# tusen-ai/RangeDet

Hardware: AMD Instinct MI355X
Metric: range-image frames/sec (64x2650, 8ch) at 1/2/4/8 GPU; Meta-Kernel HBM GB/s vs peak (higher is better)
Workload: dtype bf16

## Files before the change

include/rangedet_hip.h:

```cpp
#ifndef RANGEDET_HIP_H_
#define RANGEDET_HIP_H_
#include <stddef.h>
#include <stdint.h>

#ifdef __cplusplus
extern "C" {
#endif

#define RD_OK 0
#define RD_EINVAL (-1)
#define RD_ESHAPE (-2)
#define RD_EWORKSPACE (-3)
#define RD_EHIP (-4)

#define RD_F32 0
#define RD_BF16 1
#define RD_F16 2

#define RD_RELU_PRE 1
#define RD_ADD 2
#define RD_RELU_POST 4
#define RD_SCALE_FOLDED 8
#define RD_MFMA16 16

int rd_version(void);
const char* rd_last_error_string(void);

int rd_nchw_to_nhwc(const float* src, void* dst, int B, int C, int H, int W, int dst_cstride, int dst_coff,
                    int zero_pad, int dst_dtype, void* stream);
int rd_nhwc_to_nchw(const void* src, float* dst, int B, int C, int H, int W, int src_cstride, int src_coff,
                    int src_dtype, void* stream);

int rd_copy_rows(const void* src, long src_row_bytes, void* dst, long dst_row_bytes, long dst_offset_bytes, long bytes,
                 int rows, void* stream);

size_t rd_conv_packed_bytes(int ntaps, int cin, int cout, int dtype);
int rd_pack_conv_weight_host(const float* w_oihw_host, int cout, int cin, int kh, int kw, int dtype,
                             void* packed_host);
int rd_deconv_phase_taps(int kh, int kw, int stride_w, int pad_w, int phase);
int rd_pack_deconv_weight_host(const float* w_iohw_host, int cin, int cout, int kh, int kw, int stride_w,
                               int pad_w, int phase, int dtype, void* packed_host);
int rd_pack_deconv_weight_folded_host(const float* w_iohw_host, const float* fold_scale_host, int cin, int cout, int kh, int kw,
                                      int stride_w, int pad_w, int phase, int dtype, void* packed_host);

int rd_conv2d_bn_act(const void* x, int x_cstride, int x_coff, const void* w_packed, const float* scale,
                     const float* shift, const void* residual, int r_cstride, int r_coff, void* y,
                     int y_cstride, int y_coff, int B, int H, int Win, int cin, int cout, int kh, int kw,
                     int stride_w, int flags, int dtype, void* stream);
size_t rd_conv3x3_ex_packed_bytes(int cin, int cout, int stride_w, int x_cstride);
int rd_pack_conv3x3_ex_host(const float* w_oihw_host, const float* fold_scale_host, int cout, int cin, int stride_w,
                            int x_cstride, int dtype, void* packed_host);
int rd_pack_conv3x3_m16_host(const float* w_oihw_host, const float* fold_scale_host, int cout, int cin, int dtype, void* packed_host);
int rd_conv3x3_mfma16_ok(int cin, int cout, int stride_w, int W, int fused_output_conv);
size_t rd_conv1x1_sc_packed_bytes(int cin, int cout);
int rd_pack_conv1x1_sc_host(const float* w_oi_host, const float* fold_scale_host, int cout, int cin, int dtype,
                            void* packed_host);
int rd_conv3x3_bn_act_ex(const void* x, int x_cstride, int x_coff, const void* w_packed, const float* scale, const float* shift,
                         const void* residual, int r_cstride, int r_coff, const void* sc_x, int sc_cstride, int sc_coff,
                         int sc_cin, const void* sc_w_packed, void* y, int y_cstride, int y_coff, int B, int H, int Win, int cin,
                         int cout, int stride_w, int flags, int dtype, void* stream);
size_t rd_block64_packed_bytes(int cin);
int rd_pack_block64_host(const float* w1_oihw_host, const float* fold_scale1_host, const float* w2_oihw_host,
                         const float* fold_scale2_host, int cin, int dtype, void* packed_host);
int rd_block64_bn_act(const void* x, int x_cstride, int x_coff, int cin, const void* w_packed, const float* shift1, const float* shift2,
                      const void* sc_w_packed, void* y, int y_cstride, int y_coff, int B, int H, int W, int dtype, void* stream);
int rd_pack_block64_m16_host(const float* w1_oihw_host, const float* fold_scale1_host, const float* w2_oihw_host,
                             const float* fold_scale2_host, int dtype, void* packed_host);
int rd_pack_conv1x1_sc_m16_host(const float* w_oi_host, const float* fold_scale_host, int dtype, void* packed_host);
int rd_block64_m16_bn_act(const void* x, int x_cstride, int x_coff, const void* w_packed, const float* shift1, const float* shift2,
                          const void* sc_w_packed, void* y, int y_cstride, int y_coff, int B, int H, int W, int dtype, void* stream);

size_t rd_head_packed_bytes(void);
int rd_pack_head_weight_host(const float* w, int nout, int cin, int dtype, void* out_host);
size_t rd_head_m16_packed_bytes(void);
int rd_pack_head_weight_m16_host(const float* w, int nout, int cin, int dtype, void* out_host);
int rd_conv2d_bn_act_head_out(const void* x, int x_cstride, int x_coff, const void* w_packed, const float* scale,
                              const float* shift, int B, int H, int W, int cin, int flags, const void* head_w_packed,
                              const float* head_bias, float* out, long out_batch_stride, long n_off, int nout, int dtype,
                              void* stream);

size_t rd_conv3x3_cat_packed_bytes(int cin1, int cin2, int cout);
int rd_pack_conv3x3_cat_host(const float* w, const float* fold_scale, int cout, int cin1, int cin2, int dtype, void* out_host);
int rd_conv3x3_bn_act_cat(const void* x1, int x1_cstride, int x1_coff, int cin1, const void* x2, int x2_cstride, int x2_coff, int cin2,
                          const void* w_packed, const float* shift, void* y, int y_cstride, int y_coff, int B, int H, int W, int cout,
                          int flags, int dtype, void* stream);

int rd_deconv2d_bn_act(const void* x, int x_cstride, int x_coff, const void* w_packed_phase,
                       const float* scale, const float* shift, const void* residual, int r_cstride,
                       int r_coff, void* y, int y_cstride, int y_coff, int B, int H, int Win, int cin,
                       int cout, int kh, int kw, int stride_w, int pad_w, int phase, int flags, int dtype,
                       void* stream);

int rd_deconv2d_all_phases_ok(int kh, int kw, int stride_w, int pad_w, int cout, int dtype);
int rd_deconv2d_bn_act_all(const void* x, int x_cstride, int x_coff, const void* w_packed_all, long w_phase_bytes,
                           const float* shift, const void* residual, int r_cstride, int r_coff, void* y, int y_cstride,
                           int y_coff, int B, int H, int Win, int cin, int cout, int kh, int kw, int stride_w, int pad_w,
                           int flags, int dtype, void* stream);

int rd_deconv2d_phase_pairs_ok(int kh, int kw, int stride_w, int pad_w, int cout, int dtype);
int rd_pack_deconv_phase_pair_host(const void* phase_a, const void* phase_b, int cin, int dtype, void* out);
int rd_deconv2d_bn_act_pairs(const void* x, int x_cstride, int x_coff, const void* w_packed_pairs, long w_pair_bytes,
                             const float* shift2, const void* residual, int r_cstride, int r_coff, void* y, int y_cstride,
                             int y_coff, int B, int H, int Win, int cin, int cout, int kh, int kw, int stride_w, int pad_w,
                             int flags, int dtype, void* stream);

int rd_head_out(const void* x, int x_cstride, int x_coff, const float* w, const float* bias, float* out,
                long out_batch_stride, long n_off, int B, int H, int W, int cin, int nout, int dtype,
                void* stream);

size_t rd_meta_packed_bytes(int dtype);
int rd_pack_meta_host(const float* w0, const float* b0, const float* w1, const float* b1, const float* s1,
                      const float* t1, const float* agg, const float* s2, const float* t2, int dtype,
                      void* packed_host);
int rd_meta_kernel_fwd(const void* data, int d_cstride, int d_coff, const float* coord_nchw,
                       const void* packed, void* y, int y_cstride, int y_coff, int B, int H, int W, int dtype,
                       void* stream);

size_t rd_sorted_foreground_workspace_bytes(long N, long k);
int rd_sorted_foreground(const float* cls_score, const float* bbox_delta, const float* pc, const float* mask,
                         int B, long N, long k, int D, int apply_sigmoid, float* out_score, float* out_delta,
                         float* out_pc, int* out_idx, void* ws, size_t ws_bytes, void* stream);

int rd_decode3d_bbox(const float* bbox_delta, const float* pc, float* out, int B, long N, int box_type,
                     int is_bin, void* stream);

size_t rd_score_filter_workspace_bytes(long n);
int rd_score_filter_dets(const float* scores, const float* boxes10, long n, float min_score, float* dets,
                         int* d_count, void* ws, size_t ws_bytes, void* stream);
int rd_score_filter_dets_batched(const float* scores, long scores_bstride, const float* boxes10, long boxes_bstride,
                                 long n, float min_score, float* dets, long dets_bstride, int* d_count, void* ws,
                                 size_t ws_bytes, int B, void* stream);

#define RD_WNMS_MAX_K 65536
#define RD_TIE_STABLE 0
#define RD_TIE_REFERENCE 1
#define RD_WNMS_DIAG_NO_SKIP 0x100
#define RD_WNMS_DIAG_TILE_W(n) (((n) & 0xff) << 16)
#define RD_WNMS_DIAG_MERGE_LDS(n) (((n) & 0x7f) << 24)
size_t rd_wnms_workspace_bytes(int Kcap);
int rd_wnms_4c(const float* dets, int Kcap, const int* d_count, const int* order, int tie_order, float thresh,
               float thresh_vote, int is3d, int hash_scale, float* out_dets, int* keep, int* d_nkeep, void* ws,
               size_t ws_bytes, void* stream);
int rd_wnms_4c_batched(const float* dets, long dets_bstride, int Kcap, const int* d_count, const int* order,
                       long order_bstride, int tie_order, float thresh, float thresh_vote, int is3d, int hash_scale,
                       float* out_dets, long out_bstride, int* keep, long keep_bstride, int* d_nkeep, void* ws,
                       size_t ws_bytes, int B, void* stream);
int rd_single_overlap(const float* dets_a, const float* dets_b, long n, int is3d, float* out, void* stream);
int rd_wnms_pair_skippable(const float* dets_a, const float* dets_b, long n, unsigned char* out, void* stream);

int rd_edge_atan2f(const float* y, const float* x, long n, float* out, void* stream);

int rd_wnms_order_host(const float* dets_host, int K, int* order_host);

int rd_dets12_to_8(const float* dets12, int Mcap, const int* d_count, float* out8, void* stream);
int rd_dets12_to_8_batched(const float* dets12, long dets12_bstride, int Mcap, const int* d_count, float* out8,
                           long out8_bstride, int B, void* stream);

int rd_rotated_iou_8pt(const float* boxes1, const float* boxes2, float* ious, long n1, long n2, void* stream);
int rd_batch_rotated_iou(const float* proposal, int p_stride, const float* gt_bbox, float* iou_map, int* argmax, int B, long N,
                         int n_gt, void* stream);
int rd_batch_rotated_iou_3d(const float* proposal, int p_stride, const float* gt_bbox7, float* iou_map, int* argmax, int B, long N,
                            int n_gt, void* stream);
int rd_rotated_iou_7(const float* boxes1, const float* boxes2, float* ious, long n1, long n2, void* stream);
int rd_batch_max_iou(const float* proposals, int p_stride, const float* gt8, float* out, long n, int n_gt,
                     void* stream);

size_t rd_nms3d_workspace_bytes(long N, int B);
int rd_gather_keep_scores(const float* score, long score_bstride, int k, const int* keep_idx, int max_keep, float* out, int B,
                          void* stream);
int rd_nms3d(const float* boxes, int B, long N, float iou_thres, int max_keep, int normal_iou, int* keep_idx,
             float* bbox_after_nms, void* ws, size_t ws_bytes, void* stream);

int rd_assign3d_v2(const float* pc, const float* bbox, const float* bbox_center, const float* bbox_radius, const float* mask,
                   const float* is_in_nlz, long N, int M, float max_x, float min_x, float max_y, float min_y, float max_z,
                   float min_z, float max_dist, int* out, void* stream);
size_t rd_get_point_num_workspace_bytes(void);
int rd_get_point_num(const float* bbox_inds, long N, float* out, void* ws, size_t ws_bytes, void* stream);

typedef struct {
  float clip_lo[7], clip_hi[7];
  float mean[8], sd[8];
  float interval_lo[3], interval_hi[3];
} rd_input_norm_t;
int rd_input_transform(const float* range_image, const float* pc_vehicle_frame, const float* inclination,
                       const rd_input_norm_t* norm_host, int B, int H, int W, int Hp, int Wp, float* input_data,
                       float* coord_s1, float* pc_s1, float* pc_s2, float* pc_s4, float* mask_s1, float* mask_s2,
                       float* mask_s4, void* stream);

typedef struct {
  float *input_data, *coord_s1;
  float *pc[3], *mask[3];
  float *reg_target[3], *reg_weight[3], *reg_normalize_weight[3], *cls_target[3];
  int* bbox3d_ind;
} rd_train_outputs_t;
size_t rd_train_transform_workspace_bytes(int B);
int rd_train_transform(const float* range_image, const float* pc_vehicle_frame, const float* inclination,
                       const rd_input_norm_t* norm_host, const float* gt_bbox_imu, const float* gt_bbox_center,
                       const float* gt_limits, const float* gt_bbox_csa, const int* num_gt_host, int Mmax, float radius,
                       float max_dist, const float* reg_weight_host, int B, int H, int W, int Hp, int Wp,
                       const rd_train_outputs_t* out_host, void* ws, size_t ws_bytes, void* stream);

size_t rd_range_image_workspace_bytes(int B, int H, int W);
int rd_range_image_from_points(const float* points, const long long* offsets_host, int B, const double* incl_host,
                               const double* height_host, int H, int W, float* range_image, unsigned char* mask, int* point_index,
                               void* ws, size_t ws_bytes, void* stream);

typedef struct {
  float alpha, gamma;
  float cls_loss_weight, reg_loss_weight;
  float smooth_l1_scalar;
  float scale_loss_shift;
  int l1;
} rd_loss_param_t;
size_t rd_rpn_loss_workspace_bytes(int B, long n);
int rd_rpn_loss(const float* logit, long logit_bstride, const float* delta, long delta_bstride, const float* pc, const float* gt_bbox,
                int n_gt, const float* mask, const float* reg_target, const float* reg_weight, const float* reg_norm_weight, int B, int H,
                int Wl, const rd_loss_param_t* p_host, float* cls_loss, float* reg_loss, float* d_logit, float* d_delta,
                float* iou_target, float* boxes10, float* stats, void* ws, size_t ws_bytes, void* stream);

int rd_relu_affine_bwd(const void* g, int g_cstride, int g_coff, const void* y, int y_cstride, int y_coff, const float* scale, void* dz,
                       int dz_cstride, int dz_coff, int B, int H, int W, int C, int dtype, void* stream);
size_t rd_conv3x3_bwd_weight_workspace_bytes(int B, int H, int W, int cin, int cout, int split);
int rd_conv3x3_bwd_weight(const void* x, int x_cstride, int x_coff, const void* dz, int dz_cstride, int dz_coff, float* dW, int B, int H,
                          int W, int cin, int cout, int split, int dtype, void* ws, size_t ws_bytes, void* stream);
size_t rd_conv1x1_bwd_weight_workspace_bytes(int B, int H, int W, int cin, int cout, int split);
size_t rd_conv3x3_bwd_weight_ex_workspace_bytes(int B, int H, int Win, int cin, int cout, int stride_w, int split);
int rd_conv3x3_bwd_weight_ex(const void* x, int x_cstride, int x_coff, const void* dz, int dz_cstride, int dz_coff, float* dW, int B, int H,
                             int Win, int cin, int cout, int stride_w, int split, int dtype, void* ws, size_t ws_bytes, void* stream);
int rd_conv1x1_bwd_weight(const void* x, int x_cstride, int x_coff, const void* dz, int dz_cstride, int dz_coff, float* dW, int B, int H,
                          int W, int cin, int cout, int split, int dtype, void* ws, size_t ws_bytes, void* stream);
size_t rd_deconv_bwd_weight_workspace_bytes(int B, int H, int Win, int cin, int cout, int kw, int stride_w, int pad_w, int split);
int rd_deconv_bwd_weight(const void* x, int x_cstride, int x_coff, const void* dz, int dz_cstride, int dz_coff, float* dW, int B, int H,
                         int Win, int cin, int cout, int kw, int stride_w, int pad_w, int split, int dtype, void* ws, size_t ws_bytes,
                         void* stream);
int rd_pack_deconv_data_grad_host(const float* w, int cin, int cout, int kw, int stride_w, int pad_w, int dtype, void* out);
int rd_pack_deconv_dev(const float* w_dev, int cin, int cout, int kw, int stride_w, int pad_w, int data_grad, long w_phase_bytes, int dtype,
                       void* out_dev, void* stream);
size_t rd_head_out_bwd_workspace_bytes(int B, int H, int W, int cin, int nout);
int rd_head_out_bwd(const float* d_out, long out_batch_stride, long n_off, const void* x, int x_cstride, int x_coff, const float* w,
                    int relu_mask, const float* scale, void* dx, int dx_cstride, int dx_coff, float* dw, float* dbias, int B, int H,
                    int W, int cin, int nout, int dtype, void* ws, size_t ws_bytes, void* stream);
size_t rd_meta_bwd_packed_bytes(int dtype);
int rd_pack_meta_bwd_host(const float* w0, const float* b0, const float* w1, const float* b1, const float* s1, const float* t1,
                          const float* agg, const float* s2, const float* t2, int dtype, void* packed_host);
int rd_meta_kernel_bwd_data(const void* dz, int dz_cstride, int dz_coff, const void* data, int d_cstride, int d_coff, const float* coord_nchw,
                            const void* packed_bwd, const void* residual, int r_cstride, int r_coff, void* ddata, int g_cstride, int g_coff,
                            int B, int H, int W, int dtype, void* stream);
size_t rd_meta_kernel_bwd_workspace_bytes(int B, int H, int W, int split);
int rd_meta_kernel_bwd_params(const void* dz, int dz_cstride, int dz_coff, const void* data, int d_cstride, int d_coff, const float* coord_nchw,
                              const void* packed_bwd, float* dA, float* dW1, float* db1, float* dW0, float* db0, float* dt1, float* dq1, int B,
// ... 62 lines not shown
```

rangedet_amd/csrc/k_conv3.h:

```cpp
#pragma once
#include "k_conv.h"

namespace rd {

struct Conv3Args {
  const bf16_t* x; int x_cs, x_co; long x_bs;
  const unsigned char* w;
  const float* scale; const float* shift;
  const bf16_t* res; int r_cs, r_co; long r_bs;
  bf16_t* y; int y_cs, y_co; long y_bs;
  const unsigned char* zero16;
  int H, W, B, nslots, nchunk, flags, ncol, nrow, ntiles;
  int sw, Wo;
  int xcd;
  unsigned long long* trace;
  const unsigned char* hw;
  const float* hb;
  float* ho; long ho_bs, ho_off; int hn;
  const bf16_t* sx; int s_cs, s_co; long s_bs;
  const unsigned char* scw;
  int s_nks;
  int nph, ts_mask, y_pc, r_pc;
  long w_pb;
  const bf16_t* x2; int x2_cs, x2_co, nchunk1, nslots2; long x2_bs;
// ... 46 lines not shown
      for (int cb = 0; cb < ncb; ++cb)
        for (int lane = 0; lane < 64; ++lane) {
          const int co = conv_row16(cb, lane & 15);
          for (int j = 0; j < 8; ++j) {
            const int ci = c * 32 + (lane >> 4) * 8 + j;
            *o++ = h16_from_f32(dt, ci < cin ? get(co, ci, t) : 0.f);
          }
        }
}

inline void pack_head_frag(const float* w, int nout, int cin, void* out, int dt = RD_BF16) {
  bf16_t* o = (bf16_t*)out;
  for (int part = 0; part < 2; ++part)
    for (int ks = 0; ks < 8; ++ks)
      for (int lane = 0; lane < 64; ++lane)
        for (int j = 0; j < 8; ++j) {
          const int mm = lane & 31, c = 16 * ks + 8 * (lane >> 5) + j;
          const float v = (mm < nout && c < cin) ? w[(size_t)mm * cin + c] : 0.f;
          const bf16_t h = h16_from_f32(dt, v);
          *o++ = part == 0 ? h : h16_from_f32(dt, v - h16_to_f32(dt, h));
        }
}

inline void pack_head_frag16(const float* w, int nout, int cin, void* out, int dt = RD_BF16) {
  bf16_t* o = (bf16_t*)out;
  for (int part = 0; part < 2; ++part)
    for (int p = 0; p < 4; ++p)
      for (int lane = 0; lane < 64; ++lane)
        for (int j = 0; j < 8; ++j) {
          const int mm = lane & 15, c = 32 * p + 8 * (lane >> 4) + j;
          const float v = (mm < nout && c < cin) ? w[(size_t)mm * cin + c] : 0.f;
          const bf16_t h = h16_from_f32(dt, v);
          *o++ = part == 0 ? h : h16_from_f32(dt, v - h16_to_f32(dt, h));
        }
}

inline size_t sc_frag_bytes(int cin, int cout) { return (size_t)((cin + 15) / 16) * (cout / 32) * 1024; }
inline void pack_sc_frag(const float* w, const float* scale, int cin, int cout, void* out, int dt = RD_BF16) {
  bf16_t* o = (bf16_t*)out;
  const int nks = (cin + 15) / 16;
  for (int ks = 0; ks < nks; ++ks)
    for (int cb = 0; cb < cout / 32; ++cb)
      for (int lane = 0; lane < 64; ++lane) {
        const int co = cb * 32 + conv_row_perm(lane & 31);
        for (int j = 0; j < 8; ++j) {
          const int ci = ks * 16 + (lane >> 5) * 8 + j;
          *o++ = h16_from_f32(dt, ci < cin ? (scale ? scale[co] : 1.f) * w[(size_t)co * cin + ci] : 0.f);
        }
      }
}

constexpr int C3_BODY_M16 = 16;
enum { UK_T9 = 0, UK_T6A = 1, UK_T6B = 2, UK_T6R = 3, UK_T3 = 4, UK_P5 = 5 };
constexpr int uk_nsteps(int k) { return k == UK_T9 ? 9 : k == UK_T3 ? 3 : k == UK_P5 ? 5 : 6; }
struct C3KStep { int dh, dw, slot; };
constexpr C3KStep uk_kstep(int k, int s, int ks) {
  if (k == UK_P5) { const int t = 2 * s + ks > 8 ? 8 : 2 * s + ks; return C3KStep{t / 3, t % 3, 0}; }
  const int T = k == UK_T9 ? s : k == UK_T3 ? 3 * s + 1 : 3 * (s / 2) + (s % 2) + (k == UK_T6B ? 1 : 0);
  return C3KStep{T / 3, T % 3, ks};
}
struct C3Body { int nu; int kind[4]; };
constexpr C3Body c3_body(int BODY, int TS = 0) {
  return BODY == 1 ? C3Body{4, {UK_T6A, UK_T3, UK_T3, UK_T6A}} : BODY == 2 ? C3Body{3, {UK_T9, UK_T9, UK_P5, 0}}
       : BODY == 3 ? C3Body{1, {UK_P5, 0, 0, 0}} : C3Body{1, {TS == 0 ? UK_T9 : TS == 1 ? UK_T6A : TS == 2 ? UK_T6B : UK_T6R, 0, 0, 0}};
}
constexpr int c3_nsteps(int TS) { return uk_nsteps(c3_body(0, TS).kind[0]); }
constexpr int c3_body_steps(C3Body bd) { int n = 0; for (int u = 0; u < bd.nu; ++u) n += uk_nsteps(bd.kind[u]); return n; }
constexpr int c3_pieces(int NS, int s, C3Tile tile) {
  if (tile == C3_8x62) return NS == 9 ? (s <= 4 ? 2 : 0) : NS == 6 ? (s <= 1 ? 4 : (s == 2 ? 2 : 0)) : -1;
  return NS == 9 ? (s == 0 ? 2 : s <= 4 ? 1 : 0) : NS == 6 ? (s <= 2 ? 2 : 0) : NS == 5 ? (s <= 1 ? 3 : 0) : (s == 0 ? 6 : 0);
}
constexpr int c3_first(int NS, int s, C3Tile tile) { int n = 0; for (int t = 0; t < s; ++t) n += c3_pieces(NS, t, tile); return n; }
constexpr bool c3_schedule_ok(C3Body bd, C3Tile tile, int HPW) {
  for (int u = 0; u < bd.nu; ++u) {
    int n = 0;
    for (int s = 0; s < uk_nsteps(bd.kind[u]); ++s) {
      if (c3_pieces(uk_nsteps(bd.kind[u]), s, tile) < 0) return false;
      n += c3_pieces(uk_nsteps(bd.kind[u]), s, tile);
    }
    if (n != HPW) return false;
  }
  return true;
}
struct C3Step {
  C3KStep k1, kn;
  int pieces, first;
  int wait;
  bool ufirst, ulast;
};
struct C3Pos { int kind, ns, s; };
constexpr C3Pos c3_pos(C3Body bd, int g) {
  int u = 0;
  while (g >= uk_nsteps(bd.kind[u])) { g -= uk_nsteps(bd.kind[u]); ++u; }
  return C3Pos{bd.kind[u], uk_nsteps(bd.kind[u]), g};
}
constexpr int c3_pieces_at(C3Body bd, int g, C3Tile tile) { return c3_pieces(c3_pos(bd, g).ns, c3_pos(bd, g).s, tile); }
constexpr C3Step c3_step(C3Body bd, int g, C3Tile tile, int R, int IPW) {
  const int G = c3_body_steps(bd);
  const C3Pos p = c3_pos(bd, g), pn = c3_pos(bd, (g + 1) % G);
  int last = 0;
  for (int s = 0; s < p.ns; ++s) if (c3_pieces(p.ns, s, tile) > 0) last = s;
  int wait = (R - 3) * IPW;
  for (int d = 1; d <= R - 2; ++d) wait += c3_pieces_at(bd, ((g - d) % G + G) % G, tile);
  const int cap = (p.ns - 3 - last) * IPW;
  if (p.s == p.ns - 2 && wait > cap) wait = cap;
  return C3Step{uk_kstep(p.kind, p.s, 1), uk_kstep(pn.kind, pn.s, 0), c3_pieces(p.ns, p.s, tile), c3_first(p.ns, p.s, tile), wait, p.s == 0, p.s == p.ns - 1};
}
__host__ __device__ inline int c3b_chunk(int BODY, int i, int nchunk) {
  if (BODY != 1) return i;
  const int r2 = (i >> 2) * 2, j = i & 3, ne = nchunk >> 1;
  return j == 0 ? ne + r2 : j == 1 ? r2 : j == 2 ? r2 + 1 : ne + r2 + 1;
}
template <class F>
inline void pack_body_frag(int BODY, int cin, int cout, void* out, F get, int dt = RD_BF16) {
  const C3Body bd = c3_body(BODY);
  const int nchunk = (cin + 31) / 32, ncb = cout / 32;
  bf16_t* o = (bf16_t*)out;
  for (int i = 0; i < nchunk; ++i) {
    const int kind = bd.kind[i % bd.nu], chunk = c3b_chunk(BODY, i, nchunk);
    for (int s = 0; s < uk_nsteps(kind); ++s)
      for (int ks = 0; ks < 2; ++ks) {
        const C3KStep k = uk_kstep(kind, s, ks);
        const bool zero_tap = kind == UK_P5 && 2 * s + ks > 8;
        for (int cb = 0; cb < ncb; ++cb)
          for (int lane = 0; lane < 64; ++lane) {
            const int co = cb * 32 + conv_row_perm(lane & 31);
            for (int j = 0; j < 8; ++j) {
              const int ci = chunk * 32 + k.slot * 16 + (lane >> 5) * 8 + j;
              *o++ = h16_from_f32(dt, (ci < cin && !zero_tap) ? get(co, ci, k.dh, k.dw) : 0.f);
            }
          }
      }
  }
}
inline int conv3_body_s2(int cin, int x_cstride, bool folded) { return folded && x_cstride % 64 == 0 && cin == x_cstride ? 1 : 0; }
inline int conv3_body_small(int cin, bool folded) { return folded && cin <= 16 ? 3 : 0; }
inline int conv3_body_cat(int cin1, int cin2, bool folded) { return folded && cin1 == 64 && cin2 <= 16 ? 2 : 0; }
#define C3_WAIT_IMM(vm, lgkm) (((vm) & 15) | (((vm) >> 4) << 14) | (7 << 4) | ((lgkm) << 8))
#ifdef RD_EMU_CONTROL_NO_COUNTED_WAITS
#ifdef __HIP_DEVICE_COMPILE__
#error "RD_EMU_CONTROL_NO_COUNTED_WAITS removes the persistent conv's counted waits: emulator (host) builds only"
#endif
#define C3_VMCNT(vm) 63
#else
#define C3_VMCNT(vm) (vm)
#endif

template <int NCT, int TS = 0, bool HEAD = false, bool SC = false, bool FOLD = false, C3Tile TILE = C3_8x62,
          int DT = RD_BF16, int BODY = 0, bool M16 = false>
__global__ __launch_bounds__(256, (TILE == C3_8x32 ? 2 : 1)) void conv3x3_stream_kernel(Conv3Args a) {
  using Cfg = C3Cfg<NCT, TILE>;
  constexpr bool WD = Cfg::WIDE;
  constexpr int FPW = Cfg::FPW, FC = Cfg::FC;
  static_assert(!M16 || (NCT == 4 && WD && FOLD && !SC && TS == 0 && BODY == 0),
                "16 x 16 x 32 form: cout 128 on the 8 x 32 tiles, folded scales, all nine taps");
  static_assert(BODY == 0 || (WD && FOLD && !HEAD && (TS == 0 || TS == 1)), "heterogeneous tile bodies: 8 x 32 tiles, folded scales");
  static_assert(!WD || FOLD, "8 x 32 tile: no room for the scale / shift array");
  static_assert(!HEAD || (NCT == 4 && TS == 0), "fused output conv: cout 128, all nine taps");
  constexpr bool PH = TS == 3;
  static_assert(!PH || (FOLD && !SC && !HEAD), "all-phase transposed conv: folded scales, no shortcut / output conv");
  static_assert(!(HEAD && SC), "a head tower has no shortcut");
  constexpr int R = Cfg::R, IPW = Cfg::IPW, SLAB = Cfg::SLAB, COUT = NCT * 32;
  constexpr int C3_HALO = Cfg::HALO, C3_HPW = Cfg::HPW, C3_TH = Cfg::TH;
  constexpr int C3_TW = Cfg::TW, C3_ROWB = Cfg::ROWB, RW = Cfg::RW;
  constexpr int NR = FPW + NCT;
  constexpr int NM = FPW * NCT;
  constexpr C3Body BD = c3_body(BODY, TS);
  constexpr int BG = c3_body_steps(BD);
  constexpr int BNU = BD.nu;
  static_assert(c3_schedule_ok(BD, TILE, Cfg::HPW), "no halo-piece schedule for a unit of this body on this tile (3- and 5-step units: 8 x 32 only)");
  HIP_DYNAMIC_SHARED(unsigned char, smem);
  const int tid = threadIdx.x, lane = tid & 63, wave = __builtin_amdgcn_readfirstlane(tid >> 6);
  const int m = lane & 31, hi = lane >> 5;
  constexpr int RING = 2 * C3_HALO;
  auto hflip = [](int a_) { return C3_HALO - a_; };
  float* Sc = (float*)(smem + RING + R * SLAB);
  constexpr int HWOFF = RING + R * SLAB + 2 * COUT * (int)sizeof(float);
  if (!WD && tid < COUT) {
    Sc[tid] = a.scale ? a.scale[tid] : 1.f;
    Sc[COUT + tid] = a.shift ? a.shift[tid] : 0.f;
  }
  unsigned bzw[NCT];
  auto load_shift = [&](const float* shp) {
#pragma unroll
    for (int j = 0; j < NCT; ++j) {
      const float t = shp ? shp[32 * j + conv_row_perm(m)] : 0.f;
      const bf16_t th = H16<DT>::from_f32(t);
      const bf16_t tl = H16<DT>::from_f32(t - H16<DT>::to_f32(th));
      bzw[j] = hi ? 0u : ((unsigned)th | ((unsigned)tl << 16));
    }
  };
  if constexpr (FOLD && !M16) load_shift(a.shift);
  unsigned bzw16[M16 ? 2 : 1];
  if constexpr (M16) {
#pragma unroll
    for (int g = 0; g < 2; ++g) {
      const float t = a.shift ? a.shift[conv_row16(4 * g + (lane >> 4), lane & 15)] : 0.f;
      const bf16_t th = H16<DT>::from_f32(t);
      const bf16_t tl = H16<DT>::from_f32(t - H16<DT>::to_f32(th));
      bzw16[g] = (unsigned)th | ((unsigned)tl << 16);
    }
  }
  int tpt = 0;
#define C3_TRACE() { if (a.trace && tid == 0 && tpt < 7) a.trace[(size_t)blockIdx.x * 8 + tpt++] = wall_clock64(); }
  C3_TRACE()
  const unsigned long long clk0 = __builtin_readcyclecounter();

  const int G = gridDim.x, wg = blockIdx.x;
  const int nph = PH ? a.nph : 1;
  const int ntl = ((a.ntiles - wg + G - 1) / G) * nph;
  const int tiles_img = a.ncol * a.nrow;

#if defined(__HIP_DEVICE_COMPILE__)
  const unsigned lds0 = __builtin_amdgcn_readfirstlane((unsigned)(uintptr_t)(__attribute__((address_space(3))) void*)smem);
#endif
  auto dma_s = [&](const unsigned char* sbase, unsigned voff, int lds_off) {
#if defined(__HIP_DEVICE_COMPILE__)
    asm volatile("s_mov_b32 m0, %2\n\ts_nop 0\n\tglobal_load_lds_dwordx4 %0, %1"
                 :: "v"(voff), "s"(sbase), "s"(__builtin_amdgcn_readfirstlane(lds0 + (unsigned)lds_off)) : "memory");
#else
    __builtin_amdgcn_global_load_lds(sbase + voff, smem + lds_off, 16, 0, 0);
#endif
  };
  auto dma_v = [&](const void* vptr, int lds_off) {
#if defined(__HIP_DEVICE_COMPILE__)
    asm volatile("s_mov_b32 m0, %1\n\ts_nop 0\n\tglobal_load_lds_dwordx4 %0, off"
                 :: "v"(vptr), "s"(__builtin_amdgcn_readfirstlane(lds0 + (unsigned)lds_off)) : "memory");
#else
    __builtin_amdgcn_global_load_lds(vptr, smem + lds_off, 16, 0, 0);
#endif
  };
  const int hs = (lane & 3) ^ ((lane >> 4) & 3);
  const int l4 = lane >> 2;
  const unsigned hlane = (unsigned)(l4 * a.x_cs + hs * 8) * 2;
  int hk = 0, hc = 0;
  int hh0 = 0, hlo = 0, hlim = 0;
  const unsigned char* hbase = nullptr;
  bool hsok = false;
  int hcur = 0;
  const int xdq = (G >> 3) / a.nrow;
  const int g_ct = a.xcd ? (8 * xdq) % a.ncol : G % a.ncol, g_rb = a.xcd ? (G >> 3) % a.nrow : (G / a.ncol) % a.nrow,
            g_b = a.xcd ? (8 * xdq) / a.ncol : G / tiles_img;
  const int g_ct1 = (8 * xdq + 8) % a.ncol, g_b1 = (8 * xdq + 8) / a.ncol;
  auto tile_advance = [&](int& ct, int& rb, int& b) __attribute__((always_inline)) {
    int& d0 = a.xcd ? rb : ct;
    int& d1 = a.xcd ? ct : rb;
    const int r0 = a.xcd ? a.nrow : a.ncol, r1 = a.xcd ? a.ncol : a.nrow;
    d0 += a.xcd ? g_rb : g_ct;
    const int c1 = d0 >= r0 ? 1 : 0;
    d0 -= c1 ? r0 : 0;
    d1 += a.xcd ? (c1 ? g_ct1 : g_ct) : g_rb + c1;
    const int c2 = d1 >= r1 ? 1 : 0;
    d1 -= c2 ? r1 : 0;
    b += (a.xcd && c1 ? g_b1 : g_b) + c2;
  };
  const int xs0 = ((wg >> 3) / a.nrow) * 8 + (wg & 7);
  int f_ct = a.xcd ? xs0 % a.ncol : wg % a.ncol, f_rb = a.xcd ? (wg >> 3) % a.nrow : (wg / a.ncol) % a.nrow,
      f_b = a.xcd ? xs0 / a.ncol : wg / tiles_img;
  int c_ct = f_ct, c_rb = f_rb, c_b = f_b;
  int f_ph = 0, c_ph = 0, s_ph = 0;
  const unsigned char* htile = nullptr;
  const unsigned char* htile2 = nullptr;
  int hpxb = a.x_cs * 2, hns = 0;
  auto halo_tile = [&]() {
    const int hw0 = f_ct * C3_TW - 1;
    hh0 = f_rb * C3_TH - 1;
    hlo = hw0 < 0 ? -hw0 : 0;
    hlim = a.W - hw0;
    htile = (const unsigned char*)(a.x + (size_t)f_b * a.x_bs + a.x_co) +
            ((long)hh0 * a.W + hw0) * (long)a.x_cs * 2;
    if constexpr (WD) {
      if (a.x2) htile2 = (const unsigned char*)(a.x2 + (size_t)f_b * a.x2_bs + a.x2_co) + ((long)hh0 * a.W + hw0) * (long)a.x2_cs * 2;
    }
  };
  bool hnew = true;
  auto halo_begin = [&]() {
    if (hnew) { halo_tile(); hnew = false; }
    const int hcm = c3b_chunk(BODY, hc, a.nchunk);
    hbase = htile + hcm * 64;
    hsok = hcm * 4 + hs < a.nslots;
    hcur = hcm;
    if constexpr (WD) {
      hpxb = a.x_cs * 2; hns = a.nslots - 4 * hcm;
      if (a.x2 && hcm >= a.nchunk1) { hbase = htile2 + (hcm - a.nchunk1) * 64; hpxb = a.x2_cs * 2; hns = a.nslots2 - 4 * (hcm - a.nchunk1); }
    }
    if (hc + 1 < a.nchunk) ++hc;
    else if (hk + 1 < ntl) {
      ++hk; hc = 0;
      if constexpr (PH) {
        if (++f_ph == nph) { f_ph = 0; tile_advance(f_ct, f_rb, f_b); hnew = true; }
      } else { tile_advance(f_ct, f_rb, f_b); hnew = true; }
    }
  };
  auto halo_piece = [&](int buf, int j) {
    const int q = wave * C3_HPW + j;
    bool ok;
    const unsigned char* src;
    if constexpr (WD) {
      int ol = lane;
      asm volatile("" : "+v"(ol));
      const int pp = 16 * q + (ol >> 2), r = (pp * 1928) >> 16, cc = pp - 34 * r;
      const int hsp = (ol & 3) ^ ((cc >> 2) & 3);
      ok = hsp < hns && (unsigned)(hh0 + r) < (unsigned)a.H && cc >= hlo && cc < hlim && pp < Cfg::NPX;
      src = hbase + (long)((r * a.W + cc) * hpxb + hsp * 16);
    } else {
    const int r = q >> 2, c16 = (q & 3) * 16;
    const int cc = c16 + l4;
    ok = hsok && (unsigned)(hh0 + r) < (unsigned)a.H && cc >= hlo && cc < hlim;
    const unsigned char* sp = hbase + ((long)r * a.W + c16) * (long)a.x_cs * 2;
    src = sp + hlane;
    }
    dma_v(ok ? (const void*)src : (const void*)a.zero16, buf + q * 1024);
  };
  int fslot = 0, fslab = 0;
  const int nslab_tile = (a.nchunk / BNU) * BG;
  const unsigned char* wsrc = a.w;
  auto slab_piece = [&](int j) {
    dma_s(wsrc + (size_t)fslab * SLAB + (wave * IPW + j) * 1024, lane * 16, RING + fslot * SLAB + (wave * IPW + j) * 1024);
  };
  auto slab_advance = [&]() {
    fslot = fslot + 1 == R ? 0 : fslot + 1;
    fslab = fslab + 1 == nslab_tile ? 0 : fslab + 1;
    if constexpr (PH) {
      if (fslab == 0) {
        s_ph = s_ph + 1 == nph ? 0 : s_ph + 1;
        wsrc = a.w + (size_t)s_ph * a.w_pb;
      }
    }
  };

  int aoff[3];
#pragma unroll
  for (int d = 0; d < 3; ++d) {
    const int c = d + m;
    aoff[d] = c * 64 + (((hi ^ (c >> 2)) & 3) << 4) + wave * RW * C3_ROWB;
    if constexpr (M16) {
      const int c16 = d + (lane & 15);
      aoff[d] = c16 * 64 + ((((lane >> 4) ^ (c16 >> 2)) & 3) << 4) + wave * RW * C3_ROWB;
    }
  }
  const int boff = RING + lane * 16;
  auto side2 = [&](int ph) { return (a.ts_mask >> ph) & 1; };
  int pcol[2] = {aoff[0], aoff[1]}, pq0 = aoff[0];
  if constexpr (PH) {
    const int s0_ = side2(0), s1_ = side2(nph > 1 ? 1 : 0);
    pcol[0] = s0_ ? aoff[1] : aoff[0]; pcol[1] = s0_ ? aoff[2] : aoff[1];
    pq0 = s1_ ? aoff[1] : aoff[0];
  }
  bool lastc = false;
#define C3_AO(D) (PH ? pcol[(D)] : aoff[(D)])

  f32x16 acc[M16 ? 1 : FPW][M16 ? 1 : NCT];
  f32x4 acc6[M16 ? 4 : 1][M16 ? 8 : 1];
  s16x8 fa[2][FPW], fb[2][NCT];
  s16x8 fa16[4];
#define C3_FENCE() __builtin_amdgcn_sched_barrier(0)
#define C3_RD(BUF, K, AADDR, BADDR, KS)                                                                   \
  {                                                                                                       \
    if ((K) == 0) fa[BUF][0] = *(const s16x8*)(smem + (AADDR));                                            \
    else if ((K) <= NCT) fb[BUF][(K) - 1] = *(const s16x8*)(smem + (BADDR) + ((KS) * NCT + (K) - 1) * 1024); \
    else fa[BUF][(K) - NCT] = *(const s16x8*)(smem + (AADDR) + (((K) - NCT) / FC) * C3_ROWB + (((K) - NCT) % FC) * 2048); \
    C3_FENCE();                                                                                           \
  }
#define C3_MM(BUF, N)                                                                                     \
  {                                                                                                       \
    acc[(N) / NCT][(N) % NCT] = H16<DT>::mfma(fb[BUF][(N) % NCT], fa[BUF][(N) / NCT], acc[(N) / NCT][(N) % NCT]); \
    C3_FENCE();                                                                                           \
  }
#define C3_MMZ(BUF, N)                                                                                    \
  {                                                                                                       \
    acc[(N) / NCT][(N) % NCT] = H16<DT>::mfma(fb[BUF][(N) % NCT], fa[BUF][(N) / NCT], f32x16{});             \
    C3_FENCE();                                                                                           \
  }
#define C3_RDW16(BUF, C, BADDR) { fb[BUF][C] = *(const s16x8*)(smem + (BADDR) + (C) * 1024); C3_FENCE(); }
#define C3_RDP16(HX, AADDR) { fa16[HX] = *(const s16x8*)(smem + (AADDR) + ((HX) >> 1) * C3_ROWB + ((HX) & 1) * 1024); C3_FENCE(); }
#define C3_MM16(BK, N)                                                                                                   \
  {                                                                                                                      \
    acc6[(N) >> 2][4 * (BK) + ((N) & 3)] = H16<DT>::mfma16(fb[BK][(N) & 3], fa16[(N) >> 2], acc6[(N) >> 2][4 * (BK) + ((N) & 3)]); \
    C3_FENCE();                                                                                                          \
  }
#define C3_SYNC(VMCNT, LGKM)                                      \
  {                                                               \
    asm volatile("" ::: "memory");                                \
    __builtin_amdgcn_s_waitcnt(C3_WAIT_IMM(C3_VMCNT(VMCNT), LGKM)); \
    __builtin_amdgcn_s_barrier();                                 \
    asm volatile("" ::: "memory");                                \
    C3_FENCE();                                                   \
  }

  halo_begin();
#pragma unroll
  for (int j = 0; j < C3_HPW; ++j) halo_piece(0, j);
  if constexpr (HEAD && !WD) {
#pragma unroll
    for (int j = 0; j < 4; ++j) dma_s(a.hw + (wave * 4 + j) * 1024, lane * 16, HWOFF + (wave * 4 + j) * 1024);
  }
#pragma unroll 1
  for (int s0 = 0; s0 < R; ++s0) {
#pragma unroll
    for (int j = 0; j < IPW; ++j) slab_piece(j);
    slab_advance();
  }
  C3_SYNC(0, 0)
  C3_TRACE()
  constexpr C3KStep K00 = uk_kstep(BD.kind[0], 0, 0);
  constexpr int K00DW = K00.dw, K00DH = K00.dh;
  int rslot = 0;
  int abuf = 0;
  if constexpr (M16) {
#pragma unroll
    for (int k = 0; k < 4; ++k) C3_RDW16(0, k, boff + rslot * SLAB)
#pragma unroll
    for (int k = 0; k < 4; ++k) C3_RDP16(k, aoff[K00DW] + abuf + K00DH * C3_ROWB)
  } else {
#pragma unroll
  for (int k = 0; k < NR; ++k)
    C3_RD(0, k, C3_AO(K00DW) + abuf + K00DH * C3_ROWB, boff + rslot * SLAB, 0)
  }

#define C3_FIRST(D, G_) (BNU == 1 ? c3_first(BG, (G_), TILE) : (D).first)
#define C3_STEP(G_, MM0)                                                                                             \
  if constexpr ((G_) < BG) {                                                                                         \
    constexpr C3Step D_ = c3_step(BD, (G_), TILE, R, IPW);                                                           \
    constexpr int NP_ = IPW + D_.pieces;                                                \
    const int acur_ = (C3_AO(D_.k1.dw) + abuf + D_.k1.dh * C3_ROWB) ^ (D_.k1.slot << 5);                             \
    const int bcur_ = boff + rslot * SLAB;                                                                           \
    const int rnext_ = rslot + 1 == R ? 0 : rslot + 1;                                                               \
    int ncol_ = C3_AO(D_.kn.dw);                                                                                     \
    if constexpr (PH && D_.ulast) { if (lastc) ncol_ = pq0; }   \
    const int anext_ = (ncol_ + (D_.ulast ? hflip(abuf) : abuf) + D_.kn.dh * C3_ROWB) ^ (D_.kn.slot << 5);           \
    const int bnext_ = boff + rnext_ * SLAB;                                                                         \
    const int hbuf_ = hflip(abuf);                                                    \
    C3_FENCE();                                                                                                      \
    _Pragma("unroll") for (int n = 0; n < NM; ++n) {                                                                 \
      MM0(0, n)                                                                                                      \
      if (n < NR) C3_RD(1, n, acur_, bcur_, 1)                                                                       \
    }                                                                                                                \
    _Pragma("unroll") for (int n = 0; n < NM / 2; ++n) {                                                             \
      C3_MM(1, n)                                                                                                    \
      if (n < NR) C3_RD(0, n, anext_, bnext_, 0)                                                                     \
    }                                                                                                                \
    if (NR > NM / 2) { _Pragma("unroll") for (int n = NM / 2; n < NR; ++n) C3_RD(0, n, anext_, bnext_, 0) }          \
    C3_SYNC(D_.wait, NR)                                                                                             \
    if (D_.ufirst) halo_begin();                                                                                     \
    _Pragma("unroll") for (int n = NM / 2; n < NM; ++n) {                                                            \
      C3_MM(1, n)                                                                                                    \
                       \
      _Pragma("unroll") for (int p = 0; p < NP_; ++p)                                                                \
        if (p * (NM / 2) / NP_ == n - NM / 2) {                                                                      \
          if (p < IPW) slab_piece(p); else halo_piece(hbuf_, C3_FIRST(D_, (G_)) + p - IPW);                          \
          C3_FENCE();                                                                                                \
        }                                                                                                            \
    }                                                                                                                \
    slab_advance();                                                                                                  \
    rslot = rnext_;                                                                                                  \
    if (D_.ulast) abuf = hflip(abuf);                                                                                \
  }
#define C3_BODY_FROM1 C3_STEP(1, C3_MM) C3_STEP(2, C3_MM) C3_STEP(3, C3_MM) C3_STEP(4, C3_MM) C3_STEP(5, C3_MM) C3_STEP(6, C3_MM)       \
  C3_STEP(7, C3_MM) C3_STEP(8, C3_MM) C3_STEP(9, C3_MM) C3_STEP(10, C3_MM) C3_STEP(11, C3_MM) C3_STEP(12, C3_MM) C3_STEP(13, C3_MM)     \
  C3_STEP(14, C3_MM) C3_STEP(15, C3_MM) C3_STEP(16, C3_MM) C3_STEP(17, C3_MM) C3_STEP(18, C3_MM) C3_STEP(19, C3_MM) C3_STEP(20, C3_MM)  \
  C3_STEP(21, C3_MM) C3_STEP(22, C3_MM)
  static_assert(BG <= 23, "C3_BODY_FROM1 unrolls 23 steps");

#define C3_STEP16(S)                                                                                                 \
  {                                                                                                                  \
    constexpr C3Step D_ = c3_step(BD, (S), TILE, R, IPW);                                                            \
    constexpr int NP_ = IPW + D_.pieces;                                                                             \
    const int bcur_ = boff + rslot * SLAB;                                                                           \
    const int rnext_ = rslot + 1 == R ? 0 : rslot + 1;                                                               \
    const int anext_ = aoff[D_.kn.dw] + (D_.ulast ? hflip(abuf) : abuf) + D_.kn.dh * C3_ROWB;                        \
    const int bnext_ = boff + rnext_ * SLAB;                                                                         \
    const int hbuf_ = hflip(abuf);                                                                                   \
    C3_FENCE();                                                                                                      \
    _Pragma("unroll") for (int n = 0; n < 16; ++n) {                                                                 \
      C3_MM16(0, n)                                                                                                  \
      if (n < 4) C3_RDW16(1, n, bcur_ + 4096)                                                                        \
    }                                                                                                                \
    _Pragma("unroll") for (int n = 0; n < 8; ++n) {                                                                  \
      C3_MM16(1, n)                                                                                                  \
      if (n < 4) C3_RDW16(0, n, bnext_)                                                                              \
      if (n == 3) C3_RDP16(0, anext_)                                                                                \
      if (n == 7) C3_RDP16(1, anext_)                                                                                \
    }                                                                                                                \
    C3_SYNC(D_.wait, 6)                                                                                              \
    if (D_.ufirst) halo_begin();                                                                                     \
    _Pragma("unroll") for (int n = 8; n < 16; ++n) {                                                                 \
      C3_MM16(1, n)                                                                                                  \
      _Pragma("unroll") for (int p = 0; p < NP_; ++p)                                                                \
        if (p * 8 / NP_ == n - 8) {                                                                                  \
          if (p < IPW) slab_piece(p); else halo_piece(hbuf_, C3_FIRST(D_, (S)) + p - IPW);                           \
          C3_FENCE();                                                                                                \
        }                                                                                                            \
      if (n == 11) C3_RDP16(2, anext_)                                                                               \
      if (n == 15) C3_RDP16(3, anext_)                                                                               \
    }                                                                                                                \
    slab_advance();                                                                                                  \
    rslot = rnext_;                                                                                                  \
    if (D_.ulast) abuf = hflip(abuf);                                                                                \
  }

  for (int k = 0; k < ntl; ++k) {
    if constexpr (PH) lastc = a.nchunk == 1;
    if constexpr (M16) {
      unsigned z0 = 0u;
      asm volatile("" : "+v"(z0));
      int oq = lane >> 4;
      asm volatile("" : "+v"(oq));
      unsigned bq2[2] = {bzw16[0], bzw16[1]};
      asm volatile("" : "+v"(bq2[0]), "+v"(bq2[1]));
#pragma unroll
      for (int cb = 0; cb < 8; ++cb) {
        unsigned ob[4] = {oq == (cb & 3) ? H16<DT>::ONE * 0x10001u : z0, z0, z0, z0};
        unsigned ab[4] = {bq2[cb >> 2], z0, z0, z0};
        s16x8 ones, bz;
        memcpy(&ones, ob, 16);
        memcpy(&bz, ab, 16);
        acc6[0][cb] = H16<DT>::mfma16(bz, ones, f32x4{});
        C3_FENCE();
      }
#pragma unroll
      for (int h = 1; h < 4; ++h)
#pragma unroll
        for (int cb = 0; cb < 8; ++cb) acc6[h][cb] = acc6[0][cb];
      C3_FENCE();
#pragma unroll 1
      for (int c = 0; c < a.nchunk; ++c) {
        C3_STEP16(0) C3_STEP16(1) C3_STEP16(2) C3_STEP16(3) C3_STEP16(4) C3_STEP16(5) C3_STEP16(6) C3_STEP16(7) C3_STEP16(8)
      }
    } else {
    {
      if constexpr (FOLD) {
        unsigned z0 = 0u;
        asm volatile("" : "+v"(z0));
        const unsigned one2 = hi ? z0 : H16<DT>::ONE * 0x10001u;
        unsigned ob[4] = {one2, z0, z0, z0};
        s16x8 ones;
        memcpy(&ones, ob, 16);
#pragma unroll
        for (int n = 0; n < NM; ++n) {
          unsigned ab[4] = {bzw[n % NCT], z0, z0, z0};
          s16x8 bz;
          memcpy(&bz, ab, 16);
          acc[n / NCT][n % NCT] = H16<DT>::mfma(bz, ones, f32x16{});
        }
        C3_FENCE();
        C3_STEP(0, C3_MM)
      } else {
        C3_STEP(0, C3_MMZ)
      }
      C3_BODY_FROM1
    }
#pragma unroll 1
    for (int c = BNU; c < a.nchunk; c += BNU) {
      if constexpr (PH) lastc = c == a.nchunk - 1;
      C3_STEP(0, C3_MM) C3_BODY_FROM1
    }
    }
    if (k == 0) C3_TRACE()

    const int ct = c_ct, rb = c_rb;
    const int b = c_b;
    const int e_ph = c_ph;
    if constexpr (PH) {
      if (++c_ph == nph) { c_ph = 0; tile_advance(c_ct, c_rb, c_b); }
      const int sn_ = side2(c_ph), sq_ = side2(c_ph + 1 == nph ? 0 : c_ph + 1);
      pcol[0] = sn_ ? aoff[1] : aoff[0]; pcol[1] = sn_ ? aoff[2] : aoff[1];
      pq0 = sq_ ? aoff[1] : aoff[0];
    } else
    tile_advance(c_ct, c_rb, c_b);
    const int oh0 = rb * C3_TH + RW * wave;
    int em = m, ehi = hi, el = lane;
    if constexpr (M16) {
      asm volatile("" : "+v"(el));
      em = el & 31; ehi = el >> 5;
    } else
    asm volatile("" : "+v"(em), "+v"(ehi), "+v"(el));
    constexpr int JW = (32 * COUT * 2 <= C3_HALO / 4) ? NCT : NCT / 2, CW = JW * 32, NPASS = NCT / JW;
    static_assert(32 * CW * 2 <= C3_HALO / 4, "transpose scratch");
    constexpr int ROWB = CW * 2, SPR = CW / 8, RPI = 64 / SPR;
    unsigned char* scr = smem + hflip(abuf) + wave * (C3_HALO / 4);
    bf16_t* __restrict__ yrow0 = a.y + (size_t)b * a.y_bs + (size_t)oh0 * a.Wo * a.y_cs + a.y_co + (PH ? e_ph * a.y_pc : 0);
    const bf16_t* __restrict__ rimg0 = a.res + (size_t)b * a.r_bs + a.r_co + (PH ? e_ph * a.r_pc : 0);
    const unsigned char* __restrict__ e_hw = a.hw;
    const float* __restrict__ e_hb = a.hb;
    float* __restrict__ e_ho = a.ho;
    const long e_ho_bs = a.ho_bs;
    const int e_hn = a.hn;
    const int sh = a.sw - 1;
    if constexpr (SC) {
      const bf16_t* __restrict__ sb = a.sx + (size_t)b * a.s_bs + a.s_co + 8 * ehi;
      const unsigned char* __restrict__ wq = a.scw + el * 16;
      auto shortcut = [&](auto MKc) {
        constexpr int MK = decltype(MKc)::value;
#pragma unroll
        for (int kh = 0; kh < 8 / MK; ++kh) {
          if (kh * MK < a.s_nks) {
            s16x8 sxq[FPW][MK];
#pragma unroll
            for (int i = 0; i < FPW; ++i) {
              const int tc = 32 * (i % FC) + em, ow = ct * C3_TW + tc, oh = oh0 + i / FC;
              const bool live = tc < C3_TW && ow < a.W && oh < a.H;
              const bf16_t* sp = sb + (live ? ((size_t)oh * a.W + ow) * a.s_cs : 0) + 16 * MK * kh;
#pragma unroll
              for (int ks = 0; ks < MK; ++ks)
                if (kh * MK + ks < a.s_nks) sxq[i][ks] = *(const s16x8*)(sp + 16 * ks);
            }
#pragma unroll
            for (int ks = 0; ks < MK; ++ks)
              if (kh * MK + ks < a.s_nks) {
#pragma unroll
                for (int j = 0; j < NCT; ++j) {
                  const s16x8 wf = *(const s16x8*)(wq + (size_t)((kh * MK + ks) * NCT + j) * 1024);
#pragma unroll
                  for (int i = 0; i < FPW; ++i)
                    acc[i][j] = H16<DT>::mfma(wf, sxq[i][ks], acc[i][j]);
                }
              }
          }
          C3_FENCE();
        }
      };
      shortcut(std::integral_constant<int, 4>{});
      C3_FENCE();
    }
    auto epilogue = [&](auto FL) {
      constexpr int F = decltype(FL)::value;
      const bool relu_pre = F >= 0 ? (F & RD_RELU_PRE) != 0 : (a.flags & RD_RELU_PRE) != 0;
      const bool do_add = F >= 0 ? (F & RD_ADD) != 0 : (a.flags & RD_ADD) != 0;
      const bool relu_post = F >= 0 ? (F & RD_RELU_POST) != 0 : (a.flags & RD_RELU_POST) != 0;
      Slot16 rv[2][NCT][2];
      auto res_load = [&](int i, Slot16 (&dst)[NCT][2]) {
        const int tc = 32 * (i % FC) + em, ow = ct * C3_TW + tc, oh = oh0 + i / FC;
        const bool live = tc < C3_TW && ow < a.W && oh < a.H && !(ow & sh);
        const bf16_t* rp = rimg0 + (live ? ((size_t)oh * a.Wo + (size_t)(ow >> sh)) * a.r_cs : 0) + 16 * ehi;
#pragma unroll
        for (int j = 0; j < NCT; ++j) {
          dst[j][0] = *(const Slot16*)(rp + j * 32);
          dst[j][1] = *(const Slot16*)(rp + j * 32 + 8);
        }
      };
      if (do_add) res_load(0, rv[0]);
      const bool relu_f32 = relu_pre && do_add;
      const bool relu_i16 = relu_post || (relu_pre && !do_add);
      typedef float f32x2 __attribute__((ext_vector_type(2)));
      typedef short s16x2 __attribute__((ext_vector_type(2)));
      constexpr bool SC_HOIST = NCT == 2;
      f32x4 scq[2][4], shq[2][4];
      auto sc_load = [&](int j, f32x4 (&sc)[4], f32x4 (&sh)[4]) {
#pragma unroll
        for (int g4 = 0; g4 < 4; ++g4) {
          sc[g4] = *(const f32x4*)(Sc + j * 32 + 16 * ehi + 4 * g4);
          sh[g4] = *(const f32x4*)(Sc + COUT + j * 32 + 16 * ehi + 4 * g4);
        }
      };
      if constexpr (!FOLD) {
        sc_load(0, scq[0], shq[0]);
        if constexpr (SC_HOIST) sc_load(1, scq[1], shq[1]);
      }
#pragma unroll
      for (int i = 0; i < FPW; ++i) {
        if (do_add && i + 1 < FPW) res_load(i + 1, rv[(i + 1) & 1]);
        f32x16 h0, h1;
        if constexpr (HEAD) {
#pragma unroll
          for (int r = 0; r < 16; ++r) { h0[r] = 0.f; h1[r] = 0.f; }
        }
#pragma unroll
        for (int jp = 0; jp < NPASS; ++jp) {
        constexpr int KSP = 8 / NPASS;
        s16x8 hwq[HEAD && NPASS == 2 ? 2 : 1][HEAD && NPASS == 2 ? KSP : 1];
        if constexpr (HEAD && NPASS == 2) {
#pragma unroll
          for (int part = 0; part < 2; ++part)
#pragma unroll
            for (int ks = 0; ks < KSP; ++ks)
              hwq[part][ks] = *(const s16x8*)(e_hw + part * 8192 + (jp * KSP + ks) * 1024 + el * 16);
        }
#pragma unroll
        for (int j = jp * JW; j < (jp + 1) * JW; ++j) {
          C3_FENCE();
          const int cur = SC_HOIST ? j : (i * NCT + j) & 1;
          if constexpr (!SC_HOIST && !FOLD) sc_load((j + 1) % NCT, scq[cur ^ 1], shq[cur ^ 1]);
          const int cb = j * 32 + 16 * ehi;
          unsigned pk[8];
#pragma unroll
          for (int g4 = 0; g4 < 4; ++g4) {
#pragma unroll
            for (int h2 = 0; h2 < 2; ++h2) {
              const int r = 4 * g4 + 2 * h2;
              const f32x2 av = {acc[i][j][r], acc[i][j][r + 1]};
              f32x2 v = av;
              if constexpr (!FOLD) {
                const f32x2 s2 = {scq[cur][g4][2 * h2], scq[cur][g4][2 * h2 + 1]};
                const f32x2 t2 = {shq[cur][g4][2 * h2], shq[cur][g4][2 * h2 + 1]};
                v = av * s2 + t2;
              }
              if (relu_f32) v = f32x2{fmaxf(v[0], 0.f), fmaxf(v[1], 0.f)};
              if (do_add) {
                const unsigned w2 = rv[i & 1][j][r >> 3][(r >> 1) & 3];
                v += H16<DT>::unpk(w2);
              }
              unsigned p2 = H16<DT>::pk(v[0], v[1]);
              if (relu_i16) p2 = __builtin_bit_cast(unsigned, __builtin_elementwise_max(__builtin_bit_cast(s16x2, p2), (s16x2){0, 0}));
              pk[2 * g4 + h2] = p2;
            }
          }
#pragma unroll
          for (int u = 0; u < 2; ++u)
            *(Slot16*)(scr + em * ROWB + (((((cb - jp * CW) >> 3) + u) ^ (em & (SPR - 1))) << 4)) =
                Slot16{pk[4 * u], pk[4 * u + 1], pk[4 * u + 2], pk[4 * u + 3]};
        }
        C3_FENCE();
        __builtin_amdgcn_wave_barrier();
        if constexpr (HEAD) {
#pragma unroll
          for (int ks = 0; ks < KSP; ++ks) {
            const s16x8 bq = *(const s16x8*)(scr + em * ROWB + (((2 * ks + ehi) ^ (em & (SPR - 1))) << 4));
            s16x8 wh, wl;
            if constexpr (NPASS == 2) { wh = hwq[0][ks]; wl = hwq[1][ks]; }
            else {
              wh = *(const s16x8*)(smem + HWOFF + ks * 1024 + el * 16);
              wl = *(const s16x8*)(smem + HWOFF + 8192 + ks * 1024 + el * 16);
            }
            h0 = H16<DT>::mfma(wl, bq, h0);
            h1 = H16<DT>::mfma(wh, bq, h1);
          }
          const int tcs = 32 * (i % FC) + em, ows = ct * C3_TW + tcs, ohs = oh0 + i / FC;
          if (jp == NPASS - 1 && tcs < C3_TW && ows < a.W && ohs < a.H) {
            float* o = e_ho + (size_t)b * e_ho_bs + (a.ho_off + (size_t)ohs * a.W + ows) * e_hn + 4 * ehi;
            if (e_hn == 8 && !((size_t)o & 15)) {
              const f32x4 bv = *(const f32x4*)(e_hb + 4 * ehi);
              *(f32x4*)o = f32x4{(h0[0] + h1[0]) + bv[0], (h0[1] + h1[1]) + bv[1], (h0[2] + h1[2]) + bv[2], (h0[3] + h1[3]) + bv[3]};
            } else {
#pragma unroll
              for (int r = 0; r < 4; ++r)
                if (4 * ehi + r < e_hn) o[r] = (h0[r] + h1[r]) + e_hb[4 * ehi + r];
            }
          }
        } else {
#pragma unroll
          for (int it = 0; it < 32 / RPI; ++it) {
            const int pr = it * RPI + el / SPR, sl = el % SPR;
            const Slot16 v = *(const Slot16*)(scr + pr * ROWB + ((sl ^ (pr & (SPR - 1))) << 4));
            const int tcs = 32 * (i % FC) + pr, ows = ct * C3_TW + tcs;
            if (tcs < C3_TW && ows < a.W && oh0 + i / FC < a.H && !(ows & sh))
              __builtin_nontemporal_store(v, (Slot16*)(yrow0 + (size_t)(i / FC) * a.Wo * a.y_cs + (size_t)(ows >> sh) * a.y_cs + jp * CW + sl * 8));
          }
        }
        __builtin_amdgcn_wave_barrier();
        C3_FENCE();
        }
      }
    };
    auto epilogue16 = [&](auto FL) {
      constexpr int F = decltype(FL)::value;
      const bool relu_pre = F >= 0 ? (F & RD_RELU_PRE) != 0 : (a.flags & RD_RELU_PRE) != 0;
      const bool do_add = F >= 0 ? (F & RD_ADD) != 0 : (a.flags & RD_ADD) != 0;
      const bool relu_post = F >= 0 ? (F & RD_RELU_POST) != 0 : (a.flags & RD_RELU_POST) != 0;
      const bool relu_f32 = relu_pre && do_add;
      const bool relu_i16 = relu_post || (relu_pre && !do_add);
      typedef float f32x2 __attribute__((ext_vector_type(2)));
      typedef short s16x2 __attribute__((ext_vector_type(2)));
      const int en = el & 15, eq = el >> 4;
      Slot16 rv[2][2][JW];
      auto res_load = [&](int t, Slot16 (&dst)[2][JW]) {
        const int i = t / NPASS, jp = t % NPASS;
#pragma unroll
        for (int hf = 0; hf < 2; ++hf) {
          const int ow = ct * C3_TW + 16 * hf + en, oh = oh0 + i;
          const bool live = ow < a.W && oh < a.H;
          const bf16_t* rp = rimg0 + (live ? ((size_t)oh * a.Wo + (size_t)ow) * a.r_cs : 0) + 8 * eq + jp * CW;
#pragma unroll
          for (int pp = 0; pp < JW; ++pp) dst[hf][pp] = *(const Slot16*)(rp + 32 * pp);
        }
      };
      if (do_add) res_load(0, rv[0]);
#pragma unroll
      for (int i = 0; i < FPW; ++i) {
        f32x4 hh[HEAD ? 2 : 1][HEAD ? 2 : 1];
        if constexpr (HEAD) {
#pragma unroll
          for (int hf = 0; hf < 2; ++hf)
#pragma unroll
            for (int part = 0; part < 2; ++part) hh[hf][part] = f32x4{0.f, 0.f, 0.f, 0.f};
        }
#pragma unroll
        for (int jp = 0; jp < NPASS; ++jp) {
          const int t = NPASS * i + jp;
          if (do_add && t + 1 < NPASS * FPW) res_load(t + 1, rv[(t + 1) & 1]);
          s16x8 hwq[HEAD ? 2 : 1][HEAD ? JW : 1];
          if constexpr (HEAD) {
#pragma unroll
            for (int part = 0; part < 2; ++part)
#pragma unroll
              for (int pp = 0; pp < JW; ++pp)
                hwq[part][pp] = *(const s16x8*)(e_hw + part * 4096 + (jp * JW + pp) * 1024 + el * 16);
          }
#pragma unroll
          for (int hf = 0; hf < 2; ++hf)
#pragma unroll
            for (int pp = 0; pp < JW; ++pp) {
              C3_FENCE();
              const int p = jp * JW + pp, h = 2 * i + hf;
              unsigned pk[4];
#pragma unroll
              for (int w2 = 0; w2 < 4; ++w2) {
                const f32x4 av = acc6[h][2 * p + (w2 >> 1)];
                f32x2 v = {av[2 * (w2 & 1)], av[2 * (w2 & 1) + 1]};
                if (relu_f32) v = f32x2{fmaxf(v[0], 0.f), fmaxf(v[1], 0.f)};
                if (do_add) v += H16<DT>::unpk(rv[t & 1][hf][pp][w2]);
                unsigned p2 = H16<DT>::pk(v[0], v[1]);
                if (relu_i16) p2 = __builtin_bit_cast(unsigned, __builtin_elementwise_max(__builtin_bit_cast(s16x2, p2), (s16x2){0, 0}));
                pk[w2] = p2;
              }
              if constexpr (HEAD) {
                s16x8 bq;
                memcpy(&bq, pk, 16);
                hh[hf][0] = H16<DT>::mfma16(hwq[1][pp], bq, hh[hf][0]);
                hh[hf][1] = H16<DT>::mfma16(hwq[0][pp], bq, hh[hf][1]);
              } else {
                const int px = 16 * hf + en;
                *(Slot16*)(scr + px * ROWB + (((4 * pp + eq) ^ (px & (SPR - 1))) << 4)) = Slot16{pk[0], pk[1], pk[2], pk[3]};
              }
            }
          C3_FENCE();
          if constexpr (!HEAD) {
          __builtin_amdgcn_wave_barrier();
#pragma unroll
          for (int it = 0; it < 32 / RPI; ++it) {
            const int pr = it * RPI + el / SPR, sl = el % SPR;
            const Slot16 v = *(const Slot16*)(scr + pr * ROWB + ((sl ^ (pr & (SPR - 1))) << 4));
            const int ows = ct * C3_TW + pr;
            if (ows < a.W && oh0 + i < a.H)
              __builtin_nontemporal_store(v, (Slot16*)(yrow0 + (size_t)i * a.Wo * a.y_cs + (size_t)ows * a.y_cs + jp * CW + sl * 8));
          }
          __builtin_amdgcn_wave_barrier();
          C3_FENCE();
          }
        }
        if constexpr (HEAD) {
#pragma unroll
          for (int hf = 0; hf < 2; ++hf) {
            const int ows = ct * C3_TW + 16 * hf + en, ohs = oh0 + i;
            if (eq < 2 && ows < a.W && ohs < a.H) {
              float* o = e_ho + (size_t)b * e_ho_bs + (a.ho_off + (size_t)ohs * a.W + ows) * e_hn + 4 * eq;
              if (e_hn == 8 && !((size_t)o & 15)) {
                const f32x4 bv = *(const f32x4*)(e_hb + 4 * eq);
                *(f32x4*)o = f32x4{(hh[hf][0][0] + hh[hf][1][0]) + bv[0], (hh[hf][0][1] + hh[hf][1][1]) + bv[1],
                                   (hh[hf][0][2] + hh[hf][1][2]) + bv[2], (hh[hf][0][3] + hh[hf][1][3]) + bv[3]};
              } else {
#pragma unroll
                for (int r = 0; r < 4; ++r)
                  if (4 * eq + r < e_hn) o[r] = (hh[hf][0][r] + hh[hf][1][r]) + e_hb[4 * eq + r];
              }
            }
          }
          C3_FENCE();
        }
      }
    };
    if constexpr (M16) {
      static_assert(!M16 || (NPASS == 2 && JW == 2 && CW == 64), "M16 epilogue: two passes of 64 channels");
      if (a.flags == RD_RELU_POST) epilogue16(std::integral_constant<int, RD_RELU_POST>{});
      else if (a.flags == (RD_ADD | RD_RELU_POST)) epilogue16(std::integral_constant<int, RD_ADD | RD_RELU_POST>{});
      else epilogue16(std::integral_constant<int, -1>{});
    } else {
    if (a.flags == RD_RELU_POST) epilogue(std::integral_constant<int, RD_RELU_POST>{});
    else if (a.flags == (RD_ADD | RD_RELU_POST)) epilogue(std::integral_constant<int, RD_ADD | RD_RELU_POST>{});
    else if (TS != 0 && a.flags == (RD_RELU_PRE | RD_ADD)) epilogue(std::integral_constant<int, RD_RELU_PRE | RD_ADD>{});
    else epilogue(std::integral_constant<int, -1>{});
    }
    if (k == 0) C3_TRACE()
  }
  __builtin_amdgcn_s_waitcnt(RD_VMCNT_IMM(0));
  C3_TRACE()
  if (a.trace && tid == 0) a.trace[(size_t)blockIdx.x * 8 + 7] = __builtin_readcyclecounter() - clk0;
#undef C3_STEP16
#undef C3_MM16
#undef C3_RDP16
#undef C3_RDW16
#undef C3_BODY_FROM1
#undef C3_FIRST
#undef C3_AO
#undef C3_STEP
#undef C3_MMZ
#undef C3_SYNC
#undef C3_MM
#undef C3_RD
#undef C3_FENCE
#undef C3_TRACE
}


template <int NCT, int TS, bool HEAD, bool SC, bool FOLD, C3Tile TILE, int DT, int BODY = 0, bool M16 = false>
inline int c3_go(int grid, hipStream_t st, const Conv3Args& a) {
  auto k = conv3x3_stream_kernel<NCT, TS, HEAD, SC, FOLD, TILE, DT, BODY, M16>;
  static std::atomic<unsigned long long> seen{0};
  once_per_device(seen, [&] { allow_big_lds(k); });
  constexpr size_t lds = C3Cfg<NCT, TILE>::LDS + (HEAD && TILE == C3_8x62 ? 16384 : 0);
  hipLaunchKernelGGL(k, dim3(grid), dim3(256), lds, st, a);
  return check_launch("conv3x3_stream_kernel");
}

#ifdef RD_BUILD_F16_PRODUCTION_FORMS_ONLY
constexpr bool kF16AllForms = false;
#else
constexpr bool kF16AllForms = true;
#endif
inline bool conv3_has_form(int dt, bool fold) { return kF16AllForms || dt == RD_BF16 || fold; }

inline bool conv3_eligible(const TapList& tl, int in_stride, int out_stride, int cout, int dt, int Win, int Wq, int Wout) {
  if (!is_h16(dt) || !conv3_has_form(dt, false) || tl.n != 9 || (in_stride != 1 && in_stride != 2) || out_stride != 1) return false;
  if (Wq != (Win - 1) / in_stride + 1 || Wout != Wq) return false;
  if (cout != 64 && cout != 128) return false;
  for (int t = 0; t < 9; ++t)
    if (tl.dh[t] != t / 3 - 1 || tl.dw[t] != t % 3 - 1) return false;
  return true;
}

struct Conv3Phases { int nph, ts_mask, y_pc, r_pc; long w_pb; };
struct Conv3Src2 { const void* x; int cs, co, cin1, cin2; };
inline bool conv3_phases_eligible(int cout, int flags) {
  return (cout == 64 || cout == 128) && (flags & RD_SCALE_FOLDED);
}
inline bool conv3_mfma16_ok(int cin, int cout, int stride_w) {
  return cout == 128 && stride_w == 1 && cin >= 32 && cin % 32 == 0;
}

template <int DT>
inline int launch_conv3_dt(const void* x, int x_cs, int x_co, const void* w, const float* scale, const float* shift,
                           const void* res, int r_cs, int r_co, void* y, int y_cs, int y_co, int B, int H, int W, int cin,
                           int cout, int flags, int sw, hipStream_t st, int ts, const Conv3Args* head,
                           const Conv3Phases* ph, const Conv3Src2* s2, int body);
inline int launch_conv3(const void* x, int x_cs, int x_co, const void* w, const float* scale, const float* shift,
                        const void* res, int r_cs, int r_co, void* y, int y_cs, int y_co, int B, int H, int W, int cin,
                        int cout, int flags, int sw, hipStream_t st, int ts, const Conv3Args* head, int dt,
                        const Conv3Phases* ph, const Conv3Src2* s2, int body) {
  RD_REQUIRE(is_h16(dt), RD_EINVAL, "conv3: dtype %d (the persistent 3x3 kernel takes RD_BF16 or RD_F16)", dt);
  if (dt == RD_F16) return launch_conv3_dt<RD_F16>(x, x_cs, x_co, w, scale, shift, res, r_cs, r_co, y, y_cs, y_co, B, H, W, cin, cout, flags, sw, st, ts, head, ph, s2, body);
  return launch_conv3_dt<RD_BF16>(x, x_cs, x_co, w, scale, shift, res, r_cs, r_co, y, y_cs, y_co, B, H, W, cin, cout, flags, sw, st, ts, head, ph, s2, body);
}

template <int DT>
inline int launch_conv3_dt(const void* x, int x_cs, int x_co, const void* w, const float* scale, const float* shift,
                           const void* res, int r_cs, int r_co, void* y, int y_cs, int y_co, int B, int H, int W, int cin,
                           int cout, int flags, int sw, hipStream_t st, int ts, const Conv3Args* head,
                           const Conv3Phases* ph, const Conv3Src2* s2, int body) {
  Conv3Args a;
  memset(&a, 0, sizeof(a));
  a.nph = 1;
  if (ph) { a.nph = ph->nph; a.ts_mask = ph->ts_mask; a.y_pc = ph->y_pc; a.r_pc = ph->r_pc; a.w_pb = ph->w_pb; }
  if (head) { a.hw = head->hw; a.hb = head->hb; a.ho = head->ho; a.ho_bs = head->ho_bs; a.ho_off = head->ho_off; a.hn = head->hn; }
  const bool sc = head && head->sx;
  const bool fold = (flags & RD_SCALE_FOLDED) != 0;
  RD_REQUIRE(!fold || !scale, RD_EINVAL, "conv3: RD_SCALE_FOLDED takes no scale array (the packer folded it into the weights)");
  flags &= ~RD_SCALE_FOLDED;
  if (sc) { a.sx = head->sx; a.s_cs = head->s_cs; a.s_co = head->s_co; a.s_bs = head->s_bs; a.scw = head->scw; a.s_nks = head->s_nks; }
  a.sw = sw; a.Wo = (W - 1) / sw + 1;
  a.x = (const bf16_t*)x; a.x_cs = x_cs; a.x_co = x_co; a.x_bs = (long)H * W * x_cs;
  a.w = (const unsigned char*)w; a.scale = scale; a.shift = shift;
  a.res = (const bf16_t*)res; a.r_cs = r_cs; a.r_co = r_co; a.r_bs = (long)H * a.Wo * r_cs;
  a.y = (bf16_t*)y; a.y_cs = y_cs; a.y_co = y_co; a.y_bs = (long)H * a.Wo * y_cs;
  a.zero16 = (const unsigned char*)w + conv_packed_body_bytes(c3_nsteps(ts), cin, cout, RD_BF16);
  a.H = H; a.W = W; a.B = B; a.nslots = cin_slots(cin, RD_BF16); a.nchunk = (cin + 31) / 32; a.flags = flags;
  const bool headfuse = head && !sc;
  RD_REQUIRE(!headfuse || cout == 128, RD_ESHAPE, "conv3 + output conv: cout %d (128)", cout);
  const bool wide = fold && (!headfuse || W <= 1400 || body == C3_BODY_M16);
  const int tw = wide ? C3Cfg<4, C3_8x32>::TW : C3Cfg<4, C3_8x62>::TW, th = C3Cfg<4>::TH;
  a.ncol = (W + tw - 1) / tw; a.nrow = (H + th - 1) / th; a.ntiles = a.ncol * a.nrow * B;
  if (s2) {
    RD_REQUIRE(wide && sw == 1 && s2->cin1 > 0 && s2->cin1 % 32 == 0 && s2->cin1 + s2->cin2 == cin && s2->cin2 > 0, RD_ESHAPE,
               "conv3: a two-tensor input needs the 8 x 32 tile form and cin1 a multiple of 32 (cin1 %d, cin2 %d, cin %d)", s2->cin1, s2->cin2, cin);
    a.x2 = (const bf16_t*)s2->x; a.x2_cs = s2->cs; a.x2_co = s2->co; a.x2_bs = (long)H * W * s2->cs;
    a.nchunk1 = s2->cin1 / 32; a.nslots2 = cin_slots(s2->cin2, RD_BF16); a.nslots = a.nchunk1 * 4;
  }
  const int grid = std::min(a.ntiles, conv_num_cus() * (wide ? 2 : 1));
  a.xcd = (a.ncol * B) % 8 == 0 && grid % 8 == 0;
  if (conv_trace_buf() && (size_t)grid * 8 <= (1u << 20)) a.trace = conv_trace_buf();
  ProfScope ps(RD_PROF_CONV3, st);
#ifdef RD_CONV3_DEV_M16_ONLY
  RD_REQUIRE(wide && !sc && !ph && !s2 && sw == 1 && ts == 0 && cout == 128 && DT == RD_BF16 && (!headfuse || body == C3_BODY_M16), RD_ESHAPE, "conv16_dev: plain bf16 cout-128 form only");
  if (body == C3_BODY_M16 && headfuse) return c3_go<4, 0, true, false, true, C3_8x32, RD_BF16, 0, true>(grid, st, a);
  if (body == C3_BODY_M16) return c3_go<4, 0, false, false, true, C3_8x32, RD_BF16, 0, true>(grid, st, a);
  return c3_go<4, 0, false, false, true, C3_8x32, RD_BF16>(grid, st, a);
#else
  constexpr bool kAllForms = kF16AllForms || DT == RD_BF16;
  RD_REQUIRE(kAllForms || fold, RD_ESHAPE, "conv3: this fp16 launch form is not instantiated in the emulator build (conv3_has_form)");
  if (sc) {
    RD_REQUIRE(ts == 0 || ts == 1, RD_ESHAPE, "conv3 + shortcut: tap set %d", ts);
    RD_REQUIRE(fold, RD_EINVAL, "conv3 + shortcut: the weights must carry the folded scales (RD_SCALE_FOLDED)");
  }
  if (body == C3_BODY_M16) {
    RD_REQUIRE(wide && !sc && !ph && !s2 && sw == 1 && ts == 0 && cout == 128 && cin % 32 == 0, RD_ESHAPE,
               "conv3: the 16 x 16 x 32 form needs the 8 x 32 tile form: cout 128, folded scales, stride 1, cin a multiple of 32 (cin %d)%s", cin,
               headfuse ? " (rd_conv3x3_mfma16_ok)" : "");
    if (headfuse) return c3_go<4, 0, true, false, true, C3_8x32, DT, 0, true>(grid, st, a);
    return c3_go<4, 0, false, false, true, C3_8x32, DT, 0, true>(grid, st, a);
  }
  if (body) {
    RD_REQUIRE(wide && !headfuse && !ph && sw == 1 && a.nchunk % c3_body(body).nu == 0, RD_ESHAPE,
               "conv3: tile body %d needs the 8 x 32 tile form with folded scales (%d chunks)", body, a.nchunk);
    if (body == 1) {
      RD_REQUIRE(ts == 1 && !s2, RD_ESHAPE, "conv3: body 1 is the stride-2 pair view");
      if (sc) { if (cout == 128) return c3_go<4, 1, false, true, true, C3_8x32, DT, 1>(grid, st, a); return c3_go<2, 1, false, true, true, C3_8x32, DT, 1>(grid, st, a); }
      if (cout == 128) return c3_go<4, 1, false, false, true, C3_8x32, DT, 1>(grid, st, a);
      return c3_go<2, 1, false, false, true, C3_8x32, DT, 1>(grid, st, a);
    }
    RD_REQUIRE(ts == 0 && !sc, RD_ESHAPE, "conv3: tile body %d takes all nine taps, no shortcut", body);
    if (body == 2) { if (cout == 128) return c3_go<4, 0, false, false, true, C3_8x32, DT, 2>(grid, st, a); return c3_go<2, 0, false, false, true, C3_8x32, DT, 2>(grid, st, a); }
    if (cout == 128) return c3_go<4, 0, false, false, true, C3_8x32, DT, 3>(grid, st, a);
    return c3_go<2, 0, false, false, true, C3_8x32, DT, 3>(grid, st, a);
  }
  if (ph) {
    RD_REQUIRE(wide && !sc && !head && ts == 3 && sw == 1 && ph->nph >= 1 && ph->nph <= 8, RD_ESHAPE,
               "conv3: all phases per launch need the 8 x 32 tile form (folded scales, no shortcut / output conv)");
    if (cout == 128) return c3_go<4, 3, false, false, true, C3_8x32, DT>(grid, st, a);
    return c3_go<2, 3, false, false, true, C3_8x32, DT>(grid, st, a);
  }
  if (wide) {
    if (headfuse) return c3_go<4, 0, true, false, true, C3_8x32, DT>(grid, st, a);
#define C3_BODY(N)                                                                                        \
  {                                                                                                       \
    if (sc) return ts == 0 ? c3_go<N, 0, false, true, true, C3_8x32, DT>(grid, st, a)                     \
                           : c3_go<N, 1, false, true, true, C3_8x32, DT>(grid, st, a);                    \
    return ts == 0 ? c3_go<N, 0, false, false, true, C3_8x32, DT>(grid, st, a)                            \
         : ts == 1 ? c3_go<N, 1, false, false, true, C3_8x32, DT>(grid, st, a)                            \
                   : c3_go<N, 2, false, false, true, C3_8x32, DT>(grid, st, a);                           \
  }
    if (cout == 128) C3_BODY(4)
    C3_BODY(2)
#undef C3_BODY
  }
  if (headfuse && fold) return c3_go<4, 0, true, false, true, C3_8x62, DT>(grid, st, a);
  if constexpr (kAllForms) {
    if (headfuse) return c3_go<4, 0, true, false, false, C3_8x62, DT>(grid, st, a);
    RD_REQUIRE(!fold, RD_ESHAPE, "conv3: folded scales without an output conv take the 8 x 32 tile");
#define C3_PLAIN(N) return ts == 0 ? c3_go<N, 0, false, false, false, C3_8x62, DT>(grid, st, a) : ts == 1 ? c3_go<N, 1, false, false, false, C3_8x62, DT>(grid, st, a) : c3_go<N, 2, false, false, false, C3_8x62, DT>(grid, st, a);
    if (cout == 128) { C3_PLAIN(4) }
    C3_PLAIN(2)
#undef C3_PLAIN
  }
  return rd::fail(RD_ESHAPE, "conv3: launch form not available");
#endif
}

}
```

rangedet_amd/csrc/rd_api.hip:

```cpp
#include "k_conv1.h"
#include "k_block.h"
#include "k_assign.h"
#include "k_input.h"
#include "k_target.h"
#include "k_rangeimg.h"
#include "k_nms3d.h"
#include "k_meta.h"
#include "k_misc.h"
#include "k_riou.h"
#include "k_loss.h"
#include "k_convbwd.h"
#include "k_metabwd.h"
#include "k_norm.h"
#include "k_optim.h"
#include "k_sort.h"
#include "k_wnms.h"

#include <algorithm>
#include <string>
#include <numeric>

using namespace rd;

namespace rd {
// ... 24 lines not shown
}
inline void allow_conv_lds() {
  static std::atomic<unsigned long long> seen{0};
  once_per_device(seen, [] {
    allow_big_lds(conv_taps_kernel<RD_BF16, 4, 3>); allow_big_lds(conv_taps_kernel<RD_BF16, 4, 8>);
    allow_big_lds(conv_taps_kernel<RD_F16, 4, 3>); allow_big_lds(conv_taps_kernel<RD_F16, 4, 8>);
    allow_big_lds(conv_taps_kernel<RD_F32, 4, 8>); allow_big_lds(conv_taps_kernel<RD_F32, 4, 3>);
  });
}
}

extern "C" {

int rd_version(void) { return 100; }
const char* rd_last_error_string(void) { return rd::err_buf(); }

int rd_nchw_to_nhwc(const float* src, void* dst, int B, int C, int H, int W, int dst_cstride, int dst_coff,
                    int zero_pad, int dst_dtype, void* stream) {
  RD_REQUIRE(src && dst, RD_EINVAL, "nchw_to_nhwc: null pointer");
  RD_REQUIRE(B > 0 && C > 0 && H > 0 && W > 0 && zero_pad >= 0, RD_ESHAPE, "nchw_to_nhwc: bad shape");
  RD_REQUIRE(dst_coff >= 0 && dst_coff + C + zero_pad <= dst_cstride, RD_ESHAPE, "nchw_to_nhwc: channels exceed stride");
  hipStream_t st = (hipStream_t)stream;
  const long HW = (long)H * W, total = (long)B * (C + zero_pad) * HW;
  const int grid = (int)std::min<long>((total + 255) / 256, 8192);
  ProfScope ps(RD_PROF_LAYOUT, st);
  {
    const int ch = ch_per_slot(dst_dtype), ctot = C + zero_pad;
    if ((is_h16(dst_dtype) || dst_dtype == RD_F32) && ctot % ch == 0 && ctot / ch <= 2 && dst_cstride % ch == 0 && dst_coff % ch == 0) {
      const long npix = (long)B * HW;
      const int g2 = (int)std::min<long>((npix + 255) / 256, 8192);
#define RD_PX(DT, NS) hipLaunchKernelGGL((nchw_to_nhwc_px_kernel<DT, NS>), dim3(g2), dim3(256), 0, st, src, dst, C, HW, dst_cstride, dst_coff, npix)
      if (dst_dtype == RD_BF16) { if (ctot / ch == 1) RD_PX(RD_BF16, 1); else RD_PX(RD_BF16, 2); }
      else if (dst_dtype == RD_F16) { if (ctot / ch == 1) RD_PX(RD_F16, 1); else RD_PX(RD_F16, 2); }
      else { if (ctot / ch == 1) RD_PX(RD_F32, 1); else RD_PX(RD_F32, 2); }
#undef RD_PX
      return check_launch("nchw_to_nhwc");
    }
  }
  if (dst_dtype == RD_BF16)
    hipLaunchKernelGGL(nchw_to_nhwc_kernel<RD_BF16>, dim3(grid), dim3(256), 0, st, src, dst, C, HW, dst_cstride, dst_coff, zero_pad, total);
  else if (dst_dtype == RD_F16)
    hipLaunchKernelGGL(nchw_to_nhwc_kernel<RD_F16>, dim3(grid), dim3(256), 0, st, src, dst, C, HW, dst_cstride, dst_coff, zero_pad, total);
  else if (dst_dtype == RD_F32)
    hipLaunchKernelGGL(nchw_to_nhwc_kernel<RD_F32>, dim3(grid), dim3(256), 0, st, src, dst, C, HW, dst_cstride, dst_coff, zero_pad, total);
  else
    return rd::fail(RD_EINVAL, "nchw_to_nhwc: dtype %d", dst_dtype);
  return check_launch("nchw_to_nhwc");
}
int rd_copy_rows(const void* src, long src_row_bytes, void* dst, long dst_row_bytes, long dst_offset_bytes, long bytes,
                 int rows, void* stream) {
  RD_REQUIRE(src && dst, RD_EINVAL, "copy_rows: null pointer");
  RD_REQUIRE(rows > 0 && bytes > 0 && src_row_bytes >= bytes && dst_row_bytes >= dst_offset_bytes + bytes && dst_offset_bytes >= 0,
             RD_ESHAPE, "copy_rows: bad geometry");
  ProfScope ps(RD_PROF_LAYOUT, (hipStream_t)stream);
  if (hipMemcpy2DAsync((char*)dst + dst_offset_bytes, (size_t)dst_row_bytes, src, (size_t)src_row_bytes, (size_t)bytes,
                       (size_t)rows, hipMemcpyDeviceToDevice, (hipStream_t)stream) != hipSuccess)
    return rd::fail(RD_EHIP, "copy_rows: hipMemcpy2DAsync failed");
  return RD_OK;
}
int rd_nhwc_to_nchw(const void* src, float* dst, int B, int C, int H, int W, int src_cstride, int src_coff,
                    int src_dtype, void* stream) {
  RD_REQUIRE(src && dst, RD_EINVAL, "nhwc_to_nchw: null pointer");
  RD_REQUIRE(B > 0 && C > 0 && H > 0 && W > 0, RD_ESHAPE, "nhwc_to_nchw: bad shape");
  RD_REQUIRE(src_coff >= 0 && src_coff + C <= src_cstride, RD_ESHAPE, "nhwc_to_nchw: channels exceed stride");
  hipStream_t st = (hipStream_t)stream;
  const long HW = (long)H * W, total = (long)B * C * HW;
  const int grid = (int)std::min<long>((total + 255) / 256, 8192);
  ProfScope ps(RD_PROF_LAYOUT, st);
  if (src_dtype == RD_BF16)
    hipLaunchKernelGGL(nhwc_to_nchw_kernel<RD_BF16>, dim3(grid), dim3(256), 0, st, src, dst, C, HW, src_cstride, src_coff, total);
  else if (src_dtype == RD_F16)
    hipLaunchKernelGGL(nhwc_to_nchw_kernel<RD_F16>, dim3(grid), dim3(256), 0, st, src, dst, C, HW, src_cstride, src_coff, total);
  else if (src_dtype == RD_F32)
    hipLaunchKernelGGL(nhwc_to_nchw_kernel<RD_F32>, dim3(grid), dim3(256), 0, st, src, dst, C, HW, src_cstride, src_coff, total);
  else
    return rd::fail(RD_EINVAL, "nhwc_to_nchw: dtype %d", src_dtype);
  return check_launch("nhwc_to_nchw");
}

size_t rd_conv_packed_bytes(int ntaps, int cin, int cout, int dtype) { return conv_packed_bytes(ntaps, cin, cout, dtype); }
int rd_pack_conv_weight_host(const float* w, int cout, int cin, int kh, int kw, int dtype, void* out) {
  RD_REQUIRE(w && out, RD_EINVAL, "pack_conv: null pointer");
  RD_REQUIRE(dtype == RD_F32 || is_h16(dtype), RD_EINVAL, "pack_conv: dtype");
  RD_REQUIRE(kh * kw >= 1 && kh * kw <= 9 && (kh & 1) && (kw & 1), RD_ESHAPE, "pack_conv: kernel (%d,%d)", kh, kw);
  TapList tl = conv_taps(kh, kw);
  auto get = [&](int co, int ci, int t) { return w[(((size_t)co * cin + ci) * kh + tl.kh[t]) * kw + tl.kw[t]]; };
  memset(out, 0, conv_packed_bytes(tl.n, cin, cout, dtype));
  if (is_h16(dtype)) pack_taps_frag(tl.n, cin, cout, out, get, dtype);
  else pack_taps(tl.n, cin, cout, dtype, out, get);
  return RD_OK;
}
static bool deconv_embeds_3x3(const TapList& tl) {
  for (int t = 0; t < tl.n; ++t)
    if (tl.dh[t] < -1 || tl.dh[t] > 1 || tl.dw[t] < -1 || tl.dw[t] > 1) return false;
  return tl.n >= 1 && tl.n <= 9;
}
static int deconv_tap_set(const TapList& tl) {
  if (tl.n != 6 || !deconv_embeds_3x3(tl)) return 0;
  for (int ts = 1; ts <= 2; ++ts) {
    bool seen[6] = {false, false, false, false, false, false};
    bool ok = true;
    for (int t = 0; t < 6 && ok; ++t) {
      const int c = tl.dw[t] - (ts == 1 ? -1 : 0);
      if (c < 0 || c > 1) ok = false;
      else seen[(tl.dh[t] + 1) * 2 + c] = true;
    }
    for (int i = 0; i < 6 && ok; ++i) ok = seen[i];
    if (ok) return ts;
  }
  return 0;
}
static TapList deconv_taps_sorted(int kh, int kw, int s, int pad_w, int phase) {
  TapList tl = deconv_taps(kh, kw, s, pad_w, phase);
  if (tl.n > 9) return tl;
  for (int i = 1; i < tl.n; ++i)
    for (int j = i; j > 0 && (tl.dh[j] < tl.dh[j - 1] || (tl.dh[j] == tl.dh[j - 1] && tl.dw[j] < tl.dw[j - 1])); --j) {
      std::swap(tl.dh[j], tl.dh[j - 1]); std::swap(tl.dw[j], tl.dw[j - 1]);
      std::swap(tl.kh[j], tl.kh[j - 1]); std::swap(tl.kw[j], tl.kw[j - 1]);
    }
  return tl;
}
int rd_deconv_phase_taps(int kh, int kw, int stride_w, int pad_w, int phase) {
  if (stride_w < 1 || phase < 0 || phase >= stride_w) return RD_EINVAL;
  TapList tl = deconv_taps(kh, kw, stride_w, pad_w, phase);
  if (tl.n > 9) return RD_ESHAPE;
  return (deconv_embeds_3x3(tl) && !deconv_tap_set(tl)) ? 9 : tl.n;
}
int rd_pack_deconv_weight_host(const float* w, int cin, int cout, int kh, int kw, int stride_w, int pad_w,
                               int phase, int dtype, void* out) {
  return rd_pack_deconv_weight_folded_host(w, nullptr, cin, cout, kh, kw, stride_w, pad_w, phase, dtype, out);
}
int rd_pack_deconv_weight_folded_host(const float* w, const float* fold_scale, int cin, int cout, int kh, int kw, int stride_w,
                                      int pad_w, int phase, int dtype, void* out) {
  RD_REQUIRE(w && out, RD_EINVAL, "pack_deconv: null pointer");
  RD_REQUIRE(dtype == RD_F32 || is_h16(dtype), RD_EINVAL, "pack_deconv: dtype");
  RD_REQUIRE(stride_w >= 1 && phase >= 0 && phase < stride_w, RD_EINVAL, "pack_deconv: phase");
  TapList tl = deconv_taps_sorted(kh, kw, stride_w, pad_w, phase);
  RD_REQUIRE(tl.n >= 1 && tl.n <= 9, RD_ESHAPE, "pack_deconv: %d taps", tl.n);
  const bool emb = deconv_embeds_3x3(tl) && !deconv_tap_set(tl);
  auto get = [&](int co, int ci, int t) -> float {
    if (emb) {
      int src = -1;
      for (int u = 0; u < tl.n; ++u)
        if (tl.dh[u] == t / 3 - 1 && tl.dw[u] == t % 3 - 1) src = u;
      if (src < 0) return 0.f;
      t = src;
    }
    return (fold_scale ? fold_scale[co] : 1.f) * w[(((size_t)ci * cout + co) * kh + tl.kh[t]) * kw + tl.kw[t]];
  };
  const int nt = emb ? 9 : tl.n;
  memset(out, 0, conv_packed_bytes(nt, cin, cout, dtype));
  if (is_h16(dtype)) pack_taps_frag(nt, cin, cout, out, get, dtype);
  else pack_taps(nt, cin, cout, dtype, out, get);
  return RD_OK;
}

int rd_conv2d_bn_act(const void* x, int x_cstride, int x_coff, const void* w_packed, const float* scale,
                     const float* shift, const void* residual, int r_cstride, int r_coff, void* y, int y_cstride,
                     int y_coff, int B, int H, int Win, int cin, int cout, int kh, int kw, int stride_w, int flags,
                     int dtype, void* stream) {
  RD_REQUIRE(x && w_packed && y, RD_EINVAL, "conv2d: null pointer");
  RD_REQUIRE((kh == 1 && kw == 1) || (kh == 3 && kw == 3), RD_ESHAPE, "conv2d: kernel (%d,%d) not in {1x1,3x3}", kh, kw);
  RD_REQUIRE(stride_w == 1 || stride_w == 2, RD_ESHAPE, "conv2d: stride_w %d", stride_w);
  RD_REQUIRE(y_coff >= 0 && y_coff + cout <= y_cstride, RD_ESHAPE, "conv2d: y channels exceed stride");
  const int pad = (kw - 1) / 2;
  const int Wout = (Win + 2 * pad - kw) / stride_w + 1;
  RD_REQUIRE(!(flags & RD_SCALE_FOLDED), RD_EINVAL, "conv2d: RD_SCALE_FOLDED is taken by rd_conv3x3_bn_act_ex / rd_conv2d_bn_act_head_out / rd_deconv2d_bn_act");
  TapList tl = conv_taps(kh, kw);
  allow_conv_lds();
  return launch_conv(tl, x, x_cstride, x_coff, w_packed, scale, shift, residual, r_cstride, r_coff, y, y_cstride,
                     y_coff, B, H, Win, Wout, Wout, cin, cout, stride_w, 1, 0, flags, dtype, (hipStream_t)stream);
}
static int ex_view_cin(int cin, int x_cstride, int stride_w) { return stride_w == 2 ? x_cstride + cin : cin; }
size_t rd_conv3x3_ex_packed_bytes(int cin, int cout, int stride_w, int x_cstride) {
  return conv_packed_bytes(stride_w == 2 ? 6 : 9, ex_view_cin(cin, x_cstride, stride_w), cout, RD_BF16);
}
int rd_pack_conv3x3_ex_host(const float* w, const float* fold_scale, int cout, int cin, int stride_w, int x_cstride, int dtype,
                            void* out) {
  RD_REQUIRE(w && out, RD_EINVAL, "pack_conv3x3_ex: null pointer");
  RD_REQUIRE(is_h16(dtype), RD_EINVAL, "pack_conv3x3_ex: dtype %d (RD_BF16 or RD_F16)", dtype);
  RD_REQUIRE(stride_w == 1 || stride_w == 2, RD_ESHAPE, "pack_conv3x3_ex: stride_w %d", stride_w);
  RD_REQUIRE(cout == 64 || cout == 128, RD_ESHAPE, "pack_conv3x3_ex: cout %d", cout);
  RD_REQUIRE(stride_w == 1 || (x_cstride >= cin && x_cstride % 8 == 0), RD_ESHAPE, "pack_conv3x3_ex: x_cstride %d for cin %d", x_cstride, cin);
  auto wv = [&](int co, int ci, int dh, int dw) {
    return (fold_scale ? fold_scale[co] : 1.f) * w[(((size_t)co * cin + ci) * 3 + (dh + 1)) * 3 + (dw + 1)];
  };
  memset(out, 0, rd_conv3x3_ex_packed_bytes(cin, cout, stride_w, x_cstride));
  auto wv2 = [&](int co, int c2, int dh, int dw2) -> float {
    if (c2 < cin) return dw2 == 0 ? wv(co, c2, dh, 0) : 0.f;
    if (c2 >= x_cstride && c2 - x_cstride < cin) return wv(co, c2 - x_cstride, dh, dw2 == -1 ? -1 : 1);
    return 0.f;
  };
  if (stride_w == 1) {
    if (conv3_body_small(cin, fold_scale != nullptr))
      pack_body_frag(3, cin, cout, out, [&](int co, int ci, int dh, int dw) { return wv(co, ci, dh - 1, dw - 1); }, dtype);
    else
      pack_taps_frag(9, cin, cout, out, [&](int co, int ci, int t) { return wv(co, ci, t / 3 - 1, t % 3 - 1); }, dtype);
  } else if (conv3_body_s2(cin, x_cstride, fold_scale != nullptr)) {
    pack_body_frag(1, x_cstride + cin, cout, out, [&](int co, int c2, int dh, int dw) { return wv2(co, c2, dh - 1, dw - 1); }, dtype);
  } else {
    pack_taps_frag(6, x_cstride + cin, cout, out, [&](int co, int c2, int s) -> float { return wv2(co, c2, s / 2 - 1, s % 2 - 1); }, dtype);
  }
  return RD_OK;
}
int rd_pack_conv3x3_m16_host(const float* w, const float* fold_scale, int cout, int cin, int dtype, void* out) {
  RD_REQUIRE(w && out, RD_EINVAL, "pack_conv3x3_m16: null pointer");
  RD_REQUIRE(is_h16(dtype), RD_EINVAL, "pack_conv3x3_m16: dtype %d (RD_BF16 or RD_F16)", dtype);
  RD_REQUIRE(cout == 128 && cin >= 32 && cin % 32 == 0, RD_ESHAPE, "pack_conv3x3_m16: cout %d (128), cin %d (a multiple of 32)", cout, cin);
  memset(out, 0, rd_conv3x3_ex_packed_bytes(cin, cout, 1, cin));
  pack_taps_frag16(9, cin, cout, out, [&](int co, int ci, int t) {
    return (fold_scale ? fold_scale[co] : 1.f) * w[(((size_t)co * cin + ci) * 3 + t / 3) * 3 + t % 3];
  }, dtype);
  return RD_OK;
}
int rd_conv3x3_mfma16_ok(int cin, int cout, int stride_w, int W, int fused_output_conv) {
  (void)W; (void)fused_output_conv;
  return conv3_mfma16_ok(cin, cout, stride_w) ? 1 : 0;
}
size_t rd_conv1x1_sc_packed_bytes(int cin, int cout) { return sc_frag_bytes(cin, cout); }
int rd_pack_conv1x1_sc_host(const float* w, const float* fold_scale, int cout, int cin, int dtype, void* out) {
  RD_REQUIRE(w && out, RD_EINVAL, "pack_conv1x1_sc: null pointer");
  RD_REQUIRE(is_h16(dtype), RD_EINVAL, "pack_conv1x1_sc: dtype %d (RD_BF16 or RD_F16)", dtype);
  RD_REQUIRE((cout == 64 || cout == 128) && cin >= 1 && cin <= 128, RD_ESHAPE, "pack_conv1x1_sc: cout %d, cin %d (1..128)", cout, cin);
  pack_sc_frag(w, fold_scale, cin, cout, out, dtype);
  return RD_OK;
}
int rd_conv3x3_bn_act_ex(const void* x, int x_cstride, int x_coff, const void* w_packed, const float* scale, const float* shift,
                         const void* residual, int r_cstride, int r_coff, const void* sc_x, int sc_cstride, int sc_coff,
                         int sc_cin, const void* sc_w_packed, void* y, int y_cstride, int y_coff, int B, int H, int Win, int cin,
                         int cout, int stride_w, int flags, int dtype, void* stream) {
  RD_REQUIRE(x && w_packed && y, RD_EINVAL, "conv3x3_ex: null pointer");
  RD_REQUIRE(is_h16(dtype), RD_EINVAL, "conv3x3_ex: dtype %d (RD_BF16 or RD_F16)", dtype);
  RD_REQUIRE(B > 0 && H > 0 && Win > 0 && cin > 0 && (cout == 64 || cout == 128), RD_ESHAPE, "conv3x3_ex: shape / cout %d", cout);
  RD_REQUIRE(stride_w == 1 || (stride_w == 2 && Win % 2 == 0), RD_ESHAPE, "conv3x3_ex: stride_w %d with Win %d (stride 2 needs an even width)", stride_w, Win);
  RD_REQUIRE(y_coff >= 0 && y_coff + cout <= y_cstride, RD_ESHAPE, "conv3x3_ex: y channels exceed stride");
  RD_REQUIRE(x_cstride % 8 == 0 && x_coff % 8 == 0 && x_coff + cin_slots(cin, RD_BF16) * 8 <= x_cstride, RD_ESHAPE, "conv3x3_ex: x channel stride/offset");
  RD_REQUIRE(!(sc_x && residual) && !(sc_x && !sc_w_packed), RD_EINVAL, "conv3x3_ex: shortcut conv and residual are exclusive");
  RD_REQUIRE(!((flags & RD_ADD) && !residual && !sc_x), RD_EINVAL, "conv3x3_ex: RD_ADD without residual / shortcut");
  allow_conv_lds();
  const int v = stride_w;
  const int Wv = Win / v;
  Conv3Args e;
  memset(&e, 0, sizeof(e));
  int fl = flags;
  if (sc_x) {
    RD_REQUIRE(sc_cin >= 1 && sc_cin <= 128 && sc_cstride % 8 == 0 && sc_coff % 8 == 0 && sc_coff + ((sc_cin + 15) / 16) * 16 <= sc_cstride,
               RD_ESHAPE, "conv3x3_ex: shortcut input channels %d (stride %d, offset %d)", sc_cin, sc_cstride, sc_coff);
    e.sx = (const bf16_t*)sc_x; e.s_cs = sc_cstride * v; e.s_co = sc_coff; e.s_bs = (long)H * Wv * sc_cstride * v;
    e.scw = (const unsigned char*)sc_w_packed; e.s_nks = (sc_cin + 15) / 16;
    fl &= ~RD_ADD;
    fl |= RD_SCALE_FOLDED;
  }
  RD_REQUIRE(!(fl & RD_SCALE_FOLDED) || !scale, RD_EINVAL, "conv3x3_ex: folded weights take no scale array");
  const bool m16 = (fl & RD_MFMA16) != 0;
  fl &= ~RD_MFMA16;
  const bool folded = (fl & RD_SCALE_FOLDED) != 0;
  RD_REQUIRE(!m16 || (folded && !sc_x && conv3_mfma16_ok(cin, cout, stride_w)), RD_ESHAPE,
             "conv3x3_ex: RD_MFMA16 takes folded weights of rd_pack_conv3x3_m16_host: stride 1, cout 128, cin a multiple of 32, no fused shortcut (rd_conv3x3_mfma16_ok)");
  const int body = m16 ? C3_BODY_M16 : stride_w == 2 ? conv3_body_s2(cin, x_cstride, folded) : (sc_x ? 0 : conv3_body_small(cin, folded));
  RD_REQUIRE(!(stride_w == 1 && sc_x && conv3_body_small(cin, folded)), RD_ESHAPE, "conv3x3_ex: at most 16 input channels together with a fused shortcut is not a launch form");
  return launch_conv3(x, x_cstride * v, x_coff, w_packed, scale, shift, residual, r_cstride, r_coff, y, y_cstride, y_coff, B, H,
                      Wv, ex_view_cin(cin, x_cstride, stride_w), cout, fl, 1, (hipStream_t)stream, stride_w == 2 ? 1 : 0,
                      sc_x ? &e : nullptr, dtype, nullptr, nullptr, body);
}

size_t rd_block64_packed_bytes(int cin) { return block64_packed_bytes(cin); }
int rd_pack_block64_host(const float* w1, const float* fold_scale1, const float* w2, const float* fold_scale2, int cin, int dtype, void* out) {
  RD_REQUIRE(w1 && w2 && out, RD_EINVAL, "pack_block64: null pointer");
  RD_REQUIRE(is_h16(dtype), RD_EINVAL, "pack_block64: dtype %d (RD_BF16 or RD_F16)", dtype);
  RD_REQUIRE(cin == 64 || (cin >= 1 && cin <= 16), RD_ESHAPE, "pack_block64: %d input channels (64, or at most 16)", cin);
  pack_block64(w1, fold_scale1, w2, fold_scale2, cin, dtype, out);
  return RD_OK;
}
int rd_block64_bn_act(const void* x, int x_cstride, int x_coff, int cin, const void* w_packed, const float* shift1, const float* shift2,
                      const void* sc_w_packed, void* y, int y_cstride, int y_coff, int B, int H, int W, int dtype, void* stream) {
  RD_REQUIRE(x && w_packed && shift1 && shift2 && y, RD_EINVAL, "block64: null pointer");
  RD_REQUIRE(is_h16(dtype), RD_EINVAL, "block64: dtype %d (RD_BF16 or RD_F16)", dtype);
  RD_REQUIRE(B > 0 && H > 0 && W > 0, RD_ESHAPE, "block64: shape");
  RD_REQUIRE(cin == 64 || (cin >= 1 && cin <= 16), RD_ESHAPE, "block64: %d input channels (64, or at most 16 for the network's first block)", cin);
  RD_REQUIRE(x_cstride % 8 == 0 && x_coff % 8 == 0 && x_coff >= 0 && x_coff + cin_slots(cin, RD_BF16) * 8 <= x_cstride, RD_ESHAPE, "block64: x channel stride / offset");
  RD_REQUIRE(cin > 16 || x_coff + 16 <= x_cstride, RD_ESHAPE, "block64: the first block reads 16 channels per pixel (x_coff %d + 16 > x_cstride %d)", x_coff, x_cstride);
  RD_REQUIRE(y_cstride % 8 == 0 && y_coff % 8 == 0 && y_coff >= 0 && y_coff + 64 <= y_cstride, RD_ESHAPE, "block64: y channel stride / offset");
  RD_REQUIRE(x != y, RD_EINVAL, "block64: in-place (a tile's halo is another tile's output)");
  return launch_block64(x, x_cstride, x_coff, cin, w_packed, shift1, shift2, sc_w_packed, y, y_cstride, y_coff, B, H, W, dtype, (hipStream_t)stream);
}

int rd_pack_block64_m16_host(const float* w1, const float* fold_scale1, const float* w2, const float* fold_scale2, int dtype, void* out) {
  RD_REQUIRE(w1 && w2 && out, RD_EINVAL, "pack_block64_m16: null pointer");
  RD_REQUIRE(is_h16(dtype), RD_EINVAL, "pack_block64_m16: dtype %d (RD_BF16 or RD_F16)", dtype);
  pack_block64_m16(w1, fold_scale1, w2, fold_scale2, dtype, out);
  return RD_OK;
}
int rd_pack_conv1x1_sc_m16_host(const float* w, const float* fold_scale, int dtype, void* out) {
  RD_REQUIRE(w && out, RD_EINVAL, "pack_conv1x1_sc_m16: null pointer");
  RD_REQUIRE(is_h16(dtype), RD_EINVAL, "pack_conv1x1_sc_m16: dtype %d (RD_BF16 or RD_F16)", dtype);
  pack_sc_frag16(w, fold_scale, out, dtype);
  return RD_OK;
}
int rd_block64_m16_bn_act(const void* x, int x_cstride, int x_coff, const void* w_packed, const float* shift1, const float* shift2,
                          const void* sc_w_packed, void* y, int y_cstride, int y_coff, int B, int H, int W, int dtype, void* stream) {
  RD_REQUIRE(x && w_packed && shift1 && shift2 && y, RD_EINVAL, "block64_m16: null pointer");
  RD_REQUIRE(is_h16(dtype), RD_EINVAL, "block64_m16: dtype %d (RD_BF16 or RD_F16)", dtype);
  RD_REQUIRE(B > 0 && H > 0 && W > 0, RD_ESHAPE, "block64_m16: shape");
  RD_REQUIRE(x_cstride % 8 == 0 && x_coff % 8 == 0 && x_coff >= 0 && x_coff + 64 <= x_cstride, RD_ESHAPE, "block64_m16: x channel stride / offset");
  RD_REQUIRE(y_cstride % 8 == 0 && y_coff % 8 == 0 && y_coff >= 0 && y_coff + 64 <= y_cstride, RD_ESHAPE, "block64_m16: y channel stride / offset");
  RD_REQUIRE(x != y, RD_EINVAL, "block64_m16: in-place (a tile's halo is another tile's output)");
  return launch_block64(x, x_cstride, x_coff, 64, w_packed, shift1, shift2, sc_w_packed, y, y_cstride, y_coff, B, H, W, dtype, (hipStream_t)stream, true);
}

size_t rd_conv3x3_cat_packed_bytes(int cin1, int cin2, int cout) { return conv_packed_bytes(9, cin1 + cin2, cout, RD_BF16); }
int rd_pack_conv3x3_cat_host(const float* w, const float* fold_scale, int cout, int cin1, int cin2, int dtype, void* out) {
  RD_REQUIRE(w && out, RD_EINVAL, "pack_conv3x3_cat: null pointer");
  RD_REQUIRE(is_h16(dtype), RD_EINVAL, "pack_conv3x3_cat: dtype %d (RD_BF16 or RD_F16)", dtype);
  RD_REQUIRE((cout == 64 || cout == 128) && cin1 > 0 && cin1 % 32 == 0 && cin2 > 0 && cin2 % 8 == 0, RD_ESHAPE,
             "pack_conv3x3_cat: cout %d, cin1 %d (multiple of 32), cin2 %d (multiple of 8)", cout, cin1, cin2);
  const int cin = cin1 + cin2;
  auto wv = [&](int co, int ci, int dh, int dw) {
    return (fold_scale ? fold_scale[co] : 1.f) * w[(((size_t)co * cin + ci) * 3 + (dh + 1)) * 3 + (dw + 1)];
  };
  memset(out, 0, rd_conv3x3_cat_packed_bytes(cin1, cin2, cout));
  const int body = conv3_body_cat(cin1, cin2, fold_scale != nullptr);
  if (body) pack_body_frag(body, cin, cout, out, [&](int co, int ci, int dh, int dw) { return wv(co, ci, dh - 1, dw - 1); }, dtype);
  else pack_taps_frag(9, cin, cout, out, [&](int co, int ci, int t) { return wv(co, ci, t / 3 - 1, t % 3 - 1); }, dtype);
  return RD_OK;
}
int rd_conv3x3_bn_act_cat(const void* x1, int x1_cstride, int x1_coff, int cin1, const void* x2, int x2_cstride, int x2_coff, int cin2,
                          const void* w_packed, const float* shift, void* y, int y_cstride, int y_coff, int B, int H, int W, int cout,
                          int flags, int dtype, void* stream) {
  RD_REQUIRE(x1 && x2 && w_packed && y && shift, RD_EINVAL, "conv3x3_cat: null pointer");
  RD_REQUIRE(is_h16(dtype), RD_EINVAL, "conv3x3_cat: dtype %d (RD_BF16 or RD_F16)", dtype);
  RD_REQUIRE((flags & RD_SCALE_FOLDED) && !(flags & RD_ADD), RD_EINVAL, "conv3x3_cat: needs RD_SCALE_FOLDED weights, takes no residual");
  RD_REQUIRE(B > 0 && H > 0 && W > 0 && (cout == 64 || cout == 128), RD_ESHAPE, "conv3x3_cat: shape / cout %d", cout);
  RD_REQUIRE(cin1 > 0 && cin1 % 32 == 0 && cin2 > 0 && cin2 % 8 == 0, RD_ESHAPE, "conv3x3_cat: cin1 %d (multiple of 32), cin2 %d (multiple of 8)", cin1, cin2);
  RD_REQUIRE(y_coff >= 0 && y_coff + cout <= y_cstride, RD_ESHAPE, "conv3x3_cat: y channels exceed stride");
  RD_REQUIRE(x1_cstride % 8 == 0 && x1_coff % 8 == 0 && x1_coff + cin1 <= x1_cstride && x2_cstride % 8 == 0 && x2_coff % 8 == 0 &&
             x2_coff + cin2 <= x2_cstride, RD_ESHAPE, "conv3x3_cat: channel stride/offset");
  allow_conv_lds();
  Conv3Src2 s2;
  s2.x = x2; s2.cs = x2_cstride; s2.co = x2_coff; s2.cin1 = cin1; s2.cin2 = cin2;
  return launch_conv3(x1, x1_cstride, x1_coff, w_packed, nullptr, shift, nullptr, 0, 0, y, y_cstride, y_coff, B, H, W, cin1 + cin2, cout, flags,
                      1, (hipStream_t)stream, 0, nullptr, dtype, nullptr, &s2, conv3_body_cat(cin1, cin2, true));
}

size_t rd_head_packed_bytes(void) { return 16384; }
int rd_pack_head_weight_host(const float* w, int nout, int cin, int dtype, void* out_host) {
  RD_REQUIRE(w && out_host, RD_EINVAL, "pack_head_weight: null pointer");
  RD_REQUIRE(is_h16(dtype), RD_EINVAL, "pack_head_weight: dtype %d (RD_BF16 or RD_F16)", dtype);
  RD_REQUIRE(nout >= 1 && nout <= 8 && cin >= 1 && cin <= 128, RD_ESHAPE, "pack_head_weight: nout %d (1..8), cin %d (1..128)", nout, cin);
  pack_head_frag(w, nout, cin, out_host, dtype);
  return RD_OK;
}
size_t rd_head_m16_packed_bytes(void) { return 8192; }
int rd_pack_head_weight_m16_host(const float* w, int nout, int cin, int dtype, void* out_host) {
  RD_REQUIRE(w && out_host, RD_EINVAL, "pack_head_weight_m16: null pointer");
  RD_REQUIRE(is_h16(dtype), RD_EINVAL, "pack_head_weight_m16: dtype %d (RD_BF16 or RD_F16)", dtype);
  RD_REQUIRE(nout >= 1 && nout <= 8 && cin >= 1 && cin <= 128, RD_ESHAPE, "pack_head_weight_m16: nout %d (1..8), cin %d (1..128)", nout, cin);
  pack_head_frag16(w, nout, cin, out_host, dtype);
  return RD_OK;
}
int rd_conv2d_bn_act_head_out(const void* x, int x_cstride, int x_coff, const void* w_packed, const float* scale,
                              const float* shift, int B, int H, int W, int cin, int flags, const void* head_w_packed,
                              const float* head_bias, float* out, long out_batch_stride, long n_off, int nout, int dtype,
                              void* stream) {
  RD_REQUIRE(x && w_packed && head_w_packed && head_bias && out, RD_EINVAL, "conv2d_head_out: null pointer");
  RD_REQUIRE(is_h16(dtype), RD_EINVAL, "conv2d_head_out: dtype %d (RD_BF16 or RD_F16)", dtype);
  RD_REQUIRE(B > 0 && H > 0 && W > 0 && cin > 0 && nout >= 1 && nout <= 8, RD_ESHAPE, "conv2d_head_out: shape / nout %d (1..8)", nout);
  RD_REQUIRE(!(flags & RD_ADD), RD_EINVAL, "conv2d_head_out: no residual in a head tower");
  RD_REQUIRE(x_cstride % 8 == 0 && x_coff % 8 == 0 && x_coff + cin_slots(cin, RD_BF16) * 8 <= x_cstride, RD_ESHAPE,
             "conv2d_head_out: x channel stride/offset");
  RD_REQUIRE(!conv3_body_small(cin, (flags & RD_SCALE_FOLDED) != 0), RD_ESHAPE, "conv2d_head_out: cin %d (the packed image of a conv with <= 16 input channels is not this launch form's)", cin);
  const bool m16 = (flags & RD_MFMA16) != 0;
  RD_REQUIRE(!m16 || ((flags & RD_SCALE_FOLDED) && conv3_mfma16_ok(cin, 128, 1)), RD_ESHAPE,
             "conv2d_head_out: RD_MFMA16 (weights of rd_pack_conv3x3_m16_host) is not a launch form for cin %d at width %d (rd_conv3x3_mfma16_ok)", cin, W);
  allow_conv_lds();
  Conv3Args h;
  memset(&h, 0, sizeof(h));
  h.hw = (const unsigned char*)head_w_packed; h.hb = head_bias; h.ho = out; h.ho_bs = out_batch_stride; h.ho_off = n_off; h.hn = nout;
  return launch_conv3(x, x_cstride, x_coff, w_packed, scale, shift, nullptr, 0, 0, nullptr, 128, 0, B, H, W, cin, 128, flags & ~RD_MFMA16, 1,
                      (hipStream_t)stream, 0, &h, dtype, nullptr, nullptr, m16 ? C3_BODY_M16 : 0);
}

int rd_deconv2d_bn_act(const void* x, int x_cstride, int x_coff, const void* w_packed_phase, const float* scale,
                       const float* shift, const void* residual, int r_cstride, int r_coff, void* y, int y_cstride,
                       int y_coff, int B, int H, int Win, int cin, int cout, int kh, int kw, int stride_w, int pad_w,
                       int phase, int flags, int dtype, void* stream) {
  RD_REQUIRE(x && w_packed_phase && y, RD_EINVAL, "deconv2d: null pointer");
  RD_REQUIRE(kh == 3, RD_ESHAPE, "deconv2d: kernel height %d (only 3, pad 1, stride 1)", kh);
  RD_REQUIRE(stride_w >= 1 && phase >= 0 && phase < stride_w, RD_EINVAL, "deconv2d: phase %d of stride %d", phase, stride_w);
  RD_REQUIRE(y_coff >= 0 && y_coff + cout <= y_cstride, RD_ESHAPE, "deconv2d: y channels exceed stride");
  const int Wout = (Win - 1) * stride_w - 2 * pad_w + kw;
  RD_REQUIRE(Wout > phase, RD_ESHAPE, "deconv2d: empty phase");
  const int Wq = (Wout - phase + stride_w - 1) / stride_w;
  TapList tl = deconv_taps_sorted(kh, kw, stride_w, pad_w, phase);
  RD_REQUIRE(tl.n >= 1 && tl.n <= 9, RD_ESHAPE, "deconv2d: %d taps per phase unsupported", tl.n);
  allow_conv_lds();
  if (deconv_embeds_3x3(tl)) {
    const int ts = deconv_tap_set(tl);
    if (!ts) tl = conv_taps(3, 3);
    if (is_h16(dtype) && Wout == stride_w * Win && (cout == 64 || cout == 128) &&
        conv3_has_form(dtype, (flags & RD_SCALE_FOLDED) != 0)) {
      const bf16_t* r = (const bf16_t*)residual;
      return launch_conv3(x, x_cstride, x_coff, w_packed_phase, scale, shift, r, r_cstride * stride_w,
                          r_coff + phase * r_cstride, y, y_cstride * stride_w, y_coff + phase * y_cstride, B, H, Win, cin,
                          cout, flags, 1, (hipStream_t)stream, ts, nullptr, dtype);
    }
  }
  RD_REQUIRE(!(flags & RD_SCALE_FOLDED), RD_ESHAPE, "deconv2d: RD_SCALE_FOLDED needs the persistent 3x3 kernel (bf16, cout 64/128, "
             "taps inside the 3x3 window, Wout == stride_w * Win)");
  return launch_conv(tl, x, x_cstride, x_coff, w_packed_phase, scale, shift, residual, r_cstride, r_coff, y,
                     y_cstride, y_coff, B, H, Win, Wq, Wout, cin, cout, 1, stride_w, phase, flags, dtype,
                     (hipStream_t)stream);
}

int rd_deconv2d_all_phases_ok(int kh, int kw, int stride_w, int pad_w, int cout, int dtype) {
  if (!is_h16(dtype) || kh != 3 || stride_w < 2 || stride_w > 8 || !conv3_phases_eligible(cout, RD_SCALE_FOLDED)) return 0;
  if (kw - 2 * pad_w != stride_w) return 0;
  for (int p = 0; p < stride_w; ++p)
    if (!deconv_tap_set(deconv_taps_sorted(kh, kw, stride_w, pad_w, p))) return 0;
  return 1;
}
int rd_deconv2d_bn_act_all(const void* x, int x_cstride, int x_coff, const void* w_packed_all, long w_phase_bytes,
                           const float* shift, const void* residual, int r_cstride, int r_coff, void* y, int y_cstride,
                           int y_coff, int B, int H, int Win, int cin, int cout, int kh, int kw, int stride_w, int pad_w,
                           int flags, int dtype, void* stream) {
  RD_REQUIRE(x && w_packed_all && y, RD_EINVAL, "deconv2d_all: null pointer");
  RD_REQUIRE(is_h16(dtype), RD_EINVAL, "deconv2d_all: dtype %d (RD_BF16 or RD_F16)", dtype);
  RD_REQUIRE(flags & RD_SCALE_FOLDED, RD_EINVAL, "deconv2d_all: needs RD_SCALE_FOLDED weights (rd_pack_deconv_weight_folded_host)");
  RD_REQUIRE(!((flags & RD_ADD) && !residual), RD_EINVAL, "deconv2d_all: RD_ADD without residual");
  RD_REQUIRE(B > 0 && H > 0 && Win > 0 && cin > 0, RD_ESHAPE, "deconv2d_all: shape");
  RD_REQUIRE(y_coff >= 0 && y_coff + cout <= y_cstride, RD_ESHAPE, "deconv2d_all: y channels exceed stride");
  RD_REQUIRE(x_cstride % 8 == 0 && x_coff % 8 == 0 && x_coff + cin_slots(cin, RD_BF16) * 8 <= x_cstride, RD_ESHAPE, "deconv2d_all: x channel stride/offset");
  RD_REQUIRE(rd_deconv2d_all_phases_ok(kh, kw, stride_w, pad_w, cout, dtype), RD_ESHAPE,
             "deconv2d_all: kernel (%d,%d) stride %d pad %d cout %d is not a set of two-column 3x2 phases (use rd_deconv2d_bn_act per phase)",
             kh, kw, stride_w, pad_w, cout);
  RD_REQUIRE(w_phase_bytes >= (long)conv_packed_bytes(6, cin, cout, RD_BF16) && w_phase_bytes % 16 == 0, RD_EINVAL, "deconv2d_all: w_phase_bytes");
  allow_conv_lds();
  Conv3Phases ph;
  ph.nph = stride_w; ph.ts_mask = 0; ph.y_pc = y_cstride; ph.r_pc = r_cstride; ph.w_pb = w_phase_bytes;
  for (int p = 0; p < stride_w; ++p)
    if (deconv_tap_set(deconv_taps_sorted(kh, kw, stride_w, pad_w, p)) == 2) ph.ts_mask |= 1 << p;
  return launch_conv3(x, x_cstride, x_coff, w_packed_all, nullptr, shift, residual, r_cstride * stride_w, r_coff, y, y_cstride * stride_w,
                      y_coff, B, H, Win, cin, cout, flags, 1, (hipStream_t)stream, 3, nullptr, dtype, &ph);
}

int rd_deconv2d_phase_pairs_ok(int kh, int kw, int stride_w, int pad_w, int cout, int dtype) {
  if (!rd_deconv2d_all_phases_ok(kh, kw, stride_w, pad_w, cout, dtype) || cout != 64 || stride_w % 2) return 0;
  if (!rd_deconv2d_all_phases_ok(kh, kw, stride_w, pad_w, 128, dtype)) return 0;
  for (int p = 0; p < stride_w; p += 2)
    if (deconv_tap_set(deconv_taps_sorted(kh, kw, stride_w, pad_w, p)) != deconv_tap_set(deconv_taps_sorted(kh, kw, stride_w, pad_w, p + 1))) return 0;
  return 1;
}
int rd_pack_deconv_phase_pair_host(const void* phase_a, const void* phase_b, int cin, int dtype, void* out) {
  RD_REQUIRE(phase_a && phase_b && out, RD_EINVAL, "pack_deconv_pair: null pointer");
  RD_REQUIRE(is_h16(dtype) && cin > 0, RD_EINVAL, "pack_deconv_pair: dtype %d / cin %d", dtype, cin);
  const size_t body = conv_packed_body_bytes(6, cin, 64, RD_BF16), blocks = body / 2048;
  for (size_t i = 0; i < blocks; ++i) {
    memcpy((unsigned char*)out + i * 4096, (const unsigned char*)phase_a + i * 2048, 2048);
    memcpy((unsigned char*)out + i * 4096 + 2048, (const unsigned char*)phase_b + i * 2048, 2048);
  }
  memset((unsigned char*)out + 2 * body, 0, 2 * RD_CONV_TAIL);
  return RD_OK;
}
int rd_deconv2d_bn_act_pairs(const void* x, int x_cstride, int x_coff, const void* w_packed_pairs, long w_pair_bytes,
                             const float* shift2, const void* residual, int r_cstride, int r_coff, void* y, int y_cstride,
                             int y_coff, int B, int H, int Win, int cin, int cout, int kh, int kw, int stride_w, int pad_w,
                             int flags, int dtype, void* stream) {
  RD_REQUIRE(x && w_packed_pairs && y && shift2, RD_EINVAL, "deconv2d_pairs: null pointer");
  RD_REQUIRE(is_h16(dtype), RD_EINVAL, "deconv2d_pairs: dtype %d (RD_BF16 or RD_F16)", dtype);
  RD_REQUIRE(flags & RD_SCALE_FOLDED, RD_EINVAL, "deconv2d_pairs: needs RD_SCALE_FOLDED weights (rd_pack_deconv_weight_folded_host)");
  RD_REQUIRE(!((flags & RD_ADD) && !residual), RD_EINVAL, "deconv2d_pairs: RD_ADD without residual");
  RD_REQUIRE(B > 0 && H > 0 && Win > 0 && cin > 0, RD_ESHAPE, "deconv2d_pairs: shape");
  RD_REQUIRE(x_cstride % 8 == 0 && x_coff % 8 == 0 && x_coff + cin_slots(cin, RD_BF16) * 8 <= x_cstride, RD_ESHAPE, "deconv2d_pairs: x channel stride/offset");
  RD_REQUIRE(rd_deconv2d_phase_pairs_ok(kh, kw, stride_w, pad_w, cout, dtype), RD_ESHAPE,
             "deconv2d_pairs: kernel (%d,%d) stride %d pad %d cout %d has no phase pairs (use rd_deconv2d_bn_act_all)", kh, kw, stride_w, pad_w, cout);
  RD_REQUIRE(y_cstride == cout && y_coff == 0 && (!residual || (r_cstride == cout && r_coff == 0)), RD_ESHAPE,
             "deconv2d_pairs: the output / residual must be dense %d-channel tensors (two phases are one 128-channel write)", cout);
  RD_REQUIRE(w_pair_bytes >= (long)conv_packed_bytes(6, cin, 2 * cout, RD_BF16) && w_pair_bytes % 16 == 0, RD_EINVAL, "deconv2d_pairs: w_pair_bytes");
  allow_conv_lds();
  Conv3Phases ph;
  ph.nph = stride_w / 2; ph.ts_mask = 0; ph.y_pc = 2 * cout; ph.r_pc = 2 * cout; ph.w_pb = w_pair_bytes;
  for (int p = 0; p < stride_w; p += 2)
    if (deconv_tap_set(deconv_taps_sorted(kh, kw, stride_w, pad_w, p)) == 2) ph.ts_mask |= 1 << (p / 2);
  return launch_conv3(x, x_cstride, x_coff, w_packed_pairs, nullptr, shift2, residual, r_cstride * stride_w, r_coff, y, y_cstride * stride_w,
                      y_coff, B, H, Win, cin, 2 * cout, flags, 1, (hipStream_t)stream, 3, nullptr, dtype, &ph);
}

int rd_head_out(const void* x, int x_cstride, int x_coff, const float* w, const float* bias, float* out,
                long out_batch_stride, long n_off, int B, int H, int W, int cin, int nout, int dtype, void* stream) {
  RD_REQUIRE(x && w && bias && out, RD_EINVAL, "head_out: null pointer");
  RD_REQUIRE(cin % 8 == 0 && cin <= 128 && cin > 0, RD_ESHAPE, "head_out: cin %d (multiple of 8, <= 128)", cin);
  RD_REQUIRE(nout == 1 || nout == 7 || nout == 8, RD_ESHAPE, "head_out: nout %d not in {1,7,8}", nout);
  RD_REQUIRE(dtype == RD_F32 || is_h16(dtype), RD_EINVAL, "head_out: dtype");
  hipStream_t st = (hipStream_t)stream;
  const long HW = (long)H * W;
  dim3 grid((unsigned)std::min<long>((HW + 31) / 32, 4096), B);
  ProfScope ps(RD_PROF_HEAD_OUT, st);
  if (is_h16(dtype) && nout > 1 && cin % 16 == 0 && x_cstride % 8 == 0 && x_coff % 8 == 0) {
    dim3 g2((unsigned)std::min<long>((HW + 127) / 128, 2048), B);
#define RD_HOM(NO, DT_) hipLaunchKernelGGL((head_out_mfma_kernel<NO, DT_>), g2, dim3(256), 0, st, (const bf16_t*)x, x_cstride, x_coff, w, bias, out, out_batch_stride, n_off, HW, cin)
    if (dtype == RD_F16) { if (nout == 7) RD_HOM(7, RD_F16); else RD_HOM(8, RD_F16); }
    else { if (nout == 7) RD_HOM(7, RD_BF16); else RD_HOM(8, RD_BF16); }
#undef RD_HOM
    return check_launch("head_out");
  }
#define RD_HO(DT, NO) hipLaunchKernelGGL((head_out_kernel<DT, NO>), grid, dim3(256), 0, st, x, x_cstride, x_coff, w, bias, out, out_batch_stride, n_off, HW, cin)
  if (dtype == RD_BF16) { if (nout == 1) RD_HO(RD_BF16, 1); else if (nout == 7) RD_HO(RD_BF16, 7); else RD_HO(RD_BF16, 8); }
  else if (dtype == RD_F16) { if (nout == 1) RD_HO(RD_F16, 1); else if (nout == 7) RD_HO(RD_F16, 7); else RD_HO(RD_F16, 8); }
  else { if (nout == 1) RD_HO(RD_F32, 1); else if (nout == 7) RD_HO(RD_F32, 7); else RD_HO(RD_F32, 8); }
#undef RD_HO
  return check_launch("head_out");
}

size_t rd_meta_packed_bytes(int dtype) { return meta_layout(dtype).total; }
int rd_pack_meta_host(const float* w0, const float* b0, const float* w1, const float* b1, const float* s1,
                      const float* t1, const float* agg, const float* s2, const float* t2, int dtype, void* out) {
  RD_REQUIRE(w0 && b0 && w1 && b1 && s1 && t1 && agg && s2 && t2 && out, RD_EINVAL, "pack_meta: null pointer");
  RD_REQUIRE(dtype == RD_F32 || is_h16(dtype), RD_EINVAL, "pack_meta: dtype");
  pack_meta(w0, b0, w1, b1, s1, t1, agg, s2, t2, dtype, out);
  return RD_OK;
}
int rd_meta_kernel_fwd(const void* data, int d_cstride, int d_coff, const float* coord_nchw, const void* packed,
                       void* y, int y_cstride, int y_coff, int B, int H, int W, int dtype, void* stream) {
  RD_REQUIRE(data && coord_nchw && packed && y, RD_EINVAL, "meta_kernel: null pointer");
  RD_REQUIRE(B > 0 && H > 0 && W > 0, RD_ESHAPE, "meta_kernel: empty shape");
  RD_REQUIRE(dtype == RD_F32 || is_h16(dtype), RD_EINVAL, "meta_kernel: dtype");
  const int ch = ch_per_slot(dtype);
  RD_REQUIRE(d_cstride % ch == 0 && d_coff % ch == 0 && y_cstride % ch == 0 && y_coff % ch == 0, RD_ESHAPE,
             "meta_kernel: channel strides/offsets must be 16-byte multiples");
  RD_REQUIRE(d_coff + 64 <= d_cstride && y_coff + 64 <= y_cstride, RD_ESHAPE, "meta_kernel: needs 64 channels");
  return launch_meta(data, d_cstride, d_coff, coord_nchw, packed, y, y_cstride, y_coff, B, H, W, dtype, (hipStream_t)stream);
}

size_t rd_sorted_foreground_workspace_bytes(long N, long k) { (void)k; return (sort_ws_bytes(N) + 256 + 255) & ~(size_t)255; }
int rd_sorted_foreground(const float* cls_score, const float* bbox_delta, const float* pc, const float* mask, int B,
                         long N, long k, int D, int apply_sigmoid, float* out_score, float* out_delta, float* out_pc,
                         int* out_idx, void* ws, size_t ws_bytes, void* stream) {
  RD_REQUIRE(cls_score && bbox_delta && pc && out_score && out_delta && out_pc && ws, RD_EINVAL, "sorted_foreground: null pointer");
  RD_REQUIRE(B > 0 && N > 0 && k > 0 && D > 0, RD_ESHAPE, "sorted_foreground: empty shape");
  RD_REQUIRE(N >= k, RD_ESHAPE, "sorted_foreground: N (%ld) < num_fgs (%ld)", N, k);
  RD_REQUIRE(N < (1L << 31), RD_ESHAPE, "sorted_foreground: N too large");
  RD_REQUIRE(ws_bytes >= rd_sorted_foreground_workspace_bytes(N, k), RD_EWORKSPACE, "sorted_foreground: workspace %zu < %zu",
             ws_bytes, rd_sorted_foreground_workspace_bytes(N, k));
  hipStream_t st = (hipStream_t)stream;
  void* wsa = (void*)(((uintptr_t)ws + 255) & ~(uintptr_t)255);
  SortWs s = sort_ws_carve(wsa, N);
  ProfScope ps(RD_PROF_SORT, st);
  const size_t per = rd_sorted_foreground_workspace_bytes(N, k);
  const bool wide = ws_bytes >= per * (size_t)B;
  const long stride = wide ? (long)(per / 4) : 0;
  const int nb = wide ? B : 1;
  for (int b0 = 0; b0 < B; b0 += nb) {
    hipLaunchKernelGGL(sort_keygen_kernel, dim3((unsigned)((N + 255) / 256), nb), dim3(256), 0, st, cls_score + (size_t)b0 * N,
                       mask ? mask + (size_t)b0 * N : nullptr, N, apply_sigmoid, s.keysA, s.idxA, stride);
    unsigned *rk, *ri;
    int rc = radix_topk_pairs(s, N, k, st, nb, stride, &rk, &ri);
    if (rc != RD_OK) return rc;
    hipLaunchKernelGGL(sort_gather_kernel, dim3((unsigned)((k + 255) / 256), nb), dim3(256), 0, st, rk, ri, k, D,
                       bbox_delta + (size_t)b0 * N * D, pc + (size_t)b0 * N * 3, out_score + (size_t)b0 * k,
                       out_delta + (size_t)b0 * k * D, out_pc + (size_t)b0 * k * 3, out_idx ? out_idx + (size_t)b0 * k : nullptr,
                       stride, N);
  }
  return check_launch("sorted_foreground");
}

int rd_decode3d_bbox(const float* bbox_delta, const float* pc, float* out, int B, long N, int box_type, int is_bin,
                     void* stream) {
  RD_REQUIRE(bbox_delta && pc && out, RD_EINVAL, "decode3d: null pointer");
  RD_REQUIRE(B > 0 && N > 0, RD_ESHAPE, "decode3d: empty shape");
  RD_REQUIRE((is_bin && box_type == 7) || (!is_bin && box_type == 8), RD_ESHAPE,
             "decode3d: box_type %d with is_bin=%d (8 for regular, 7 for bin)", box_type, is_bin);
  hipStream_t st = (hipStream_t)stream;
  const long n = (long)B * N;
  ProfScope ps(RD_PROF_DECODE, st);
  hipLaunchKernelGGL(decode3d_kernel, dim3((unsigned)((n + 255) / 256)), dim3(256), 0, st, bbox_delta, pc, out, n, box_type, is_bin);
  return check_launch("decode3d");
}

size_t rd_score_filter_workspace_bytes(long n) { return (size_t)((n + 255) / 256 + 8) * 4 + 256; }
int rd_score_filter_dets_batched(const float* scores, long scores_bstride, const float* boxes10, long boxes_bstride,
                                 long n, float min_score, float* dets, long dets_bstride, int* d_count, void* ws,
                                 size_t ws_bytes, int B, void* stream) {
  RD_REQUIRE(scores && boxes10 && dets && d_count && ws, RD_EINVAL, "score_filter: null pointer");
  RD_REQUIRE(n > 0 && B > 0, RD_ESHAPE, "score_filter: empty input");
  const size_t per = rd_score_filter_workspace_bytes(n);
  RD_REQUIRE(ws_bytes >= per * (size_t)B, RD_EWORKSPACE, "score_filter: workspace %zu < %zu", ws_bytes, per * (size_t)B);
  hipStream_t st = (hipStream_t)stream;
  int* blk = (int*)(((uintptr_t)ws + 255) & ~(uintptr_t)255);
  const int nblk = (int)((n + 255) / 256);
  const long blk_bs = nblk + 8;
  ProfScope ps(RD_PROF_WNMS, st);
  hipLaunchKernelGGL(filter_count_kernel, dim3(nblk, B), dim3(256), 0, st, scores, n, min_score, blk, scores_bstride, blk_bs);
  hipLaunchKernelGGL(filter_scan_kernel, dim3(B), dim3(256), 0, st, blk, nblk, d_count, blk_bs);
  hipLaunchKernelGGL(filter_scatter_kernel, dim3(nblk, B), dim3(256), 0, st, scores, boxes10, n, min_score, blk, dets,
                     scores_bstride, boxes_bstride, blk_bs, dets_bstride);
  return check_launch("score_filter");
}
int rd_score_filter_dets(const float* scores, const float* boxes10, long n, float min_score, float* dets, int* d_count,
                         void* ws, size_t ws_bytes, void* stream) {
  return rd_score_filter_dets_batched(scores, 0, boxes10, 0, n, min_score, dets, 0, d_count, ws, ws_bytes, 1, stream);
}

size_t rd_wnms_workspace_bytes(int Kcap) { return Kcap > 0 ? wnms_ws_bytes(Kcap) : 0; }
int rd_wnms_4c_batched(const float* dets, long dets_bstride, int Kcap, const int* d_count, const int* order,
                       long order_bstride, int tie_order, float thresh, float thresh_vote, int is3d, int hash_scale,
                       float* out_dets, long out_bstride, int* keep, long keep_bstride, int* d_nkeep, void* ws,
                       size_t ws_bytes, int B, void* stream) {
  RD_REQUIRE(dets && out_dets && keep && d_nkeep && ws, RD_EINVAL, "wnms_4c: null pointer");
  RD_REQUIRE(Kcap > 0 && Kcap <= RD_WNMS_MAX_K, RD_ESHAPE, "wnms_4c: Kcap %d not in [1, %d]", Kcap, RD_WNMS_MAX_K);
  RD_REQUIRE(B > 0, RD_ESHAPE, "wnms_4c: batch %d", B);
  const int diag = tie_order & ~0xff;
  tie_order &= 0xff;
  RD_REQUIRE(tie_order == RD_TIE_STABLE || tie_order == RD_TIE_REFERENCE, RD_EINVAL, "wnms_4c: tie_order %d", tie_order);
  RD_REQUIRE(!(diag & ~(RD_WNMS_DIAG_NO_SKIP | (0xff << 16) | (0x7f << 24))), RD_EINVAL, "wnms_4c: unknown diagnostic bits 0x%x", diag);
  const size_t per = rd_wnms_workspace_bytes(Kcap);
  RD_REQUIRE(ws_bytes >= per * (size_t)B, RD_EWORKSPACE, "wnms_4c: workspace %zu < %zu", ws_bytes, per * (size_t)B);
  RD_REQUIRE(order || B == 1 || tie_order == RD_TIE_REFERENCE, RD_EINVAL,
             "wnms_4c: the batched call needs an explicit processing order or RD_TIE_REFERENCE");
  hipStream_t st = (hipStream_t)stream;
  static std::atomic<unsigned long long> seen_lds{0};
  once_per_device(seen_lds, [] {
    allow_big_lds(wnms_tie_order_kernel); allow_big_lds(wnms_scan_kernel); allow_big_lds(wnms_scan4_kernel); allow_big_lds(wnms_merge_kernel);
  });
  WnmsWs w = wnms_ws_carve(ws, Kcap);
  ProfScope ps(RD_PROF_WNMS, st);
  WnmsBatch bs;
  bs.dets = dets_bstride; bs.order = order_bstride; bs.prep = (long)(per / 4); bs.words = (long)(per / 8);
  bs.ints = (long)(per / 4); bs.keep = keep_bstride; bs.out = out_bstride;
  const int* ord = order;
  if (!ord && tie_order == RD_TIE_REFERENCE) {
    const size_t lds = TIE_STACK_BYTES + (Kcap <= TIE_LDS_K ? (size_t)Kcap * 8 + 3 * ((size_t)Kcap / 32 + 2) * 4 : 0);
    hipLaunchKernelGGL(wnms_tie_order_kernel, dim3(1, 1, B), dim3(256), lds, st, dets, Kcap, d_count, w.order, bs, (long)(per / 4),
                       w.scratch);
    ord = w.order;
    bs.order = (long)(per / 4);
  } else if (!ord) {
    void* swa = (void*)(((uintptr_t)w.sort_ws + 255) & ~(uintptr_t)255);
    SortWs s = sort_ws_carve(swa, Kcap);
// ... 900 lines not shown
```

rangedet_amd/lib.py:

```python
import ctypes
import os

import numpy as np

RD_OK, RD_EINVAL, RD_ESHAPE, RD_EWORKSPACE, RD_EHIP = 0, -1, -2, -3, -4
RD_F32, RD_BF16, RD_F16 = 0, 1, 2
H16 = (RD_BF16, RD_F16)
RD_RELU_PRE, RD_ADD, RD_RELU_POST, RD_SCALE_FOLDED, RD_MFMA16 = 1, 2, 4, 8, 16
RD_WNMS_MAX_K = 65536
RD_WNMS_DIAG_NO_SKIP = 0x100


def RD_WNMS_DIAG_TILE_W(n):
    return (n & 0xff) << 16


def RD_WNMS_DIAG_MERGE_LDS(n):
    return (n & 0x7f) << 24

RD_TIE_STABLE, RD_TIE_REFERENCE = 0, 1
PROF_KINDS = {"conv": 0, "meta": 1, "head_out": 2, "sort": 3, "decode": 4, "wnms": 5, "layout": 6, "conv3": 7, "block": 8}

_HERE = os.path.dirname(os.path.abspath(__file__))
DEFAULT_PATH = os.environ.get("RANGEDET_HIP_LIB") or os.path.join(_HERE, "librangedet_hip.so")

c_int, c_long, c_float, c_size_t, c_void_p = ctypes.c_int, ctypes.c_long, ctypes.c_float, ctypes.c_size_t, ctypes.c_void_p

SIGNATURES = {
    "rd_version": (c_int, []),
    "rd_last_error_string": (ctypes.c_char_p, []),
    "rd_nchw_to_nhwc": (c_int, [c_void_p, c_void_p, c_int, c_int, c_int, c_int, c_int, c_int, c_int, c_int, c_void_p]),
    "rd_nhwc_to_nchw": (c_int, [c_void_p, c_void_p, c_int, c_int, c_int, c_int, c_int, c_int, c_int, c_void_p]),
    "rd_copy_rows": (c_int, [c_void_p, c_long, c_void_p, c_long, c_long, c_long, c_int, c_void_p]),
    "rd_conv_packed_bytes": (c_size_t, [c_int, c_int, c_int, c_int]),
    "rd_pack_conv_weight_host": (c_int, [c_void_p, c_int, c_int, c_int, c_int, c_int, c_void_p]),
    "rd_deconv_phase_taps": (c_int, [c_int, c_int, c_int, c_int, c_int]),
    "rd_pack_deconv_weight_host": (c_int, [c_void_p, c_int, c_int, c_int, c_int, c_int, c_int, c_int, c_int, c_void_p]),
    "rd_pack_deconv_weight_folded_host": (c_int, [c_void_p, c_void_p, c_int, c_int, c_int, c_int, c_int, c_int, c_int, c_int, c_void_p]),
    "rd_conv2d_bn_act": (c_int, [c_void_p, c_int, c_int, c_void_p, c_void_p, c_void_p, c_void_p, c_int, c_int, c_void_p,
                                 c_int, c_int, c_int, c_int, c_int, c_int, c_int, c_int, c_int, c_int, c_int, c_int, c_void_p]),
    "rd_conv3x3_ex_packed_bytes": (c_size_t, [c_int, c_int, c_int, c_int]),
    "rd_pack_conv3x3_ex_host": (c_int, [c_void_p, c_void_p, c_int, c_int, c_int, c_int, c_int, c_void_p]),
    "rd_pack_conv3x3_m16_host": (c_int, [c_void_p, c_void_p, c_int, c_int, c_int, c_void_p]),
    "rd_conv3x3_mfma16_ok": (c_int, [c_int, c_int, c_int, c_int, c_int]),
    "rd_conv1x1_sc_packed_bytes": (c_size_t, [c_int, c_int]),
    "rd_pack_conv1x1_sc_host": (c_int, [c_void_p, c_void_p, c_int, c_int, c_int, c_void_p]),
    "rd_conv3x3_bn_act_ex": (c_int, [c_void_p, c_int, c_int, c_void_p, c_void_p, c_void_p, c_void_p, c_int, c_int, c_void_p, c_int,
                                     c_int, c_int, c_void_p, c_void_p, c_int, c_int, c_int, c_int, c_int, c_int, c_int, c_int,
                                     c_int, c_int, c_void_p]),
    "rd_deconv2d_bn_act": (c_int, [c_void_p, c_int, c_int, c_void_p, c_void_p, c_void_p, c_void_p, c_int, c_int, c_void_p,
                                   c_int, c_int, c_int, c_int, c_int, c_int, c_int, c_int, c_int, c_int, c_int, c_int,
                                   c_int, c_int, c_void_p]),
    "rd_conv3x3_cat_packed_bytes": (c_size_t, [c_int, c_int, c_int]),
    "rd_pack_conv3x3_cat_host": (c_int, [c_void_p, c_void_p, c_int, c_int, c_int, c_int, c_void_p]),
    "rd_conv3x3_bn_act_cat": (c_int, [c_void_p, c_int, c_int, c_int, c_void_p, c_int, c_int, c_int, c_void_p, c_void_p, c_void_p, c_int, c_int,
                                      c_int, c_int, c_int, c_int, c_int, c_int, c_void_p]),
    "rd_deconv2d_all_phases_ok": (c_int, [c_int, c_int, c_int, c_int, c_int, c_int]),
    "rd_deconv2d_bn_act_all": (c_int, [c_void_p, c_int, c_int, c_void_p, c_long, c_void_p, c_void_p, c_int, c_int, c_void_p,
                                       c_int, c_int, c_int, c_int, c_int, c_int, c_int, c_int, c_int, c_int, c_int, c_int,
                                       c_int, c_void_p]),
    "rd_deconv2d_phase_pairs_ok": (c_int, [c_int, c_int, c_int, c_int, c_int, c_int]),
    "rd_pack_deconv_phase_pair_host": (c_int, [c_void_p, c_void_p, c_int, c_int, c_void_p]),
    "rd_deconv2d_bn_act_pairs": (c_int, [c_void_p, c_int, c_int, c_void_p, c_long, c_void_p, c_void_p, c_int, c_int, c_void_p,
                                         c_int, c_int, c_int, c_int, c_int, c_int, c_int, c_int, c_int, c_int, c_int, c_int,
                                         c_int, c_void_p]),
    "rd_block64_packed_bytes": (c_size_t, [c_int]),
    "rd_pack_block64_host": (c_int, [c_void_p, c_void_p, c_void_p, c_void_p, c_int, c_int, c_void_p]),
    "rd_pack_block64_m16_host": (c_int, [c_void_p, c_void_p, c_void_p, c_void_p, c_int, c_void_p]),
    "rd_pack_conv1x1_sc_m16_host": (c_int, [c_void_p, c_void_p, c_int, c_void_p]),
    "rd_block64_m16_bn_act": (c_int, [c_void_p, c_int, c_int, c_void_p, c_void_p, c_void_p, c_void_p, c_void_p, c_int, c_int, c_int, c_int,
                                      c_int, c_int, c_void_p]),
    "rd_block64_bn_act": (c_int, [c_void_p, c_int, c_int, c_int, c_void_p, c_void_p, c_void_p, c_void_p, c_void_p, c_int, c_int, c_int, c_int,
                                  c_int, c_int, c_void_p]),
    "rd_head_packed_bytes": (c_size_t, []),
    "rd_head_m16_packed_bytes": (c_size_t, []),
    "rd_pack_head_weight_host": (c_int, [c_void_p, c_int, c_int, c_int, c_void_p]),
    "rd_pack_head_weight_m16_host": (c_int, [c_void_p, c_int, c_int, c_int, c_void_p]),
    "rd_conv2d_bn_act_head_out": (c_int, [c_void_p, c_int, c_int, c_void_p, c_void_p, c_void_p, c_int, c_int, c_int, c_int, c_int,
                                          c_void_p, c_void_p, c_void_p, c_long, c_long, c_int, c_int, c_void_p]),
    "rd_head_out": (c_int, [c_void_p, c_int, c_int, c_void_p, c_void_p, c_void_p, c_long, c_long, c_int, c_int, c_int,
                            c_int, c_int, c_int, c_void_p]),
    "rd_meta_packed_bytes": (c_size_t, [c_int]),
    "rd_pack_meta_host": (c_int, [c_void_p] * 9 + [c_int, c_void_p]),
    "rd_meta_kernel_fwd": (c_int, [c_void_p, c_int, c_int, c_void_p, c_void_p, c_void_p, c_int, c_int, c_int, c_int,
                                   c_int, c_int, c_void_p]),
    "rd_meta_bwd_packed_bytes": (c_size_t, [c_int]),
    "rd_pack_meta_bwd_host": (c_int, [c_void_p] * 9 + [c_int, c_void_p]),
    "rd_meta_kernel_bwd_data": (c_int, [c_void_p, c_int, c_int, c_void_p, c_int, c_int, c_void_p, c_void_p, c_void_p, c_int, c_int, c_void_p, c_int,
                                        c_int, c_int, c_int, c_int, c_int, c_void_p]),
    "rd_meta_kernel_bwd_workspace_bytes": (c_size_t, [c_int, c_int, c_int, c_int]),
    "rd_meta_kernel_bwd_params": (c_int, [c_void_p, c_int, c_int, c_void_p, c_int, c_int, c_void_p, c_void_p] + [c_void_p] * 7
                                  + [c_int, c_int, c_int, c_int, c_int, c_void_p, c_size_t, c_void_p]),
    "rd_sorted_foreground_workspace_bytes": (c_size_t, [c_long, c_long]),
    "rd_sorted_foreground": (c_int, [c_void_p, c_void_p, c_void_p, c_void_p, c_int, c_long, c_long, c_int, c_int,
                                     c_void_p, c_void_p, c_void_p, c_void_p, c_void_p, c_size_t, c_void_p]),
    "rd_decode3d_bbox": (c_int, [c_void_p, c_void_p, c_void_p, c_int, c_long, c_int, c_int, c_void_p]),
    "rd_score_filter_workspace_bytes": (c_size_t, [c_long]),
    "rd_score_filter_dets": (c_int, [c_void_p, c_void_p, c_long, c_float, c_void_p, c_void_p, c_void_p, c_size_t, c_void_p]),
    "rd_score_filter_dets_batched": (c_int, [c_void_p, c_long, c_void_p, c_long, c_long, c_float, c_void_p, c_long, c_void_p,
                                             c_void_p, c_size_t, c_int, c_void_p]),
    "rd_wnms_workspace_bytes": (c_size_t, [c_int]),
    "rd_wnms_4c_batched": (c_int, [c_void_p, c_long, c_int, c_void_p, c_void_p, c_long, c_int, c_float, c_float, c_int, c_int,
                                   c_void_p, c_long, c_void_p, c_long, c_void_p, c_void_p, c_size_t, c_int, c_void_p]),
    "rd_dets12_to_8_batched": (c_int, [c_void_p, c_long, c_int, c_void_p, c_void_p, c_long, c_int, c_void_p]),
    "rd_wnms_4c": (c_int, [c_void_p, c_int, c_void_p, c_void_p, c_int, c_float, c_float, c_int, c_int, c_void_p, c_void_p,
                           c_void_p, c_void_p, c_size_t, c_void_p]),
    "rd_single_overlap": (c_int, [c_void_p, c_void_p, c_long, c_int, c_void_p, c_void_p]),
    "rd_wnms_order_host": (c_int, [c_void_p, c_int, c_void_p]),
    "rd_edge_atan2f": (c_int, [c_void_p, c_void_p, c_long, c_void_p, c_void_p]),
    "rd_wnms_pair_skippable": (c_int, [c_void_p, c_void_p, c_long, c_void_p, c_void_p]),
    "rd_dets12_to_8": (c_int, [c_void_p, c_int, c_void_p, c_void_p, c_void_p]),
    "rd_rotated_iou_8pt": (c_int, [c_void_p, c_void_p, c_void_p, c_long, c_long, c_void_p]),
    "rd_batch_rotated_iou": (c_int, [c_void_p, c_int, c_void_p, c_void_p, c_void_p, c_int, c_long, c_int, c_void_p]),
    "rd_batch_rotated_iou_3d": (c_int, [c_void_p, c_int, c_void_p, c_void_p, c_void_p, c_int, c_long, c_int, c_void_p]),
    "rd_rotated_iou_7": (c_int, [c_void_p, c_void_p, c_void_p, c_long, c_long, c_void_p]),
    "rd_batch_max_iou": (c_int, [c_void_p, c_int, c_void_p, c_void_p, c_long, c_int, c_void_p]),
    "rd_gather_keep_scores": (c_int, [c_void_p, c_long, c_int, c_void_p, c_int, c_void_p, c_int, c_void_p]),
    "rd_nms3d_workspace_bytes": (c_size_t, [c_long, c_int]),
    "rd_nms3d": (c_int, [c_void_p, c_int, c_long, c_float, c_int, c_int, c_void_p, c_void_p, c_void_p, c_size_t, c_void_p]),
    "rd_assign3d_v2": (c_int, [c_void_p] * 6 + [c_long, c_int] + [c_float] * 7 + [c_void_p, c_void_p]),
    "rd_get_point_num_workspace_bytes": (c_size_t, []),
    "rd_get_point_num": (c_int, [c_void_p, c_long, c_void_p, c_void_p, c_size_t, c_void_p]),
    "rd_input_transform": (c_int, [c_void_p, c_void_p, c_void_p, c_void_p, c_int, c_int, c_int, c_int, c_int] + [c_void_p] * 8 + [c_void_p]),
    "rd_train_transform_workspace_bytes": (c_size_t, [c_int]),
    "rd_train_transform": (c_int, [c_void_p] * 9 + [c_int, c_float, c_float, c_void_p, c_int, c_int, c_int, c_int, c_int,
                                   c_void_p, c_void_p, c_size_t, c_void_p]),
    "rd_range_image_workspace_bytes": (c_size_t, [c_int, c_int, c_int]),
    "rd_range_image_from_points": (c_int, [c_void_p, c_void_p, c_int, c_void_p, c_void_p, c_int, c_int, c_void_p, c_void_p, c_void_p,
                                           c_void_p, c_size_t, c_void_p]),
    "rd_rpn_loss_workspace_bytes": (c_size_t, [c_int, c_long]),
    "rd_rpn_loss": (c_int, [c_void_p, c_long, c_void_p, c_long, c_void_p, c_void_p, c_int] + [c_void_p] * 4 + [c_int, c_int, c_int]
                    + [c_void_p] * 9 + [c_size_t, c_void_p]),
    "rd_relu_affine_bwd": (c_int, [c_void_p, c_int, c_int, c_void_p, c_int, c_int, c_void_p, c_void_p, c_int, c_int, c_int, c_int, c_int,
                                   c_int, c_int, c_void_p]),
    "rd_conv3x3_bwd_weight_workspace_bytes": (c_size_t, [c_int, c_int, c_int, c_int, c_int, c_int]),
    "rd_conv3x3_bwd_weight": (c_int, [c_void_p, c_int, c_int, c_void_p, c_int, c_int, c_void_p, c_int, c_int, c_int, c_int, c_int, c_int,
                                      c_int, c_void_p, c_size_t, c_void_p]),
    "rd_conv3x3_bwd_weight_ex_workspace_bytes": (c_size_t, [c_int, c_int, c_int, c_int, c_int, c_int, c_int]),
    "rd_conv3x3_bwd_weight_ex": (c_int, [c_void_p, c_int, c_int, c_void_p, c_int, c_int, c_void_p, c_int, c_int, c_int, c_int, c_int, c_int,
                                         c_int, c_int, c_void_p, c_size_t, c_void_p]),
    "rd_conv1x1_bwd_weight_workspace_bytes": (c_size_t, [c_int, c_int, c_int, c_int, c_int, c_int]),
    "rd_conv1x1_bwd_weight": (c_int, [c_void_p, c_int, c_int, c_void_p, c_int, c_int, c_void_p, c_int, c_int, c_int, c_int, c_int, c_int,
                                      c_int, c_void_p, c_size_t, c_void_p]),
    "rd_deconv_bwd_weight_workspace_bytes": (c_size_t, [c_int] * 9),
    "rd_deconv_bwd_weight": (c_int, [c_void_p, c_int, c_int, c_void_p, c_int, c_int, c_void_p, c_int, c_int, c_int, c_int, c_int, c_int,
                                     c_int, c_int, c_int, c_int, c_void_p, c_size_t, c_void_p]),
    "rd_pack_deconv_data_grad_host": (c_int, [c_void_p, c_int, c_int, c_int, c_int, c_int, c_int, c_void_p]),
    "rd_pack_deconv_dev": (c_int, [c_void_p, c_int, c_int, c_int, c_int, c_int, c_int, c_long, c_int, c_void_p, c_void_p]),
    "rd_affine_relu_add": (c_int, [c_void_p, c_int, c_int, c_void_p, c_void_p, c_void_p, c_int, c_int, c_void_p, c_int, c_int, c_int, c_int,
                                   c_int, c_int, c_int, c_void_p]),
    "rd_head_out_bwd_workspace_bytes": (c_size_t, [c_int, c_int, c_int, c_int, c_int]),
    "rd_head_out_bwd": (c_int, [c_void_p, c_long, c_long, c_void_p, c_int, c_int, c_void_p, c_int, c_void_p, c_void_p, c_int, c_int,
                                c_void_p, c_void_p, c_int, c_int, c_int, c_int, c_int, c_int, c_void_p, c_size_t, c_void_p]),
    "rd_bn_stats_workspace_bytes": (c_size_t, [c_int, c_int, c_int, c_int, c_int]),
    "rd_bn_stats": (c_int, [c_void_p, c_int, c_int, c_void_p, c_void_p, c_int, c_int, c_int, c_int, c_int, c_int, c_void_p, c_size_t,
                            c_void_p]),
    "rd_bn_fold": (c_int, [c_void_p] * 4 + [c_float, c_float, c_long, c_int] + [c_void_p] * 5 + [c_int, c_void_p]),
    "rd_affine_relu": (c_int, [c_void_p, c_int, c_int, c_void_p, c_void_p, c_int, c_void_p, c_int, c_int, c_int, c_int, c_int, c_int, c_int,
                               c_void_p]),
    "rd_bn_relu_bwd_workspace_bytes": (c_size_t, [c_int, c_int, c_int, c_int, c_int]),
    "rd_bn_relu_bwd": (c_int, [c_void_p, c_int, c_int, c_void_p, c_int, c_int] + [c_void_p] * 5 + [c_int, c_void_p, c_int, c_int, c_void_p,
                               c_void_p, c_int, c_int, c_int, c_int, c_int, c_int, c_void_p, c_size_t, c_void_p]),
    "rd_affine_add_relu": (c_int, [c_void_p, c_int, c_int, c_void_p, c_void_p, c_void_p, c_int, c_int, c_void_p, c_void_p, c_int, c_void_p,
                                   c_int, c_int, c_int, c_int, c_int, c_int, c_int, c_void_p]),
    "rd_bn_add_relu_bwd_workspace_bytes": (c_size_t, [c_int, c_int, c_int, c_int, c_int, c_int]),
    "rd_bn_add_relu_bwd": (c_int, [c_void_p, c_int, c_int, c_void_p, c_int, c_int, c_void_p, c_int, c_int] + [c_void_p] * 10
                           + [c_void_p, c_int, c_int, c_void_p, c_int, c_int] + [c_void_p] * 4
                           + [c_int, c_int, c_int, c_int, c_int, c_int, c_void_p, c_size_t, c_void_p]),
    "rd_sgd_table_bytes": (c_size_t, [c_void_p, c_int]),
    "rd_sgd_table_host": (c_int, [c_void_p, c_int, c_int, c_void_p]),
    "rd_sgd_mom_update": (c_int, [c_void_p, c_void_p, c_float, c_float, c_float, c_float, c_float, c_void_p]),
    "rd_pack_conv3x3_dev": (c_int, [c_void_p, c_void_p, c_int, c_int, c_int, c_int, c_void_p, c_void_p]),
    "rd_prof_enable": (c_int, [c_int]),
    "rd_prof_reset": (c_int, []),
    "rd_prof_get": (c_int, [c_int, ctypes.POINTER(ctypes.c_double), ctypes.POINTER(c_long)]),
}


class SgdTensor(ctypes.Structure):
    _fields_ = [("weight", c_void_p), ("grad", c_void_p), ("mom", c_void_p), ("n", c_long), ("lr_mult", c_float), ("wd_mult", c_float),
                ("cout", c_int), ("cin", c_int), ("pack_fwd", c_void_p), ("pack_bwd", c_void_p), ("fold_scale", c_void_p),
                ("stride_w", c_int)]


class RangeDetError(RuntimeError):
    def __init__(self, code, msg):
        super().__init__("librangedet_hip error %d: %s" % (code, msg))
        self.code = code


def ptr(x):
    if x is None:
        return None
    if isinstance(x, int):
        return x
    if isinstance(x, np.ndarray):
        return x.ctypes.data
    if hasattr(x, "data_ptr"):
        return x.data_ptr()
    raise TypeError("cannot take the address of %r" % type(x))


class Lib:
    def __init__(self, path=DEFAULT_PATH):
        if not os.path.exists(path):
            raise RuntimeError(
                "%s not found: the HIP extension is not built (run `python -m rangedet_amd.build`). "
                "There is no CPU fallback." % path)
        self.path = path
        if os.path.basename(path).startswith("librangedet_hip"):
            try:
                import torch
            except ImportError:
                pass
        self.cdll = ctypes.CDLL(path)
        for name, (res, args) in SIGNATURES.items():
            fn = getattr(self.cdll, name)
            fn.restype = res
            fn.argtypes = args
        self.rd_last_error_string = self.cdll.rd_last_error_string

    def call(self, name, *args):
        rc = getattr(self.cdll, name)(*args)
        if rc < 0:
            raise RangeDetError(rc, self.cdll.rd_last_error_string().decode())
        return rc

    def raw(self, name):
        return getattr(self.cdll, name)

    def pack_conv_weight(self, w_oihw, dtype):
        w = np.ascontiguousarray(w_oihw, dtype=np.float32)
        cout, cin, kh, kw = w.shape
        out = np.zeros(self.cdll.rd_conv_packed_bytes(kh * kw, cin, cout, dtype), dtype=np.uint8)
        self.call("rd_pack_conv_weight_host", w.ctypes.data, cout, cin, kh, kw, dtype, out.ctypes.data)
        return out

    def pack_conv3x3_ex(self, w_oihw, stride_w, x_cstride, fold_scale=None, dtype=RD_BF16):
        w = np.ascontiguousarray(w_oihw, dtype=np.float32)
        cout, cin = w.shape[:2]
        assert w.shape[2:] == (3, 3)
        fs = None if fold_scale is None else np.ascontiguousarray(fold_scale, dtype=np.float32)
        out = np.zeros(self.cdll.rd_conv3x3_ex_packed_bytes(cin, cout, stride_w, x_cstride), dtype=np.uint8)
        self.call("rd_pack_conv3x3_ex_host", w.ctypes.data, None if fs is None else fs.ctypes.data, cout, cin, stride_w,
                  x_cstride, dtype, out.ctypes.data)
        return out

    def pack_conv3x3_m16(self, w_oihw, fold_scale, dtype=RD_BF16):
        w = np.ascontiguousarray(w_oihw, dtype=np.float32)
        cout, cin = w.shape[:2]
        assert w.shape[2:] == (3, 3)
        fs = np.ascontiguousarray(fold_scale, dtype=np.float32)
        out = np.zeros(self.cdll.rd_conv3x3_ex_packed_bytes(cin, cout, 1, cin), dtype=np.uint8)
        self.call("rd_pack_conv3x3_m16_host", w.ctypes.data, fs.ctypes.data, cout, cin, dtype, out.ctypes.data)
        return out

    def pack_conv3x3_cat(self, w_oihw, cin1, cin2, fold_scale=None, dtype=RD_BF16):
        w = np.ascontiguousarray(w_oihw, dtype=np.float32)
        cout = w.shape[0]
        assert w.shape[1:] == (cin1 + cin2, 3, 3)
        fs = None if fold_scale is None else np.ascontiguousarray(fold_scale, dtype=np.float32)
        out = np.zeros(self.cdll.rd_conv3x3_cat_packed_bytes(cin1, cin2, cout), dtype=np.uint8)
        self.call("rd_pack_conv3x3_cat_host", w.ctypes.data, None if fs is None else fs.ctypes.data, cout, cin1, cin2, dtype, out.ctypes.data)
        return out

    def pack_conv1x1_sc(self, w_oi, fold_scale=None, dtype=RD_BF16):
        w = np.ascontiguousarray(w_oi, dtype=np.float32).reshape(w_oi.shape[0], -1)
        cout, cin = w.shape
        fs = None if fold_scale is None else np.ascontiguousarray(fold_scale, dtype=np.float32)
        out = np.zeros(self.cdll.rd_conv1x1_sc_packed_bytes(cin, cout), dtype=np.uint8)
        self.call("rd_pack_conv1x1_sc_host", w.ctypes.data, None if fs is None else fs.ctypes.data, cout, cin, dtype, out.ctypes.data)
        return out

    def pack_block64(self, w1_oihw, scale1, w2_oihw, scale2, dtype=RD_BF16, m16=False):
        w1, w2 = (np.ascontiguousarray(w, dtype=np.float32) for w in (w1_oihw, w2_oihw))
        s1, s2 = (np.ascontiguousarray(v, dtype=np.float32) for v in (scale1, scale2))
        cin = w1.shape[1]
        assert w1.shape == (64, cin, 3, 3) and w2.shape == (64, 64, 3, 3) and s1.shape == (64,) and s2.shape == (64,)
        out = np.zeros(self.cdll.rd_block64_packed_bytes(cin), dtype=np.uint8)
        if m16:
            assert cin == 64
            self.call("rd_pack_block64_m16_host", w1.ctypes.data, s1.ctypes.data, w2.ctypes.data, s2.ctypes.data, dtype, out.ctypes.data)
        else:
            self.call("rd_pack_block64_host", w1.ctypes.data, s1.ctypes.data, w2.ctypes.data, s2.ctypes.data, cin, dtype, out.ctypes.data)
        return out

    def pack_conv1x1_sc_m16(self, w_oi, fold_scale, dtype=RD_BF16):
        w = np.ascontiguousarray(w_oi, dtype=np.float32).reshape(64, 64)
        fs = np.ascontiguousarray(fold_scale, dtype=np.float32)
        out = np.zeros(self.cdll.rd_conv1x1_sc_packed_bytes(64, 64), dtype=np.uint8)
        self.call("rd_pack_conv1x1_sc_m16_host", w.ctypes.data, fs.ctypes.data, dtype, out.ctypes.data)
        return out

    def pack_deconv_weight(self, w_iohw, stride_w, pad_w, phase, dtype, fold_scale=None):
        w = np.ascontiguousarray(w_iohw, dtype=np.float32)
        cin, cout, kh, kw = w.shape
        nt = self.cdll.rd_deconv_phase_taps(kh, kw, stride_w, pad_w, phase)
        if nt < 0:
            raise RangeDetError(nt, "deconv phase taps")
        out = np.zeros(self.cdll.rd_conv_packed_bytes(nt, cin, cout, dtype), dtype=np.uint8)
        fs = None if fold_scale is None else np.ascontiguousarray(fold_scale, dtype=np.float32)
        self.call("rd_pack_deconv_weight_folded_host", w.ctypes.data, None if fs is None else fs.ctypes.data, cin, cout, kh, kw,
                  stride_w, pad_w, phase, dtype, out.ctypes.data)
        return out

    def pack_deconv_data_grad(self, w_iohw, stride_w, pad_w, dtype):
        w = np.ascontiguousarray(w_iohw, dtype=np.float32)
        cin, cout, kh, kw = w.shape
        assert kh == 3
        out = np.zeros(self.cdll.rd_conv3x3_ex_packed_bytes(stride_w * cout, cin, 1, stride_w * cout), dtype=np.uint8)
        self.call("rd_pack_deconv_data_grad_host", w.ctypes.data, cin, cout, kw, stride_w, pad_w, dtype, out.ctypes.data)
        return out

    def pack_deconv_phase_pair(self, img_a, img_b, cin, dtype):
        assert img_a.nbytes == img_b.nbytes
        out = np.empty(2 * img_a.nbytes, np.uint8)
        a, b = np.ascontiguousarray(img_a), np.ascontiguousarray(img_b)
        self.call("rd_pack_deconv_phase_pair_host", a.ctypes.data, b.ctypes.data, cin, dtype, out.ctypes.data)
        return out

    def pack_head_weight(self, w, dtype=RD_BF16, m16=False):
        w = np.ascontiguousarray(w, dtype=np.float32)
        out = np.zeros(self.cdll.rd_head_m16_packed_bytes() if m16 else self.cdll.rd_head_packed_bytes(), dtype=np.uint8)
        self.call("rd_pack_head_weight_m16_host" if m16 else "rd_pack_head_weight_host", w.ctypes.data, w.shape[0], w.shape[1], dtype, out.ctypes.data)
        return out

    def pack_meta(self, w0, b0, w1, b1, s1, t1, agg, s2, t2, dtype):
        arrs = [np.ascontiguousarray(a, dtype=np.float32) for a in (w0, b0, w1, b1, s1, t1, agg, s2, t2)]
        assert arrs[0].shape == (32, 3) and arrs[2].shape == (64, 32) and arrs[6].shape == (64, 576)
        out = np.zeros(self.cdll.rd_meta_packed_bytes(dtype), dtype=np.uint8)
        self.call("rd_pack_meta_host", *[a.ctypes.data for a in arrs], dtype, out.ctypes.data)
        return out

    def pack_meta_bwd(self, w0, b0, w1, b1, s1, t1, agg, s2, t2, dtype):
        arrs = [np.ascontiguousarray(a, dtype=np.float32) for a in (w0, b0, w1, b1, s1, t1, agg, s2, t2)]
        assert arrs[0].shape == (32, 3) and arrs[2].shape == (64, 32) and arrs[6].shape == (64, 576)
        out = np.zeros(max(self.cdll.rd_meta_bwd_packed_bytes(dtype), 16), dtype=np.uint8)
        self.call("rd_pack_meta_bwd_host", *[a.ctypes.data for a in arrs], dtype, out.ctypes.data)
        return out

    def sgd_table(self, tensors, dtype=RD_BF16):
        arr = (SgdTensor * len(tensors))(*tensors)
        nbytes = self.cdll.rd_sgd_table_bytes(ctypes.addressof(arr), len(tensors))
        out = np.zeros(max(nbytes, 8), dtype=np.uint8)
        self.call("rd_sgd_table_host", ctypes.addressof(arr), len(tensors), dtype, out.ctypes.data)
        return out

    def wnms_order_host(self, dets):
        d = np.ascontiguousarray(dets, dtype=np.float32).reshape(-1, 12)
        order = np.empty(d.shape[0], dtype=np.int32)
        self.call("rd_wnms_order_host", d.ctypes.data, d.shape[0], order.ctypes.data)
        return order

    def prof(self):
        out = {}
        ms, n = ctypes.c_double(), c_long()
        for k, v in PROF_KINDS.items():
            self.call("rd_prof_get", v, ctypes.byref(ms), ctypes.byref(n))
            out[k] = (ms.value, n.value)
        return out


_LIB = None


def get_lib():
    global _LIB
    if _LIB is None:
        _LIB = Lib(DEFAULT_PATH)
    return _LIB
```

rangedet_amd/lower.py:

```python
from dataclasses import dataclass, field

from . import devswitch
from .lib import H16, RD_ADD, RD_BF16, RD_F16, RD_F32, RD_RELU_POST, RD_RELU_PRE


@dataclass
class TRef:
    buf: int
    C: int
    H: int
    W: int
    cs: int
    co: int = 0
    cmap: tuple = None
    tail: "TRef" = None


@dataclass
class FlatRef:
    buf: int
    shape: tuple


@dataclass
class Plan:
    dtype: int
    batch: int
    steps: list = field(default_factory=list)
    buffers: dict = field(default_factory=dict)
    outputs: list = field(default_factory=list)
    input_vars: dict = field(default_factory=dict)
    num_classes: int = 1


def step_refs(step):
    def walk(path, v):
        if isinstance(v, (TRef, FlatRef)):
            yield path, v
            if isinstance(v, TRef) and v.tail is not None:
                yield from walk(path + ".tail", v.tail)
        elif isinstance(v, (dict, list, tuple)):
            for k, x in (v.items() if isinstance(v, dict) else enumerate(v)):
                yield from walk(path + "." + str(k) if path else str(k), x)
    return walk("", step)


def conv_steps(steps):
    for st in steps:
        if st["kind"] == "block":
            yield st["a"], 0.5
            yield st["b"], 0.5
        elif st["kind"] == "conv":
            yield st, 1
        elif st["kind"] == "deconv":
            yield st, 1 if st.get("one_launch") else st["stride_w"]


def _strip_cast(s):
    while s.op == "cast":
        s = s.inputs[0]
    return s


def _is(s, op, **attrs):
    return s.op == op and all(s.attrs.get(k) == v for k, v in attrs.items())


class Lowering:
    def __init__(self, group, input_shapes, dtype, batch):
        assert dtype in (RD_F32, RD_BF16, RD_F16)
        self.dtype = dtype
        self.h16 = dtype in H16
        self.esz = 2 if self.h16 else 4
        self.gran = 16 if self.h16 else 8
        self.B = batch
        self.shapes = dict(input_shapes)
        self.plan = Plan(dtype=dtype, batch=batch)
        self.memo = {}
        self.nbuf = 0
        self.consumers = {}
        self._count_consumers(group)
        for out in group.inputs:
            self.plan.outputs.append(self.emit_value(out))
        self._fuse_head_out()
        self._fuse_blocks()
        self._mark_mfma16()

    def _mark_mfma16(self):
        if not self.h16 or devswitch.get("RD_NO_MFMA16"):
            return
        for st in self.plan.steps:
            if st["kind"] == "block" and st["a"]["cin"] == 64 and not devswitch.get("RD_NO_MFMA16_BLOCK"):
                st["m16"] = True
            if st["kind"] == "conv" and tuple(st["k"]) == (3, 3) and st["cout"] == 128 and st["stride_w"] == 1 and st.get("ex") and \
                    st.get("fold") and not st.get("sc") and st.get("x2") is None and not st.get("s2view"):
                cin = len(st["cmap"]) if st.get("cmap") else st["cin"]
                if cin % 32 == 0 and cin >= 32:
                    st["m16"] = True

    def _fuse_blocks(self):
        if not self.h16 or devswitch.get("RD_NO_FUSE_BLOCK"):
            return
        steps = self.plan.steps
        uses = self._uses()

        def plain64(st, first=False):
            if not (st["kind"] == "conv" and tuple(st["k"]) == (3, 3) and st["stride_w"] == 1 and st["cout"] == 64 and st.get("ex") and
                    st.get("fold") and not st.get("head") and st.get("x2") is None and st["x"].tail is None):
                return False
            if first and st["x"].cs - st["x"].co == 16 and st["x"].C <= 16:
                return True
            return st["cin"] == 64 and st["x"].C == 64 and not st.get("cmap")

        out, i = [], 0
        while i < len(steps):
            a = steps[i]
            b = steps[i + 1] if i + 1 < len(steps) else None
            ok = b is not None and plain64(a, first=True) and plain64(b) and a["flags"] == RD_RELU_POST and a["res"] is None and not a.get("sc") and \
                b["flags"] == (RD_ADD | RD_RELU_POST) and b["x"] == a["out"] and a["out"].co == 0 and a["out"].cs == 64 and \
                sorted(uses.get(a["out"].buf, [])) == [(i, "out"), (i + 1, "x")] and b["out"].buf != a["x"].buf
            if ok:
                small = a["x"].C <= 16
                if b.get("sc"):
                    ok = b["res"] is None and b["sc_x"] == a["x"] and (small or (b["sc"]["cin"] == 64 and not b["sc"].get("cmap")))
                else:
                    ok = b["res"] == a["x"] and not small
            if ok:
                blk = dict(kind="block", name=a["name"] + " + " + b["name"], a=a, b=b, x=a["x"], out=b["out"])
                a["in_block"] = b["in_block"] = True
                self.plan.buffers.pop(a["out"].buf, None)
                out.append(blk)
                i += 2
            else:
                out.append(a)
                i += 1
        self.plan.steps = out

    def _fuse_head_out(self):
        if not self.h16:
            return
        steps = self.plan.steps
        uses = self._uses()
        drop = set()
        for i, st in enumerate(steps):
            if st["kind"] != "head_out" or st["nout"] > 8:
                continue
            x = st["x"]
            refs = uses.get(x.buf, [])
            prod = [j for j, key in refs if key == "out"]
            if len({j for j, _ in refs}) != 2 or len(prod) != 1 or x.co != 0 or x.C != 128:
                continue
            c = steps[prod[0]]
            if not (c["kind"] == "conv" and tuple(c["k"]) == (3, 3) and c["cout"] == 128 and c["stride_w"] == 1 and
                    c["flags"] == RD_RELU_POST and c.get("res") is None and c["out"] == x and c.get("x2") is None):
                continue
            c["head"] = dict(name=st["name"], rows=st["rows"], nout=st["nout"], out=st["out"], n_off=st["n_off"], N=st["N"])
            c["head_out"] = st["out"]
            drop.add(i)
        self.plan.steps = [st for i, st in enumerate(steps) if i not in drop]

    def _uses(self):
        uses = {}
        for i, st in enumerate(self.plan.steps):
            for path, v in step_refs(st):
                uses.setdefault(v.buf, []).append((i, path))
        for path, v in step_refs(self.plan.outputs):
            uses.setdefault(v.buf, []).append((-1, "output." + path))
        return uses

    def _count_consumers(self, root):
        seen = set()

        def walk(s):
            for i in s.inputs:
                self.consumers[i.uid] = self.consumers.get(i.uid, 0) + 1
                if i.uid not in seen:
                    seen.add(i.uid)
                    walk(i)
        walk(root)

    def new_buf(self, nbytes, persistent=False, zero=False):
        self.nbuf += 1
        self.plan.buffers[self.nbuf] = dict(nbytes=int(nbytes), persistent=persistent, zero=zero)
        return self.nbuf

    def new_act(self, C, H, W, persistent=False, zero=False, cs=None):
        cs = cs or -(-C // self.gran) * self.gran
        buf = self.new_buf(self.B * H * W * cs * self.esz, persistent or cs != C, zero or cs != C)
        return TRef(buf, C, H, W, cs, 0)

    def step(self, kind, **kw):
        kw["kind"] = kind
        for key, v in kw.items():
            if isinstance(v, TRef) and v.tail is not None and not (kind == "conv" and key == "x" and kw.get("x2") is v.tail and tuple(kw.get("k", ())) == (3, 3)):
                raise NotImplementedError("%s step %r: operand %r is a virtual concat [%d channels | %d more from another tensor]; only a "
                                          "3x3 stride-1 convolution can read it (set RD_CONCAT_BUFFER=1 for a materialised concat)" %
                                          (kind, kw.get("name", ""), key, v.C, v.tail.C))
        self.plan.steps.append(kw)

    def want_input(self, name):
        if name not in self.shapes:
            raise KeyError("lowering needs the shape of input variable %r" % name)
        self.plan.input_vars[name] = tuple(self.shapes[name])
        return tuple(self.shapes[name])

    def emit_act(self, s, dest=None):
        s = _strip_cast(s)
        key = s.uid
        if s.op == "var" and dest is not None:
            return self._emit_act(s, dest)
        if key in self.memo:
            if dest is not None:
                raise NotImplementedError("%s is needed both stand-alone and inside a concat buffer" % s.name)
            return self.memo[key]
        r = self._emit_act(s, dest)
        if dest is None:
            self.memo[key] = r
        return r

    def _out(self, C, H, W, dest):
        if dest is None:
            return self.new_act(C, H, W)
        buf, cs, co = dest
        return TRef(buf, C, H, W, cs, co)

    def _emit_act(self, s, dest):
        if s.op == "var":
            C, H, W = self.want_input(s.name)
            out = self._out(C, H, W, dest) if dest else self.new_act(C, H, W, persistent=True)
            pad = (out.cs - out.co - C) if dest is None else 0
            self.step("nchw_in", name=s.name, out=out, zero_pad=pad)
            return out
        if _is(s, "Activation", act_type="relu"):
            inner = s.inputs[0]
            if inner.op == "elemwise_add":
                return self._residual_block(inner, dest)
            if inner.op == "BatchNorm" and inner.inputs[0].op == "Convolution":
                conv = inner.inputs[0]
                meta = self._match_meta(conv)
                if meta is not None:
                    return self._emit_meta(meta, conv, inner, dest)
                return self._conv_bn(conv, inner, RD_RELU_POST, None, dest)
        if s.op == "BatchNorm" and s.inputs[0].op == "Convolution":
            return self._conv_bn(s.inputs[0], s, 0, None, dest)
        if s.op == "elemwise_add":
            return self._agg_add(s, dest)
        if _is(s, "concat", dim=1):
            return self._concat(s, dest)
        raise NotImplementedError("no HIP lowering for %r (op %s) as an activation" % (s.name, s.op))

    def _conv_geom(self, conv, x):
# ... 353 lines not shown
```

rangedet_amd/runtime.py:

```python
from collections import namedtuple

import numpy as np

from . import lib as rdlib
from .lower import step_refs


class TorchAllocator:

    def __init__(self, device="cuda:0", stream=None):
        import torch
        if not torch.cuda.is_available():
            raise RuntimeError("rangedet_amd needs a ROCm GPU (torch.cuda.is_available() is False); there is no CPU fallback")
        self.torch = torch
        self.device = torch.device(device)
        torch.cuda.set_device(self.device)
        self._stream = stream

    @property
    def stream(self):
        st = self._stream or self.torch.cuda.current_stream(self.device)
        return st.cuda_stream

    def alloc(self, nbytes, zero=False):
# ... 83 lines not shown
        self.plan = plan
        self.lib = lib or rdlib.get_lib()
        self.alloc = alloc or TorchAllocator()
        self.dtype = plan.dtype
        self.B = plan.batch
        self._phys = {}
        self._held = []
        self._sorted_idx = []
        self._assign_buffers(reuse_buffers)
        self._bound = [self._bind(st, params) for st in plan.steps]

    def _assign_buffers(self, reuse):
        plan = self.plan
        last_use, first_def = {}, {}
        for i, st in enumerate(plan.steps):
            for _, v in step_refs(st):
                if v.buf in plan.buffers:
                    last_use[v.buf] = i
                    first_def.setdefault(v.buf, i)
        for _, v in step_refs(plan.outputs):
            last_use[v.buf] = len(plan.steps) + 1
        free = {}
        release = {}
        for b, i in last_use.items():
            release.setdefault(i, []).append(b)
        order = sorted(plan.buffers, key=lambda b: first_def.get(b, 0))
        by_def = {}
        for b in order:
            by_def.setdefault(first_def.get(b, 0), []).append(b)
        for i in range(len(plan.steps) + 2):
            for b in by_def.get(i, []):
                info = plan.buffers[b]
                if reuse and not info["persistent"] and free.get(info["nbytes"]):
                    self._phys[b] = free[info["nbytes"]].pop()
                else:
                    self._phys[b] = self.alloc.alloc(info["nbytes"], zero=info["zero"])
            for b in release.get(i, []):
                info = plan.buffers[b]
                if reuse and not info["persistent"] and last_use[b] <= len(plan.steps):
                    free.setdefault(info["nbytes"], []).append(self._phys[b])
        self.device_bytes = sum(int(t.numel()) if hasattr(t, "numel") else len(t) for t in {id(v): v for v in self._phys.values()}.values())

    def p(self, ref):
        return self.alloc.ptr(self._phys[ref.buf])

    def _up(self, arr):
        if arr is None:
            return None
        self._held.append(self.alloc.upload(arr))
        return self.alloc.ptr(self._held[-1])

    def _ws(self, nbytes):
        self._held.append(self.alloc.alloc(nbytes))
        return self._held[-1]

    def _at(self, ref):
        return (self.p(ref), ref.cs, ref.co) if ref is not None else (None, 0, 0)

    def _bind(self, st, P):
        binder = self._BINDERS.get(st["kind"])
        if binder is None:
            raise RuntimeError("unknown plan step %r" % st["kind"])
        calls = []
        for name, *args in binder(self, st, P):
            want = len(rdlib.SIGNATURES[name][1]) - 1
            if len(args) != want:
                raise TypeError("step %r (%s): %s bound with %d arguments before the stream, the library takes %d" %
                                (st.get("name", ""), st["kind"], name, len(args), want))
            calls.append((name, tuple(args), tuple((j, a) for j, a in enumerate(args) if isinstance(a, Input))))
        return calls

    def _bind_nchw_in(self, st, P):
        o, B = st["out"], self.B
        yield ("rd_nchw_to_nhwc", Input(st["name"], (B, o.C, o.H, o.W), True), self.p(o), B, o.C, o.H, o.W, o.cs, o.co, st["zero_pad"], self.dtype)

    def _bind_block(self, st, P):
        L, dt = self.lib, self.dtype
        ca, cb, x, o = st["a"], st["b"], st["x"], st["out"]
        w1, w2 = (np.asarray(P[c["name"] + "_weight"], np.float32) for c in (ca, cb))
        w1 = cmap_cols(w1, ca.get("cmap"))
        (s1, t1), (s2, t2) = bn_affine(P, ca["bn"], ca["eps"]), bn_affine(P, cb["bn"], cb["eps"])
        cin = w1.shape[1]
        m16 = bool(st.get("m16")) and cin == 64
        sc_w = None
        if cb.get("sc"):
            sc = cb["sc"]
            wsc = cmap_cols(np.asarray(P[sc["name"] + "_weight"], np.float32).reshape(64, -1), sc.get("cmap"))
            ss, ts = bn_affine(P, sc["bn"], sc["eps"])
            sc_w = L.pack_conv1x1_sc_m16(wsc, ss, dtype=dt) if m16 else L.pack_conv1x1_sc(wsc, fold_scale=ss, dtype=dt)
            t2 = (t2.astype(np.float64) + ts).astype(np.float32)
        tail = (self._up(L.pack_block64(w1, s1, w2, s2, dtype=dt, m16=m16)), self._up(t1), self._up(t2), self._up(sc_w),
                *self._at(o), self.B, x.H, x.W, dt)
        if m16:
            yield ("rd_block64_m16_bn_act", *self._at(x), *tail)
        else:
            yield ("rd_block64_bn_act", *self._at(x), cin, *tail)

    def _conv_form(self, st, cin):
        head, sc, cat = bool(st.get("head")), bool(st.get("sc")), st.get("x2") is not None
        fold = bool(st.get("ex") and st.get("fold"))
        if head + sc + cat > 1 or ((head or sc) and not st.get("ex")):
            raise NotImplementedError("conv step %r: no launch form for head=%s sc=%s x2=%s ex=%s" % (st["name"], head, sc, cat, st.get("ex")))
        if sc or cat:
            return ("ex_sc" if sc else "cat"), False
        m16 = fold and bool(st.get("m16")) and \
            self.lib.raw("rd_conv3x3_mfma16_ok")(cin, st["cout"], 1, st["x"].W, 1 if head else 0) == 1
        return ("head" if head else "ex_fold" if fold else "ex" if st.get("ex") else "plain"), m16

    def _bind_conv(self, st, P):
        L, dt, B = self.lib, self.dtype, self.B
        x, o, r, cout, sw = st["x"], st.get("out"), st.get("res"), st["cout"], st["stride_w"]
        w = cmap_cols(pad_rows(np.asarray(P[st["name"] + "_weight"], np.float32), cout), st.get("cmap"))
        s, t = bn_affine(P, st["bn"], st["eps"], pad_to=cout)
        form, m16 = self._conv_form(st, w.shape[1])
        folded = form in ("cat", "ex_fold") or (form == "head" and st.get("fold"))
        flags = st["flags"] | (rdlib.RD_SCALE_FOLDED if folded else 0) | (rdlib.RD_MFMA16 if m16 else 0)
        scale = None if folded or form == "ex_sc" else self._up(s)
        if form == "plain":
            yield ("rd_conv2d_bn_act", *self._at(x), self._up(L.pack_conv_weight(w, dt)), scale, self._up(t), *self._at(r), *self._at(o),
                   B, x.H, x.W, st["cin"], cout, st["k"][0], st["k"][1], sw, flags, dt)
            return
        if form == "cat":
            x2 = st["x2"]
            yield ("rd_conv3x3_bn_act_cat", *self._at(x), x.C, *self._at(x2), x2.cs, self._up(L.pack_conv3x3_cat(w, x.C, x2.cs, fold_scale=s, dtype=dt)),
                   self._up(t), *self._at(o), B, x.H, x.W, cout, flags, dt)
            return
        wimg = self._up(L.pack_conv3x3_m16(w, s, dtype=dt) if m16 else
                        L.pack_conv3x3_ex(w, sw, x.cs, fold_scale=None if scale is not None else s, dtype=dt))
        if form == "head":
            h = st["head"]
            r0, r1 = h["rows"]
            hw = np.asarray(P[h["name"] + "_weight"], np.float32).reshape(-1, cout)[r0:r1]
            yield ("rd_conv2d_bn_act_head_out", *self._at(x), wimg, scale, self._up(t), B, x.H, x.W, st["cin"], flags,
                   self._up(L.pack_head_weight(hw, dtype=dt, m16=m16)), self._up(np.asarray(P[h["name"] + "_bias"], np.float32)[r0:r1]),
                   self.p(h["out"]), h["N"] * h["nout"], h["n_off"], h["nout"], dt)
            return
        sc_x, sc_cin, sc_w = None, 0, None
        if form == "ex_sc":
            sc, sc_x = st["sc"], st["sc_x"]
            wsc = np.asarray(P[sc["name"] + "_weight"], np.float32)
            wsc = cmap_cols(pad_rows(wsc.reshape(wsc.shape[0], -1), cout), sc.get("cmap"))
            ss, ts = bn_affine(P, sc["bn"], sc["eps"], pad_to=cout)
            sc_cin, sc_w = len(sc["cmap"]) if sc.get("cmap") else sc["cin"], self._up(L.pack_conv1x1_sc(wsc, fold_scale=ss, dtype=dt))
            t = (t.astype(np.float64) + ts).astype(np.float32)
        yield ("rd_conv3x3_bn_act_ex", *self._at(x), wimg, scale, self._up(t), *self._at(r), *self._at(sc_x), sc_cin, sc_w, *self._at(o),
               B, x.H, x.W, len(st["cmap"]) if st.get("cmap") else st["cin"], cout, sw, flags, dt)

    def _bind_deconv(self, st, P):
        L, dt = self.lib, self.dtype
        x, o, r, cout, sw, pw, (kh, kw) = st["x"], st["out"], st["res"], st["cout"], st["stride_w"], st["pad_w"], st["k"]
        w = pad_rows(np.asarray(P[st["name"] + "_weight"], np.float32), cout, axis=1)
        s, t = bn_affine(P, st["bn"], st["eps"], pad_to=cout)
        fold = bool(st.get("fold"))
        imgs = [L.pack_deconv_weight(w, sw, pw, ph, dt, fold_scale=s if fold else None) for ph in range(sw)]
        flags = st["flags"] | (rdlib.RD_SCALE_FOLDED if fold else 0)
        geom = (*self._at(r), *self._at(o), self.B, x.H, x.W, st["cin"], cout, kh, kw, sw, pw)
        dense = all(v.cs == cout and v.co == 0 for v in (o, r) if v is not None)
        all_phases = bool(st.get("one_launch")) and len({len(i) for i in imgs}) == 1 and \
            L.raw("rd_deconv2d_all_phases_ok")(kh, kw, sw, pw, cout, dt) == 1
        if all_phases and dense and L.raw("rd_deconv2d_phase_pairs_ok")(kh, kw, sw, pw, cout, dt) == 1:
            pimgs = [L.pack_deconv_phase_pair(imgs[p], imgs[p + 1], st["cin"], dt) for p in range(0, sw, 2)]
            yield ("rd_deconv2d_bn_act_pairs", *self._at(x), self._up(np.concatenate(pimgs)), len(pimgs[0]), self._up(np.concatenate([t, t])),
                   *geom, flags, dt)
        elif all_phases:
            yield ("rd_deconv2d_bn_act_all", *self._at(x), self._up(np.concatenate(imgs)), len(imgs[0]), self._up(t), *geom, flags, dt)
        else:
            scale, shift = (None if fold else self._up(s)), self._up(t)
            for ph in range(sw):
                yield ("rd_deconv2d_bn_act", *self._at(x), self._up(imgs[ph]), scale, shift, *geom, ph, flags, dt)

    def _bind_meta(self, st, P):
        x, o, B = st["x"], st["out"], self.B
        s1, t1 = bn_affine(P, st["bn1"], st["eps1"])
        s2, t2 = bn_affine(P, st["bn2"], st["eps2"])
        pk = self.lib.pack_meta(P[st["mlp0"] + "_weight"].reshape(32, 3), P[st["mlp0"] + "_bias"],
                                P[st["mlp1"] + "_weight"].reshape(64, 32), P[st["mlp1"] + "_bias"], s1, t1,
                                P[st["agg"] + "_weight"].reshape(64, 576), s2, t2, self.dtype)
        yield ("rd_meta_kernel_fwd", *self._at(x), Input(st["coord"], (B, 3, x.H, x.W), True), self._up(pk), *self._at(o), B, x.H, x.W, self.dtype)

    def _bind_head_out(self, st, P):
        x = st["x"]
        r0, r1 = st["rows"]
        w = np.asarray(P[st["name"] + "_weight"], np.float32).reshape(-1, x.C)[r0:r1]
        yield ("rd_head_out", *self._at(x), self._up(w), self._up(np.asarray(P[st["name"] + "_bias"], np.float32)[r0:r1]), self.p(st["out"]),
               st["N"] * st["nout"], st["n_off"], self.B, x.H, x.W, x.C, st["nout"], self.dtype)

    def _bind_concat_in(self, st, P):
        row = st["N"] * st["last"] * 4
        off = 0
        for name, n in st["names"]:
            yield ("rd_copy_rows", Input(name, (self.B, n), False), n * st["last"] * 4, self.p(st["out"]), row, off * st["last"] * 4,
                   n * st["last"] * 4, self.B)
            off += n

    def _bind_sorted_fg(self, st, P):
        A, B = self.alloc, self.B
        nb = self.lib.raw("rd_sorted_foreground_workspace_bytes")(st["N"], st["k"]) * B
        idx = self._ws(B * st["k"] * 4) if self.keep_sorted_idx else None
        self._sorted_idx.append((idx, st["k"]))
        yield ("rd_sorted_foreground", self.p(st["score"]), self.p(st["delta"]), self.p(st["pc"]), self.p(st["mask"]), B, st["N"], st["k"],
               st["D"], st["apply_sigmoid"], self.p(st["out_score"]), self.p(st["out_delta"]), self.p(st["out_pc"]),
               A.ptr(idx) if idx is not None else None, A.ptr(self._ws(nb)), nb)

    def _bind_decode(self, st, P):
        yield ("rd_decode3d_bbox", self.p(st["delta"]), self.p(st["pc"]), self.p(st["out"]), self.B, st["k"], st["box_type"], st["is_bin"])

    def _bind_batch_riou(self, st, P):
        three_d = st.get("iou_type", "bev") == "3d"
        yield ("rd_batch_rotated_iou_3d" if three_d else "rd_batch_rotated_iou", self.p(st["boxes"]), 10,
               Input(st["gt"], (self.B, st["n_gt"], 7 if three_d else 8), True), self.p(st["out"]), None, self.B, st["N"], st["n_gt"])

    def _bind_nms3d(self, st, P):
        nb = self.lib.raw("rd_nms3d_workspace_bytes")(st["N"], self.B)
        yield ("rd_nms3d", self.p(st["boxes"]), self.B, st["N"], st["thr"], st["max_keep"], st["normal_iou"], self.p(st["keep"]),
               self.p(st["out"]), self.alloc.ptr(self._ws(nb)), nb)

    _BINDERS = {"nchw_in": _bind_nchw_in, "block": _bind_block, "conv": _bind_conv, "deconv": _bind_deconv, "meta": _bind_meta,
                "head_out": _bind_head_out, "concat_in": _bind_concat_in, "sorted_fg": _bind_sorted_fg, "decode": _bind_decode,
                "batch_riou": _bind_batch_riou, "nms3d": _bind_nms3d}

    def forward(self, inputs, only=None, dev=None):
        A, B = self.alloc, self.B
        call, stream = self.lib.call, A.stream
        dev = {} if dev is None else dev
        for calls in (self._bound if only is None else [self._bound[only]]):
            for name, args, slots in calls:
                if slots:
                    args = list(args)
                    for j, slot in slots:
                        if slot.name not in dev:
                            dev[slot.name] = A.as_device_f32(inputs[slot.name])
                        src = dev[slot.name]
                        shape = tuple(src.shape)
                        assert (shape if slot.exact else shape[:len(slot.shape)]) == slot.shape, (slot.name, shape, slot.shape)
                        args[j] = A.ptr(src)
                call(name, *args, stream)
        if only is not None:
            return None
        outs = []
        for kind, v in self.plan.outputs:
            if kind == "flat":
                outs.append(A.view_f32(self._phys[v.buf], (B,) + tuple(v.shape)))
            elif kind == "flat_i32":
                outs.append(A.view_i32(self._phys[v.buf], (B,) + tuple(v.shape)))
            elif kind == "input":
                outs.append(inputs.get(v))
            else:
                outs.append(np.zeros(v, np.float32))
        return outs

    def read_flat(self, ref):
        self.alloc.sync()
        return np.array(self.alloc.to_numpy(self.alloc.view_f32(self._phys[ref.buf], (self.B,) + tuple(ref.shape))))

    def sorted_idx(self, which=0):
        idx, k = self._sorted_idx[which]
        self.alloc.sync()
        return np.array(self.alloc.to_numpy(self.alloc.view_i32(idx, (self.B, k))))

    def debug_tensor(self, ref):
        A, L = self.alloc, self.lib
        out = A.alloc(self.B * ref.C * ref.H * ref.W * 4)
        L.call("rd_nhwc_to_nchw", self.p(ref), A.ptr(out), self.B, ref.C, ref.H, ref.W, ref.cs, ref.co, self.dtype, A.stream)
        A.sync()
        return A.to_numpy(A.view_f32(out, (self.B, ref.C, ref.H, ref.W)))
```

Baseline: 934.5.

## Extend 16x16x32 MFMA conv body to all-phase transposed conv launches

Lets the persistent conv3 kernel's 16x16x32 MFMA form run the all-phases and phase-pair transposed-conv paths. It adds m16 weight packing for deconv phases and pairs, per-phase A-offset recomputation for the 16-lane layout, a final-chunk unit that prefetches the next phase's column, and a RELU_PRE|ADD epilogue. The lowering pass turns it on for folded one-launch deconvs with cout 64, stride 4 and cin a multiple of 32. The goal is higher matrix throughput or better LDS use in the upsampling layers, at the cost of extra template instances and register pressure.

```diff
diff --git a/include/rangedet_hip.h b/include/rangedet_hip.h
--- a/include/rangedet_hip.h
+++ b/include/rangedet_hip.h
@@ -96,6 +96,10 @@
                            const float* shift, const void* residual, int r_cstride, int r_coff, void* y, int y_cstride,
                            int y_coff, int B, int H, int Win, int cin, int cout, int kh, int kw, int stride_w, int pad_w,
                            int flags, int dtype, void* stream);
+int rd_deconv2d_mfma16_ok(int cin, int cout, int phase_pairs);
+int rd_pack_deconv_weight_m16_host(const float* w_iohw_host, const float* fold_scale_host, int cin, int cout, int kh, int kw,
+                                   int stride_w, int pad_w, int phase, int dtype, void* packed_host);
+int rd_pack_deconv_phase_pair_m16_host(const void* phase_a, const void* phase_b, int cin, int dtype, void* out);
 
 int rd_deconv2d_phase_pairs_ok(int kh, int kw, int stride_w, int pad_w, int cout, int dtype);
 int rd_pack_deconv_phase_pair_host(const void* phase_a, const void* phase_b, int cin, int dtype, void* out);
diff --git a/rangedet_amd/csrc/k_conv3.h b/rangedet_amd/csrc/k_conv3.h
--- a/rangedet_amd/csrc/k_conv3.h
+++ b/rangedet_amd/csrc/k_conv3.h
@@ -222,8 +222,8 @@
   using Cfg = C3Cfg<NCT, TILE>;
   constexpr bool WD = Cfg::WIDE;
   constexpr int FPW = Cfg::FPW, FC = Cfg::FC;
-  static_assert(!M16 || (NCT == 4 && WD && FOLD && !SC && TS == 0 && BODY == 0),
-                "16 x 16 x 32 form: cout 128 on the 8 x 32 tiles, folded scales, all nine taps");
+  static_assert(!M16 || (NCT == 4 && WD && FOLD && !SC && (TS == 0 || TS == 3) && BODY == 0),
+                "16 x 16 x 32 form: cout 128 on the 8 x 32 tiles, folded scales, all nine taps or all phases of a transposed conv");
   static_assert(BODY == 0 || (WD && FOLD && !HEAD && (TS == 0 || TS == 1)), "heterogeneous tile bodies: 8 x 32 tiles, folded scales");
   static_assert(!WD || FOLD, "8 x 32 tile: no room for the scale / shift array");
   static_assert(!HEAD || (NCT == 4 && TS == 0), "fused output conv: cout 128, all nine taps");
@@ -400,14 +400,15 @@
   };
 
   int aoff[3];
+  auto aoff16 = [&](int d, int l) {
+    const int c16 = d + (l & 15);
+    return c16 * 64 + ((((l >> 4) ^ (c16 >> 2)) & 3) << 4) + wave * RW * C3_ROWB;
+  };
 #pragma unroll
   for (int d = 0; d < 3; ++d) {
     const int c = d + m;
     aoff[d] = c * 64 + (((hi ^ (c >> 2)) & 3) << 4) + wave * RW * C3_ROWB;
-    if constexpr (M16) {
-      const int c16 = d + (lane & 15);
-      aoff[d] = c16 * 64 + ((((lane >> 4) ^ (c16 >> 2)) & 3) << 4) + wave * RW * C3_ROWB;
-    }
+    if constexpr (M16) aoff[d] = aoff16(d, lane);
   }
   const int boff = RING + lane * 16;
   auto side2 = [&](int ph) { return (a.ts_mask >> ph) & 1; };
@@ -481,7 +482,7 @@
 #pragma unroll
     for (int k = 0; k < 4; ++k) C3_RDW16(0, k, boff + rslot * SLAB)
 #pragma unroll
-    for (int k = 0; k < 4; ++k) C3_RDP16(k, aoff[K00DW] + abuf + K00DH * C3_ROWB)
+    for (int k = 0; k < 4; ++k) C3_RDP16(k, C3_AO(K00DW) + abuf + K00DH * C3_ROWB)
   } else {
 #pragma unroll
   for (int k = 0; k < NR; ++k)
@@ -532,13 +533,14 @@
   C3_STEP(21, C3_MM) C3_STEP(22, C3_MM)
   static_assert(BG <= 23, "C3_BODY_FROM1 unrolls 23 steps");
 
-#define C3_STEP16(S)                                                                                                 \
-  {                                                                                                                  \
+#define C3_STEP16(S, LASTC)                                                                                          \
+  if constexpr ((S) < BG) {                                                                                          \
     constexpr C3Step D_ = c3_step(BD, (S), TILE, R, IPW);                                                            \
     constexpr int NP_ = IPW + D_.pieces;                                                                             \
     const int bcur_ = boff + rslot * SLAB;                                                                           \
     const int rnext_ = rslot + 1 == R ? 0 : rslot + 1;                                                               \
-    const int anext_ = aoff[D_.kn.dw] + (D_.ulast ? hflip(abuf) : abuf) + D_.kn.dh * C3_ROWB;                        \
+     \
+    const int anext_ = (PH && D_.ulast && (LASTC) ? pq0 : C3_AO(D_.kn.dw)) + (D_.ulast ? hflip(abuf) : abuf) + D_.kn.dh * C3_ROWB; \
     const int bnext_ = boff + rnext_ * SLAB;                                                                         \
     const int hbuf_ = hflip(abuf);                                                                                   \
     C3_FENCE();                                                                                                      \
@@ -593,10 +595,12 @@
 #pragma unroll
         for (int cb = 0; cb < 8; ++cb) acc6[h][cb] = acc6[0][cb];
       C3_FENCE();
+#define C3_UNIT16(LASTC) C3_STEP16(0, LASTC) C3_STEP16(1, LASTC) C3_STEP16(2, LASTC) C3_STEP16(3, LASTC) C3_STEP16(4, LASTC) C3_STEP16(5, LASTC) \
+  C3_STEP16(6, LASTC) C3_STEP16(7, LASTC) C3_STEP16(8, LASTC)
 #pragma unroll 1
-      for (int c = 0; c < a.nchunk; ++c) {
-        C3_STEP16(0) C3_STEP16(1) C3_STEP16(2) C3_STEP16(3) C3_STEP16(4) C3_STEP16(5) C3_STEP16(6) C3_STEP16(7) C3_STEP16(8)
-      }
+      for (int c = PH ? 1 : 0; c < a.nchunk; ++c) { C3_UNIT16(false) }
+      if constexpr (PH) { C3_UNIT16(true) }
+#undef C3_UNIT16
     } else {
     {
       if constexpr (FOLD) {
@@ -634,8 +638,15 @@
     if constexpr (PH) {
       if (++c_ph == nph) { c_ph = 0; tile_advance(c_ct, c_rb, c_b); }
       const int sn_ = side2(c_ph), sq_ = side2(c_ph + 1 == nph ? 0 : c_ph + 1);
+      if constexpr (M16) {
+        int ol = lane;
+        asm volatile("" : "+v"(ol));
+        pcol[0] = aoff16(sn_, ol); pcol[1] = aoff16(sn_ + 1, ol);
+        pq0 = aoff16(sq_, ol);
+      } else {
       pcol[0] = sn_ ? aoff[1] : aoff[0]; pcol[1] = sn_ ? aoff[2] : aoff[1];
       pq0 = sq_ ? aoff[1] : aoff[0];
+      }
     } else
     tile_advance(c_ct, c_rb, c_b);
     const int oh0 = rb * C3_TH + RW * wave;
@@ -933,6 +944,7 @@
       static_assert(!M16 || (NPASS == 2 && JW == 2 && CW == 64), "M16 epilogue: two passes of 64 channels");
       if (a.flags == RD_RELU_POST) epilogue16(std::integral_constant<int, RD_RELU_POST>{});
       else if (a.flags == (RD_ADD | RD_RELU_POST)) epilogue16(std::integral_constant<int, RD_ADD | RD_RELU_POST>{});
+      else if (TS != 0 && a.flags == (RD_RELU_PRE | RD_ADD)) epilogue16(std::integral_constant<int, RD_RELU_PRE | RD_ADD>{});
       else epilogue16(std::integral_constant<int, -1>{});
     } else {
     if (a.flags == RD_RELU_POST) epilogue(std::integral_constant<int, RD_RELU_POST>{});
@@ -996,6 +1008,7 @@
 inline bool conv3_mfma16_ok(int cin, int cout, int stride_w) {
   return cout == 128 && stride_w == 1 && cin >= 32 && cin % 32 == 0;
 }
+inline bool conv3_mfma16_phases_ok(int cin, int cout) { return cout == 128 && cin >= 32 && cin % 32 == 0; }
 
 template <int DT>
 inline int launch_conv3_dt(const void* x, int x_cs, int x_co, const void* w, const float* scale, const float* shift,
@@ -1049,7 +1062,8 @@
   if (conv_trace_buf() && (size_t)grid * 8 <= (1u << 20)) a.trace = conv_trace_buf();
   ProfScope ps(RD_PROF_CONV3, st);
 #ifdef RD_CONV3_DEV_M16_ONLY
-  RD_REQUIRE(wide && !sc && !ph && !s2 && sw == 1 && ts == 0 && cout == 128 && DT == RD_BF16 && (!headfuse || body == C3_BODY_M16), RD_ESHAPE, "conv16_dev: plain bf16 cout-128 form only");
+  RD_REQUIRE(wide && !sc && !s2 && sw == 1 && ts == (ph ? 3 : 0) && cout == 128 && DT == RD_BF16 && (!headfuse || (body == C3_BODY_M16 && !ph)), RD_ESHAPE, "conv16_dev: plain bf16 cout-128 form only");
+  if (ph) { if (body == C3_BODY_M16) return c3_go<4, 3, false, false, true, C3_8x32, RD_BF16, 0, true>(grid, st, a); return c3_go<4, 3, false, false, true, C3_8x32, RD_BF16>(grid, st, a); }
   if (body == C3_BODY_M16 && headfuse) return c3_go<4, 0, true, false, true, C3_8x32, RD_BF16, 0, true>(grid, st, a);
   if (body == C3_BODY_M16) return c3_go<4, 0, false, false, true, C3_8x32, RD_BF16, 0, true>(grid, st, a);
   return c3_go<4, 0, false, false, true, C3_8x32, RD_BF16>(grid, st, a);
@@ -1060,6 +1074,11 @@
     RD_REQUIRE(ts == 0 || ts == 1, RD_ESHAPE, "conv3 + shortcut: tap set %d", ts);
     RD_REQUIRE(fold, RD_EINVAL, "conv3 + shortcut: the weights must carry the folded scales (RD_SCALE_FOLDED)");
   }
+  if (body == C3_BODY_M16 && ph) {
+    RD_REQUIRE(wide && !sc && !head && !s2 && ts == 3 && sw == 1 && ph->nph >= 1 && ph->nph <= 8 && conv3_mfma16_phases_ok(cin, cout), RD_ESHAPE,
+               "conv3: the 16 x 16 x 32 form of all phases per launch needs cout 128 (or a pair of 64) and cin a multiple of 32 (cin %d, cout %d)", cin, cout);
+    return c3_go<4, 3, false, false, true, C3_8x32, DT, 0, true>(grid, st, a);
+  }
   if (body == C3_BODY_M16) {
     RD_REQUIRE(wide && !sc && !ph && !s2 && sw == 1 && ts == 0 && cout == 128 && cin % 32 == 0, RD_ESHAPE,
                "conv3: the 16 x 16 x 32 form needs the 8 x 32 tile form: cout 128, folded scales, stride 1, cin a multiple of 32 (cin %d)%s", cin,
diff --git a/rangedet_amd/csrc/rd_api.hip b/rangedet_amd/csrc/rd_api.hip
--- a/rangedet_amd/csrc/rd_api.hip
+++ b/rangedet_amd/csrc/rd_api.hip
@@ -200,6 +200,20 @@
   memset(out, 0, conv_packed_bytes(nt, cin, cout, dtype));
   if (is_h16(dtype)) pack_taps_frag(nt, cin, cout, out, get, dtype);
   else pack_taps(nt, cin, cout, dtype, out, get);
+  return RD_OK;
+}
+int rd_pack_deconv_weight_m16_host(const float* w, const float* fold_scale, int cin, int cout, int kh, int kw, int stride_w, int pad_w,
+                                   int phase, int dtype, void* out) {
+  RD_REQUIRE(w && out && fold_scale, RD_EINVAL, "pack_deconv_m16: null pointer");
+  RD_REQUIRE(is_h16(dtype), RD_EINVAL, "pack_deconv_m16: dtype %d (RD_BF16 or RD_F16)", dtype);
+  RD_REQUIRE(stride_w >= 1 && phase >= 0 && phase < stride_w, RD_EINVAL, "pack_deconv_m16: phase");
+  RD_REQUIRE((cout == 64 || cout == 128) && cin >= 32 && cin % 32 == 0, RD_ESHAPE, "pack_deconv_m16: cout %d (64, 128), cin %d (a multiple of 32)", cout, cin);
+  TapList tl = deconv_taps_sorted(kh, kw, stride_w, pad_w, phase);
+  RD_REQUIRE(tl.n == 6 && deconv_embeds_3x3(tl) && deconv_tap_set(tl), RD_ESHAPE, "pack_deconv_m16: phase %d is not a 3 x 2-tap set", phase);
+  memset(out, 0, conv_packed_bytes(6, cin, cout, dtype));
+  pack_taps_frag16(6, cin, cout, out, [&](int co, int ci, int t) {
+    return fold_scale[co] * w[(((size_t)ci * cout + co) * kh + tl.kh[t]) * kw + tl.kw[t]];
+  }, dtype);
   return RD_OK;
 }
 
@@ -482,14 +496,19 @@
              "deconv2d_all: kernel (%d,%d) stride %d pad %d cout %d is not a set of two-column 3x2 phases (use rd_deconv2d_bn_act per phase)",
              kh, kw, stride_w, pad_w, cout);
   RD_REQUIRE(w_phase_bytes >= (long)conv_packed_bytes(6, cin, cout, RD_BF16) && w_phase_bytes % 16 == 0, RD_EINVAL, "deconv2d_all: w_phase_bytes");
+  const bool m16 = (flags & RD_MFMA16) != 0;
+  flags &= ~RD_MFMA16;
+  RD_REQUIRE(!m16 || conv3_mfma16_phases_ok(cin, cout), RD_ESHAPE,
+             "deconv2d_all: RD_MFMA16 is not a launch form for cin %d, cout %d (rd_deconv2d_mfma16_ok)", cin, cout);
   allow_conv_lds();
   Conv3Phases ph;
   ph.nph = stride_w; ph.ts_mask = 0; ph.y_pc = y_cstride; ph.r_pc = r_cstride; ph.w_pb = w_phase_bytes;
   for (int p = 0; p < stride_w; ++p)
     if (deconv_tap_set(deconv_taps_sorted(kh, kw, stride_w, pad_w, p)) == 2) ph.ts_mask |= 1 << p;
   return launch_conv3(x, x_cstride, x_coff, w_packed_all, nullptr, shift, residual, r_cstride * stride_w, r_coff, y, y_cstride * stride_w,
-                      y_coff, B, H, Win, cin, cout, flags, 1, (hipStream_t)stream, 3, nullptr, dtype, &ph);
-}
+                      y_coff, B, H, Win, cin, cout, flags, 1, (hipStream_t)stream, 3, nullptr, dtype, &ph, nullptr, m16 ? C3_BODY_M16 : 0);
+}
+int rd_deconv2d_mfma16_ok(int cin, int cout, int phase_pairs) { return conv3_mfma16_phases_ok(cin, phase_pairs ? 2 * cout : cout) ? 1 : 0; }
 
 int rd_deconv2d_phase_pairs_ok(int kh, int kw, int stride_w, int pad_w, int cout, int dtype) {
   if (!rd_deconv2d_all_phases_ok(kh, kw, stride_w, pad_w, cout, dtype) || cout != 64 || stride_w % 2) return 0;
@@ -505,6 +524,17 @@
   for (size_t i = 0; i < blocks; ++i) {
     memcpy((unsigned char*)out + i * 4096, (const unsigned char*)phase_a + i * 2048, 2048);
     memcpy((unsigned char*)out + i * 4096 + 2048, (const unsigned char*)phase_b + i * 2048, 2048);
+  }
+  memset((unsigned char*)out + 2 * body, 0, 2 * RD_CONV_TAIL);
+  return RD_OK;
+}
+int rd_pack_deconv_phase_pair_m16_host(const void* phase_a, const void* phase_b, int cin, int dtype, void* out) {
+  RD_REQUIRE(phase_a && phase_b && out, RD_EINVAL, "pack_deconv_pair_m16: null pointer");
+  RD_REQUIRE(is_h16(dtype) && cin >= 32 && cin % 32 == 0, RD_EINVAL, "pack_deconv_pair_m16: dtype %d / cin %d (a multiple of 32)", dtype, cin);
+  const size_t body = conv_packed_body_bytes(6, cin, 64, RD_BF16), blocks = body / 4096;
+  for (size_t i = 0; i < blocks; ++i) {
+    memcpy((unsigned char*)out + i * 8192, (const unsigned char*)phase_a + i * 4096, 4096);
+    memcpy((unsigned char*)out + i * 8192 + 4096, (const unsigned char*)phase_b + i * 4096, 4096);
   }
   memset((unsigned char*)out + 2 * body, 0, 2 * RD_CONV_TAIL);
   return RD_OK;
@@ -524,13 +554,17 @@
   RD_REQUIRE(y_cstride == cout && y_coff == 0 && (!residual || (r_cstride == cout && r_coff == 0)), RD_ESHAPE,
              "deconv2d_pairs: the output / residual must be dense %d-channel tensors (two phases are one 128-channel write)", cout);
   RD_REQUIRE(w_pair_bytes >= (long)conv_packed_bytes(6, cin, 2 * cout, RD_BF16) && w_pair_bytes % 16 == 0, RD_EINVAL, "deconv2d_pairs: w_pair_bytes");
+  const bool m16 = (flags & RD_MFMA16) != 0;
+  flags &= ~RD_MFMA16;
+  RD_REQUIRE(!m16 || conv3_mfma16_phases_ok(cin, 2 * cout), RD_ESHAPE,
+             "deconv2d_pairs: RD_MFMA16 is not a launch form for cin %d, cout %d (rd_deconv2d_mfma16_ok)", cin, cout);
   allow_conv_lds();
   Conv3Phases ph;
   ph.nph = stride_w / 2; ph.ts_mask = 0; ph.y_pc = 2 * cout; ph.r_pc = 2 * cout; ph.w_pb = w_pair_bytes;
   for (int p = 0; p < stride_w; p += 2)
     if (deconv_tap_set(deconv_taps_sorted(kh, kw, stride_w, pad_w, p)) == 2) ph.ts_mask |= 1 << (p / 2);
   return launch_conv3(x, x_cstride, x_coff, w_packed_pairs, nullptr, shift2, residual, r_cstride * stride_w, r_coff, y, y_cstride * stride_w,
-                      y_coff, B, H, Win, cin, 2 * cout, flags, 1, (hipStream_t)stream, 3, nullptr, dtype, &ph);
+                      y_coff, B, H, Win, cin, 2 * cout, flags, 1, (hipStream_t)stream, 3, nullptr, dtype, &ph, nullptr, m16 ? C3_BODY_M16 : 0);
 }
 
 int rd_head_out(const void* x, int x_cstride, int x_coff, const float* w, const float* bias, float* out,
diff --git a/rangedet_amd/lib.py b/rangedet_amd/lib.py
--- a/rangedet_amd/lib.py
+++ b/rangedet_amd/lib.py
@@ -59,6 +59,9 @@
     "rd_deconv2d_bn_act_all": (c_int, [c_void_p, c_int, c_int, c_void_p, c_long, c_void_p, c_void_p, c_int, c_int, c_void_p,
                                        c_int, c_int, c_int, c_int, c_int, c_int, c_int, c_int, c_int, c_int, c_int, c_int,
                                        c_int, c_void_p]),
+    "rd_deconv2d_mfma16_ok": (c_int, [c_int, c_int, c_int]),
+    "rd_pack_deconv_weight_m16_host": (c_int, [c_void_p, c_void_p, c_int, c_int, c_int, c_int, c_int, c_int, c_int, c_int, c_void_p]),
+    "rd_pack_deconv_phase_pair_m16_host": (c_int, [c_void_p, c_void_p, c_int, c_int, c_void_p]),
     "rd_deconv2d_phase_pairs_ok": (c_int, [c_int, c_int, c_int, c_int, c_int, c_int]),
     "rd_pack_deconv_phase_pair_host": (c_int, [c_void_p, c_void_p, c_int, c_int, c_void_p]),
     "rd_deconv2d_bn_act_pairs": (c_int, [c_void_p, c_int, c_int, c_void_p, c_long, c_void_p, c_void_p, c_int, c_int, c_void_p,
@@ -292,7 +295,7 @@
         self.call("rd_pack_conv1x1_sc_m16_host", w.ctypes.data, fs.ctypes.data, dtype, out.ctypes.data)
         return out
 
-    def pack_deconv_weight(self, w_iohw, stride_w, pad_w, phase, dtype, fold_scale=None):
+    def pack_deconv_weight(self, w_iohw, stride_w, pad_w, phase, dtype, fold_scale=None, m16=False):
         w = np.ascontiguousarray(w_iohw, dtype=np.float32)
         cin, cout, kh, kw = w.shape
         nt = self.cdll.rd_deconv_phase_taps(kh, kw, stride_w, pad_w, phase)
@@ -300,8 +303,8 @@
             raise RangeDetError(nt, "deconv phase taps")
         out = np.zeros(self.cdll.rd_conv_packed_bytes(nt, cin, cout, dtype), dtype=np.uint8)
         fs = None if fold_scale is None else np.ascontiguousarray(fold_scale, dtype=np.float32)
-        self.call("rd_pack_deconv_weight_folded_host", w.ctypes.data, None if fs is None else fs.ctypes.data, cin, cout, kh, kw,
-                  stride_w, pad_w, phase, dtype, out.ctypes.data)
+        self.call("rd_pack_deconv_weight_m16_host" if m16 else "rd_pack_deconv_weight_folded_host", w.ctypes.data,
+                  None if fs is None else fs.ctypes.data, cin, cout, kh, kw, stride_w, pad_w, phase, dtype, out.ctypes.data)
         return out
 
     def pack_deconv_data_grad(self, w_iohw, stride_w, pad_w, dtype):
@@ -312,11 +315,12 @@
         self.call("rd_pack_deconv_data_grad_host", w.ctypes.data, cin, cout, kw, stride_w, pad_w, dtype, out.ctypes.data)
         return out
 
-    def pack_deconv_phase_pair(self, img_a, img_b, cin, dtype):
+    def pack_deconv_phase_pair(self, img_a, img_b, cin, dtype, m16=False):
         assert img_a.nbytes == img_b.nbytes
         out = np.empty(2 * img_a.nbytes, np.uint8)
         a, b = np.ascontiguousarray(img_a), np.ascontiguousarray(img_b)
-        self.call("rd_pack_deconv_phase_pair_host", a.ctypes.data, b.ctypes.data, cin, dtype, out.ctypes.data)
+        self.call("rd_pack_deconv_phase_pair_m16_host" if m16 else "rd_pack_deconv_phase_pair_host", a.ctypes.data, b.ctypes.data, cin, dtype,
+                  out.ctypes.data)
         return out
 
     def pack_head_weight(self, w, dtype=RD_BF16, m16=False):
diff --git a/rangedet_amd/lower.py b/rangedet_amd/lower.py
--- a/rangedet_amd/lower.py
+++ b/rangedet_amd/lower.py
@@ -97,6 +97,9 @@
                 cin = len(st["cmap"]) if st.get("cmap") else st["cin"]
                 if cin % 32 == 0 and cin >= 32:
                     st["m16"] = True
+            if st["kind"] == "deconv" and st.get("fold") and st.get("one_launch") and st["cin"] % 32 == 0 and st["cin"] >= 32 and \
+                    st["cout"] == 64 and st["stride_w"] == 4:
+                st["m16"] = True
 
     def _fuse_blocks(self):
         if not self.h16 or devswitch.get("RD_NO_FUSE_BLOCK"):
diff --git a/rangedet_amd/runtime.py b/rangedet_amd/runtime.py
--- a/rangedet_amd/runtime.py
+++ b/rangedet_amd/runtime.py
@@ -259,14 +259,17 @@
         w = pad_rows(np.asarray(P[st["name"] + "_weight"], np.float32), cout, axis=1)
         s, t = bn_affine(P, st["bn"], st["eps"], pad_to=cout)
         fold = bool(st.get("fold"))
-        imgs = [L.pack_deconv_weight(w, sw, pw, ph, dt, fold_scale=s if fold else None) for ph in range(sw)]
         flags = st["flags"] | (rdlib.RD_SCALE_FOLDED if fold else 0)
         geom = (*self._at(r), *self._at(o), self.B, x.H, x.W, st["cin"], cout, kh, kw, sw, pw)
         dense = all(v.cs == cout and v.co == 0 for v in (o, r) if v is not None)
-        all_phases = bool(st.get("one_launch")) and len({len(i) for i in imgs}) == 1 and \
+        all_phases = bool(st.get("one_launch")) and len({L.raw("rd_deconv_phase_taps")(kh, kw, sw, pw, ph) for ph in range(sw)}) == 1 and \
             L.raw("rd_deconv2d_all_phases_ok")(kh, kw, sw, pw, cout, dt) == 1
-        if all_phases and dense and L.raw("rd_deconv2d_phase_pairs_ok")(kh, kw, sw, pw, cout, dt) == 1:
-            pimgs = [L.pack_deconv_phase_pair(imgs[p], imgs[p + 1], st["cin"], dt) for p in range(0, sw, 2)]
+        pairs = all_phases and dense and L.raw("rd_deconv2d_phase_pairs_ok")(kh, kw, sw, pw, cout, dt) == 1
+        m16 = all_phases and fold and bool(st.get("m16")) and L.raw("rd_deconv2d_mfma16_ok")(st["cin"], cout, 1 if pairs else 0) == 1
+        flags |= rdlib.RD_MFMA16 if m16 else 0
+        imgs = [L.pack_deconv_weight(w, sw, pw, ph, dt, fold_scale=s if fold else None, m16=m16) for ph in range(sw)]
+        if pairs:
+            pimgs = [L.pack_deconv_phase_pair(imgs[p], imgs[p + 1], st["cin"], dt, m16=m16) for p in range(0, sw, 2)]
             yield ("rd_deconv2d_bn_act_pairs", *self._at(x), self._up(np.concatenate(pimgs)), len(pimgs[0]), self._up(np.concatenate([t, t])),
                    *geom, flags, dt)
         elif all_phases:
```

New measurement: 936.5 (median of 6 runs). No clear change (+0.2%).
